# laertispappas/MPI-k-selection

Measured on AMD Instinct MI355X. Metric: Gkeys/s exact k-th select, 2^30 int32 (1 GPU) / 2^33 (8 GPU); % HBM roofline, higher is better.
Workload: dtype int32; 1 GPU; exact k-th select (median) of 2^30 int32 keys per GPU, uniform_half; n_total=1073741824, k=536870912, keys_per_gpu=1073741824, family=uniform_half, parallelism=single, ranks=1

## Files before the change

include/kth.h:

```cpp
#ifndef KTH_H
#define KTH_H

#include <stddef.h>
#include <stdint.h>

#ifdef __cplusplus
extern "C" {
#endif

#define KTH_OK 0
#define KTH_EINVAL (-1)
#define KTH_ENOMEM (-2)
#define KTH_EHIP (-3)
#define KTH_ENODEV (-4)
#define KTH_EINTERNAL (-5)
#define KTH_ECOMM (-6)

#define KTH_VERSION 1

#define KTH_PATH_LDS 1
#define KTH_PATH_RADIX 2
#define KTH_PATH_WINDOW 3
#define KTH_PATH_WINDOW_FALLBACK 4

typedef struct kth_ctx kth_ctx;

typedef struct kth_stats {
    int32_t path;
    int32_t mode;
    uint32_t lo_key, hi_key;
    uint64_t n, k;
    uint64_t cnt_lt;
    uint64_t cnt_eq_lo, cnt_eq_hi;
    uint64_t candidates;
    uint64_t capacity;
    int32_t answer;
    int32_t error;
} kth_stats;

const char *kth_strerror(int code);
int kth_version(void);
const char *kth_build_id(void);
int kth_device_count(void);

int kth_select_i32(const int32_t *keys, int64_t n, int64_t k, int32_t *out);

int kth_ctx_create(int device, kth_ctx **ctx);
int kth_ctx_destroy(kth_ctx *ctx);
int kth_ctx_set_stream(kth_ctx *ctx, void *hip_stream);
int kth_ctx_sync(kth_ctx *ctx);
int kth_ctx_reserve(kth_ctx *ctx, int64_t n);

int kth_select_i32_ctx(kth_ctx *ctx, const int32_t *keys, int64_t n, int64_t k, int32_t *out);

int kth_select_i32_async(kth_ctx *ctx, const int32_t *d_keys, int64_t n, int64_t k, int32_t *d_out);

int kth_ctx_last_stats(kth_ctx *ctx, kth_stats *st);

int kth_ctx_coop(const kth_ctx *ctx);

#define KTH_HOOK_FAULT_TOPK_RANK 1
#define KTH_HOOK_FAULT_BARRIER 2
#define KTH_HOOK_TOPK_SEG_CAP 3
int kth_ctx_test_hook(kth_ctx *ctx, int hook, int64_t value);

int kth_ctx_enable_timing(kth_ctx *ctx, int on);
int kth_ctx_take_timing(kth_ctx *ctx, int64_t *n_selects, double *main_ms, double *total_ms);

#define KTH_ROWS_MAX_COLS 16384
int kth_select_rows_i32(kth_ctx *ctx, const int32_t *d_keys, int64_t rows, int32_t cols, int32_t k,
                        int32_t *d_out);
int kth_select_rows_f32(kth_ctx *ctx, const float *d_keys, int64_t rows, int32_t cols, int32_t k,
                        float *d_out);

#define KTH_TOPK_MAX_COLS 4096
int kth_topk_rows_i32(kth_ctx *ctx, const int32_t *d_keys, int64_t rows, int32_t cols, int32_t k, int largest,
                      int32_t *d_vals, int32_t *d_idx);
int kth_topk_rows_f32(kth_ctx *ctx, const float *d_keys, int64_t rows, int32_t cols, int32_t k, int largest,
                      float *d_vals, int32_t *d_idx);

int kth_topk_i32(kth_ctx *ctx, const int32_t *d_keys, int64_t n, int64_t k, int largest, int32_t *d_vals,
                 int64_t *d_idx);

int kth_fill_synthetic(kth_ctx *ctx, int32_t *d_out, int64_t n, int64_t offset, int64_t n_total,
                       int dist, uint64_t seed, int32_t param);

#define KTH_STATS_WORDS (8 + 2 * 2048)
#define KTH_DIST_DONE 3
#define KTH_DIST_MAX_LEVELS 3
#define KTH_DIST_LEVELS KTH_DIST_MAX_LEVELS
int kth_dist_begin(kth_ctx *ctx, uint64_t *d_slots, int64_t n_total, int64_t k);
int kth_dist_sample(kth_ctx *ctx, const int32_t *d_keys, int64_t n_local, uint32_t *d_sample,
                    int64_t s_local);
int kth_dist_window(kth_ctx *ctx, const uint32_t *d_sample, int64_t s_total);
int kth_dist_scan(kth_ctx *ctx, const int32_t *d_keys, int64_t n_local);
int kth_dist_level(kth_ctx *ctx, const int32_t *d_keys, int64_t n_local, int level);
int kth_dist_result(kth_ctx *ctx, int32_t *d_out);
int kth_dist_result_early(kth_ctx *ctx, int32_t *d_out);
int kth_dist_select_rccl(kth_ctx *ctx, void *nccl_all_reduce, void *nccl_all_gather, void *nccl_comm, int world,
                         const int32_t *d_keys, int64_t n_local, int64_t n_total, int64_t k, uint64_t *d_slots,
                         uint32_t *d_sample, uint32_t *d_gathered, int64_t s_local, int32_t *d_out, int early);
int64_t kth_dist_sample_size(int64_t n);
int kth_sample_chunk(void);
double kth_window_z(void);
int64_t kth_dist_cand_capacity(int64_t n_local);
int kth_window_slack64(void);

typedef struct kth_sharded kth_sharded;
int kth_sharded_create(const int *devices, int ngpu, kth_sharded **out);
int kth_sharded_destroy(kth_sharded *h);
int kth_sharded_select_i32(kth_sharded *h, const int32_t *const *shards, const int64_t *shard_n, int64_t k,
                           int32_t *out);
int kth_select_i32_sharded(const int32_t *const *dev_shards, const int64_t *shard_n, int ngpu, int64_t k,
                           int32_t *out);
int64_t kth_sharded_sample_split(const int64_t *shard_n, int P, int64_t *s_dev);
double kth_sharded_enqueue_us(const kth_sharded *h);

#ifdef __cplusplus
}
#endif
#endif
```

mpi-k-selection_amd/csrc/kth_api.hip:

```cpp
#include <hip/hip_runtime.h>

#include <algorithm>
#include <cmath>
#include <cstdio>
#include <cstdlib>
#include <cstring>
#include <vector>

#include "kth.h"
#include "kth_internal.h"
#include "kth_kernels.hip"
#include "kth_topk.hpp"

using kth::SelState;
using kth::StepArgs;
using kth::u64;

namespace {

constexpr int64_t SMALL_N = 16384;
constexpr int64_t RADIX_MAX_N = 1ll << 22;
constexpr int64_t SAMPLE_MAX = 1ll << 20;
constexpr double WINDOW_Z = 5.0;
double window_z() {
    static const double z = [] {
        const char *e = getenv("KTH_WINDOW_Z");
        const double v = e ? atof(e) : 0.0;
        return v > 0.0 ? v : WINDOW_Z;
    }();
    return z;
}
constexpr int LEVEL_GRID_MAX = 1024;
constexpr int POST_DENSE_GRID = 256;
constexpr int HEAD_GRID_MAX = 64;
int gather_grid(u64 nchunks) {
    const u64 per_wg = (u64)(kth::DENSE_BLK / kth::WAVE) * kth::GATHER_BATCH;
    return (int)std::max<u64>(1, (nchunks + per_wg - 1) / per_wg);
}
constexpr size_t ISLOT_WORDS = 3 * (size_t)kth::STATS_WORDS + 2;
constexpr size_t HSLOT_OFF = ISLOT_WORDS;
constexpr size_t HSLOT_WORDS = (size_t)kth::HEAD_LEVELS * kth::STATS_WORDS;
constexpr size_t FSLOT_OFF = HSLOT_OFF + HSLOT_WORDS;
constexpr size_t FSLOT_WORDS = (size_t)kth::FIN_LEVELS * kth::STATS_WORDS;
constexpr size_t PRE_OFF = FSLOT_OFF + 2 * FSLOT_WORDS;
constexpr size_t PRE_SET_WORDS = (size_t)kth::PRE_WORDS / 2;
static_assert(kth::PRE_WORDS % 4 == 0, "PreHist sets stay 16-byte aligned");
constexpr size_t ZERO_WORDS = PRE_OFF + 2 * PRE_SET_WORDS;
constexpr size_t BAR_OFF = ZERO_WORDS;
constexpr size_t TAIL_OFF = BAR_OFF + kth::BAR_WORDS / 2;
constexpr size_t SLOT_ALLOC_WORDS = TAIL_OFF + kth::FIN_LDS_KEYS / 2;
static_assert(kth::BAR_TAIL % 2 == 0, "the tail word is a u64");
constexpr u64 FIN_SPARSE_PER_WG = (u64)kth::DENSE_BLK * kth::FIN_UNROLL * 4;
constexpr double HEAD_SLACK = 1.5;
static_assert(KTH_STATS_WORDS == kth::STATS_WORDS, "include/kth.h slot size");
constexpr int MAX_EVENTS = 4 * 2048;
constexpr u64 TK_STAGE_MAX_FRAC = 16;
constexpr int TK5_SPLIT = 4;
constexpr int COOP_BACKOFF = 64;
constexpr uint64_t DSCAN_PER_WG = 1ull << 16;

#define HIP_TRY(x)                                                                                    \
    do {                                                                                              \
        hipError_t e_ = (x);                                                                          \
        if (e_ != hipSuccess) {                                                                       \
            if (getenv("KTH_DEBUG")) fprintf(stderr, "kth: %s failed: %s\n", #x, hipGetErrorString(e_)); \
            return KTH_EHIP;                                                                          \
        }                                                                                             \
    } while (0)

#define KTH_TRY(x)              \
    do {                        \
        int r_ = (x);           \
        if (r_ != KTH_OK) return r_; \
    } while (0)

}

struct kth_ctx {
    int device = 0;
    int main_grid[7] = {0, 0, 0, 0, 0, 0, 0};
    bool fault_topk_rank = false;
    bool fault_barrier = false;
    bool fault_once = false;
    bool topk_stage = true;
    u64 topk_seg_cap = 0;
    u64 sparse_per_wg = 0;
    int post_dense_grid = POST_DENSE_GRID;
    int post_sparse_grid = LEVEL_GRID_MAX;
    bool coop = true;
    bool coop_wanted = true;
    int coop_backoff = 0;
    bool coop_resident = true;
    int fin_grid = 256;
    uint32_t head_slack64 = (uint32_t)(HEAD_SLACK * 64);
    uint32_t head_abs_div = 1024;
    int fin_set = 0;
    bool pre_hist = true;
    hipStream_t stream = nullptr;
    bool own_stream = false;
    int num_cu = 256;
    SelState *st = nullptr;
    u64 *islots = nullptr;
    uint32_t *sample = nullptr;
    u64 sample_cap = 0;
    uint32_t *cand = nullptr;
    u64 cand_cap = 0;
    uint32_t *cand_rows = nullptr;
    u64 cand_rows_cap = 0;
    int32_t *tk_segv = nullptr;
    u64 tk_segv_cap = 0;
    uint8_t *tk_segp = nullptr;
    u64 tk_segp_cap = 0;
    uint32_t *tk_wcnt = nullptr;
    u64 tk_wcnt_cap = 0;
    uint32_t *tk_wstart = nullptr;
    u64 tk_wstart_cap = 0;
    kth::TkSeg tk_seg{};
    int32_t *staging = nullptr;
    u64 staging_cap = 0;
    u64 *topk = nullptr;
    u64 topk_cap = 0;
    int32_t *d_status = nullptr;
    int32_t *h_status = nullptr;
    SelState *h_state = nullptr;
    int last_state = -1;
    bool timing = false;
    std::vector<hipEvent_t> ev_main, ev_total;
    int main_used = 0, total_used = 0;
    bool dirty = false;
    bool dist_zero = false;
    bool dist_open = false;
    bool dist_coop_window = false;
    bool counts_left = false;
    u64 *stamps = nullptr;
    int stamp_next = 0;
    u64 *uslots = nullptr;
    int64_t dist_n = 0, dist_k = 0, dist_cap = 0;
    int dist_level_next = 0;
    u64 dscan_per_wg = DSCAN_PER_WG;
    int dist_levels = -1;
    int dist_result_slot = -1;
    int32_t *dist_early_out = nullptr;
    uint32_t *h_dist = nullptr;
    uint32_t *d_dist = nullptr;
    hipEvent_t ev_dist = nullptr;
    uint32_t dist_tag = 0;
};

namespace {

u64 *islot(kth_ctx *c, int i) { return c->islots + (size_t)i * kth::STATS_WORDS; }
u64 *cand_count(kth_ctx *c) { return c->islots + 3 * (size_t)kth::STATS_WORDS; }

int set_device(kth_ctx *c) {
    HIP_TRY(hipSetDevice(c->device));
    return KTH_OK;
}

int grow(void **p, u64 *cap, u64 want_bytes) {
    if (*cap >= want_bytes) return KTH_OK;
    (void)hipDeviceSynchronize();
    if (*p) (void)hipFree(*p);
    *p = nullptr;
    *cap = 0;
    if (hipMalloc(p, want_bytes) != hipSuccess) {
        (void)hipGetLastError();
        *p = nullptr;
        return KTH_ENOMEM;
    }
    *cap = want_bytes;
    return KTH_OK;
}

u64 cand_capacity(int64_t n) { return std::max<u64>(1ull << 20, (u64)n / 32); }

int64_t sample_size(int64_t n) {
    int64_t s = (n / 64) & ~int64_t(63);
    return std::min<int64_t>(SAMPLE_MAX, std::max<int64_t>(s, 64));
}

int reserve_cand(kth_ctx *c, int64_t n) {
    u64 bytes = cand_capacity(n) * 4;
    return grow(reinterpret_cast<void **>(&c->cand), &c->cand_cap, bytes);
}

void window_ranks(int64_t n, int64_t k, int64_t s, u64 *r_lo, u64 *r_hi) {
    const double p = (double)k / (double)n;
    const double r = p * (double)s;
    const double sig = std::sqrt(std::max(1.0, (double)s * p * (1.0 - p)));
    const double z = window_z();
    const double lo = std::floor(r - z * sig - 2.0), hi = std::ceil(r + z * sig + 2.0);
    *r_lo = lo < 1.0 ? 0 : (u64)lo;
    *r_hi = hi > (double)s ? (u64)s + 1 : (u64)std::max(1.0, hi);
}

constexpr int STAMP_LAUNCHES = 16, STAMP_WGS = 4096;
u64 *next_stamps(kth_ctx *c) {
    if (!c->stamps || c->stamp_next >= STAMP_LAUNCHES) return nullptr;
    return c->stamps + (size_t)(c->stamp_next++) * STAMP_WGS * 8;
}

void dump_stamps(kth_ctx *c) {
    if (!c->stamps) return;
    std::vector<u64> h((size_t)STAMP_LAUNCHES * STAMP_WGS * 8);
    (void)hipStreamSynchronize(c->stream);
    (void)hipMemcpy(h.data(), c->stamps, h.size() * 8, hipMemcpyDeviceToHost);
    u64 prev_end = 0;
    for (int l = 0; l < c->stamp_next; ++l) {
        const u64 *b = h.data() + (size_t)l * STAMP_WGS * 8;
        u64 t0 = ~0ull, tend = 0;
        int nwg = 0;
        for (int w = 0; w < STAMP_WGS; ++w)
            if (b[w * 8]) {
                nwg++;
                t0 = std::min(t0, b[w * 8]);
                for (int i = 0; i < 8; ++i) tend = std::max(tend, b[w * 8 + i]);
            }
        if (!nwg) continue;
        fprintf(stderr, "kth-stamps launch %d wgs %4d gap %7.2f |", l, nwg, prev_end ? (t0 - prev_end) / 100.0 : 0.0);
        for (int i = 0; i < 8; ++i) {
            double sum = 0, mx = 0;
            int cnt = 0;
            for (int w = 0; w < STAMP_WGS; ++w)
                if (b[w * 8] && b[w * 8 + i]) {
                    const double d = (b[w * 8 + i] - t0) / 100.0;
                    sum += d;
                    mx = std::max(mx, d);
                    cnt++;
                }
            if (cnt) fprintf(stderr, " p%d %6.2f/%6.2f", i, sum / cnt, mx);
        }
        fprintf(stderr, "\n");
        if (nwg >= 512) {
            std::vector<double> e;
            std::vector<double> ex[8];
            for (int w = 0; w < STAMP_WGS; ++w)
                if (b[w * 8] && b[w * 8 + 5]) {
                    const double d = (b[w * 8 + 5] - t0) / 100.0;
                    e.push_back(d);
                    ex[w % 8].push_back(d);
                }
            std::sort(e.begin(), e.end());
            if (!e.empty()) {
                auto pc = [&](double q) { return e[std::min(e.size() - 1, (size_t)(q * (double)e.size()))]; };
                fprintf(stderr, "kth-stamps   p5 pct: 1%% %.1f 10%% %.1f 25%% %.1f 50%% %.1f 75%% %.1f 90%% %.1f 99%% %.1f max %.1f\n",
                        pc(0.01), pc(0.10), pc(0.25), pc(0.50), pc(0.75), pc(0.90), pc(0.99), e.back());
                fprintf(stderr, "kth-stamps   p5 mean by wg%%8:");
                for (int x = 0; x < 8; ++x) {
                    double sm = 0;
                    for (double d : ex[x]) sm += d;
                    fprintf(stderr, " %.1f", ex[x].empty() ? 0.0 : sm / ex[x].size());
                }
                fprintf(stderr, "\n");
            }
        }
        if (nwg >= 512) {
            for (int x = 0; x < 8; ++x) {
                double sum = 0, mn = 1e30, mx = 0;
                int cnt = 0;
                for (int w = x; w < STAMP_WGS; w += 8)
                    if (b[w * 8] && b[w * 8 + 3]) {
                        const double d = (b[w * 8 + 3] - t0) / 100.0;
                        sum += d;
                        mn = std::min(mn, d);
                        mx = std::max(mx, d);
                        cnt++;
                    }
                if (cnt) fprintf(stderr, "kth-stamps   wg%%8=%d p3 min %7.2f mean %7.2f max %7.2f\n", x, mn, sum / cnt, mx);
            }
        }
        prev_end = tend;
    }
    (void)hipMemsetAsync(c->stamps, 0, h.size() * 8, c->stream);
    c->stamp_next = 0;
}

StepArgs step(kth_ctx *c, int adv, int st_in, int st_out, const u64 *in, u64 *acc, u64 *zero) {
    StepArgs a;
    memset(&a, 0, sizeof a);
    a.stamps = next_stamps(c);
    a.st_in = st_in >= 0 ? c->st + st_in : nullptr;
    a.st_out = c->st + st_out;
    a.stats_in = in;
    a.stats_acc = acc;
    a.stats_zero = zero;
    a.adv = adv;
    a.cand = c->cand;
    a.cand_count = cand_count(c);
    a.cap = c->cand_cap / 4;
    return a;
}

void ev_mark(kth_ctx *c, std::vector<hipEvent_t> &pool, int &used) {
    if (!c->timing || used >= (int)pool.size()) return;
    (void)hipEventRecord(pool[used++], c->stream);
}
void ev_main(kth_ctx *c) { ev_mark(c, c->ev_main, c->main_used); }

int launch_check() {
    hipError_t e = hipGetLastError();
    if (e != hipSuccess) {
        if (getenv("KTH_DEBUG")) fprintf(stderr, "kth: launch failed: %s\n", hipGetErrorString(e));
        return KTH_EHIP;
    }
    return KTH_OK;
}

constexpr u64 DENSE_PER_WG = 1ull << 16;
constexpr u64 SPARSE_PER_WG = (u64)kth::BLK * kth::LEVEL_UNROLL * 4;

int level_grid(u64 count, u64 per_wg) {
    u64 g = (count + per_wg - 1) / per_wg;
    return (int)std::max<u64>(1, std::min<u64>(LEVEL_GRID_MAX, g));
}

u64 sparse_wg(const kth_ctx *c) { return c->sparse_per_wg ? c->sparse_per_wg : SPARSE_PER_WG; }

void launch_level(kth_ctx *c, StepArgs a, bool dense, int grid) {
    if (dense) {
        a.min_per_wg = DENSE_PER_WG;
        kth::k_level<kth::DENSE_BLK><<<grid, kth::DENSE_BLK, 0, c->stream>>>(a);
    } else {
        a.min_per_wg = sparse_wg(c);
        kth::k_level<kth::BLK><<<grid, kth::BLK, 0, c->stream>>>(a);
    }
}

int run_small(kth_ctx *c, const int32_t *keys, int64_t n, int64_t k, int32_t *d_out, int32_t *d_status) {
    c->last_state = 1;
    ev_main(c);
    kth::k_small<<<1, kth::SMALL_BLOCK, (size_t)n * 4, c->stream>>>(keys, (u64)n, (u64)k, d_out, d_status,
                                                                    c->st + 1);
    ev_main(c);
    return launch_check();
}

kth::CoopArgs coop_args(kth_ctx *c, u64 slot_off, int32_t *d_out, int32_t *d_status) {
    kth::CoopArgs x;
    memset(&x, 0, sizeof x);
    x.slots = c->islots + slot_off;
    x.bar = reinterpret_cast<uint32_t *>(c->islots + BAR_OFF);
    x.tail = reinterpret_cast<uint32_t *>(c->islots + TAIL_OFF);
    x.d_out = d_out;
    x.d_status = d_status;
    x.dense_per_wg = DENSE_PER_WG;
    x.sparse_per_wg = FIN_SPARSE_PER_WG;
    x.slack64 = c->head_slack64;
    x.fault = c->fault_barrier ? 1u : 0u;
    if (c->fault_once) c->fault_barrier = false;
    return x;
}

constexpr size_t FIN_DYN_LDS = (size_t)kth::FIN_LDS_KEYS * 4;
uint32_t *pre_set(kth_ctx *c, int set) {
    return reinterpret_cast<uint32_t *>(c->islots + PRE_OFF + (size_t)set * PRE_SET_WORDS);
}

void launch_finish(kth_ctx *c, StepArgs a, int32_t *d_out, int32_t *d_status, bool with_pre = false) {
    const size_t mine = FSLOT_OFF + (size_t)c->fin_set * FSLOT_WORDS;
    a.stats_zero = c->islots + FSLOT_OFF + (size_t)(1 - c->fin_set) * FSLOT_WORDS;
    a.zero_words = FSLOT_WORDS;
    kth::CoopArgs x = coop_args(c, mine, d_out, d_status);
    x.zero2 = c->islots + HSLOT_OFF;
    x.zero2_words = HSLOT_WORDS;
    x.pre = with_pre ? pre_set(c, c->fin_set) : nullptr;
    x.pre_zero = pre_set(c, 1 - c->fin_set);
    kth::k_finish<<<c->fin_grid, kth::DENSE_BLK, FIN_DYN_LDS, c->stream>>>(a, x);
    c->fin_set ^= 1;
}

int run_radix(kth_ctx *c, const int32_t *keys, int64_t n, int64_t k, int32_t *d_out, int32_t *d_status) {
    if (c->coop) {
        StepArgs a = step(c, kth::ADV_INIT_FULL, -1, 1, nullptr, nullptr, nullptr);
        a.keys = keys;
        a.n_local = (u64)n;
        a.init_n = (u64)n;
        a.init_k = (u64)k;
        ev_main(c);
        launch_finish(c, a, d_out, d_status);
        ev_main(c);
        c->last_state = 1;
        return launch_check();
    }
    StepArgs a = step(c, kth::ADV_INIT_FULL, -1, 0, nullptr, islot(c, 1), islot(c, 2));
    a.keys = keys;
    a.n_local = (u64)n;
    a.init_n = (u64)n;
    a.init_k = (u64)k;
    ev_main(c);
    launch_level(c, a, true, level_grid((u64)n, DENSE_PER_WG));
    ev_main(c);
    a = step(c, kth::ADV_PICK, 0, 1, islot(c, 1), islot(c, 2), islot(c, 0));
    a.keys = keys;
    a.n_local = (u64)n;
    launch_level(c, a, false, level_grid((u64)n, sparse_wg(c)));
    a = step(c, kth::ADV_PICK, 1, 0, islot(c, 2), islot(c, 0), islot(c, 1));
    a.keys = keys;
    a.n_local = (u64)n;
    launch_level(c, a, false, level_grid((u64)n, sparse_wg(c)));
    a = step(c, kth::ADV_PICK, 0, 1, islot(c, 0), nullptr, nullptr);
    kth::k_result<<<1, kth::BLK, 0, c->stream>>>(a, d_out, d_status, c->islots, ISLOT_WORDS);
    c->last_state = 1;
    return launch_check();
}

void launch_main(kth_ctx *c, const StepArgs &a, int tflag, uint32_t *tflags) {
    const int g = c->main_grid[tflag];
    const kth::TkSeg none{};
    switch (tflag) {
    case 1: kth::k_main<1><<<g, kth::BLK, 0, c->stream>>>(a, c->cand, tflags, nullptr, none); break;
    case 2: kth::k_main<2><<<g, kth::BLK, 0, c->stream>>>(a, c->cand, tflags, nullptr, none); break;
    case 3: kth::k_main<3><<<g, kth::BLK, 0, c->stream>>>(a, c->cand, tflags, c->cand_rows, none); break;
    case 4: kth::k_main<4><<<g, kth::BLK, 0, c->stream>>>(a, c->cand, tflags, c->cand_rows, none); break;
    case 5: kth::k_main<5><<<g, kth::BLK, 0, c->stream>>>(a, c->cand, tflags, nullptr, c->tk_seg); break;
    case 6: kth::k_main<6><<<g, kth::BLK, 0, c->stream>>>(a, c->cand, tflags, nullptr, c->tk_seg); break;
    default: kth::k_main<0><<<g, kth::BLK, 0, c->stream>>>(a, c->cand, nullptr, nullptr, none); break;
    }
}

int run_window(kth_ctx *c, const int32_t *keys, int64_t n, int64_t k, int32_t *d_out, int32_t *d_status,
               int tflag = 0, uint32_t *tflags = nullptr) {
    const int64_t s = sample_size(n);
    const u64 nchunks = ((u64)s + kth::SAMPLE_CHUNK - 1) / kth::SAMPLE_CHUNK;
    const u64 stride = (u64)n / nchunks;
    u64 r_lo, r_hi;
    window_ranks(n, k, s, &r_lo, &r_hi);
    KTH_TRY(grow(reinterpret_cast<void **>(&c->sample), &c->sample_cap, (u64)s * 4));
    KTH_TRY(reserve_cand(c, n));

    if (c->coop) {
        StepArgs a = step(c, kth::ADV_INIT_SAMPLE, -1, 0, nullptr, nullptr, islot(c, 1));
        a.zero_words = 2 * (u64)kth::STATS_WORDS + 1;
        a.init_n = (u64)n;
        a.init_k = (u64)k;
        a.init_s = (u64)s;
        a.r_lo = r_lo;
        a.r_hi = r_hi;
        kth::CoopArgs hx = coop_args(c, HSLOT_OFF, nullptr, nullptr);
        if (tflag == 0 && c->head_abs_div) hx.abs_min = (u64)s / c->head_abs_div;
        kth::k_head<<<gather_grid(nchunks), kth::DENSE_BLK, 0, c->stream>>>(a, hx, keys, (u64)n, stride, c->sample,
                                                                          (u64)s);
        a = step(c, kth::ADV_CARRY, 0, 1, nullptr, islot(c, 1), nullptr);
        a.keys = keys;
        a.n_local = (u64)n;
        const bool pre = tflag == 0 && c->pre_hist;
        if (pre) a.pre_hist = pre_set(c, c->fin_set);
        ev_main(c);
        launch_main(c, a, tflag, tflags);
        ev_main(c);
        a = step(c, kth::ADV_DECIDE, 1, 0, islot(c, 1), nullptr, nullptr);
        a.keys = keys;
        a.n_local = (u64)n;
        launch_finish(c, a, d_out, d_status, pre);
        c->last_state = 0;
        c->counts_left = true;
        return launch_check();
    }
    StepArgs a = step(c, kth::ADV_INIT_SAMPLE, -1, 0, nullptr, islot(c, 1), islot(c, 2));
    a.init_n = (u64)n;
    a.init_k = (u64)k;
    a.init_s = (u64)s;
    a.r_lo = r_lo;
    a.r_hi = r_hi;
    kth::k_gather<true><<<gather_grid(nchunks), kth::DENSE_BLK, 0, c->stream>>>(a, keys, (u64)n, stride, c->sample,
                                                                              (u64)s);
    const int gs = level_grid((u64)s, sparse_wg(c));
    a = step(c, kth::ADV_PICK, 0, 1, islot(c, 1), islot(c, 2), islot(c, 0));
    a.sample = c->sample;
    a.sample_count = (u64)s;
    launch_level(c, a, false, gs);
    a = step(c, kth::ADV_PICK, 1, 0, islot(c, 2), islot(c, 0), islot(c, 1));
    a.sample = c->sample;
    a.sample_count = (u64)s;
    launch_level(c, a, false, gs);
    a = step(c, kth::ADV_PICK, 0, 1, islot(c, 0), islot(c, 1), islot(c, 2));
    a.keys = keys;
    a.n_local = (u64)n;
    ev_main(c);
    launch_main(c, a, tflag, tflags);
    ev_main(c);
    a = step(c, kth::ADV_DECIDE, 1, 0, islot(c, 1), islot(c, 2), islot(c, 0));
    a.keys = keys;
    a.n_local = (u64)n;
    launch_level(c, a, true, c->post_dense_grid);
    a = step(c, kth::ADV_PICK, 0, 1, islot(c, 2), islot(c, 0), islot(c, 1));
    a.keys = keys;
    a.n_local = (u64)n;
    launch_level(c, a, false, c->post_sparse_grid);
    a = step(c, kth::ADV_PICK, 1, 0, islot(c, 0), islot(c, 1), islot(c, 2));
    a.keys = keys;
    a.n_local = (u64)n;
    launch_level(c, a, false, c->post_sparse_grid);
    a = step(c, kth::ADV_PICK, 0, 1, islot(c, 1), nullptr, nullptr);
    kth::k_result<<<1, kth::BLK, 0, c->stream>>>(a, d_out, d_status, c->islots, ISLOT_WORDS);
    c->last_state = 1;
    return launch_check();
}

void coop_tick(kth_ctx *c) {
    if (c->coop_backoff > 0 && --c->coop_backoff == 0) c->coop = c->coop_wanted;
}

int select_async(kth_ctx *c, const int32_t *d_keys, int64_t n, int64_t k, int32_t *d_out, int32_t *d_status,
                 int tflag = 0, uint32_t *tflags = nullptr) {
    if (!c || !d_keys || (!d_out && !d_status) || n < 1 || k < 1 || k > n) return KTH_EINVAL;
    KTH_TRY(set_device(c));
    coop_tick(c);
    if (c->dirty) {
        HIP_TRY(hipMemsetAsync(c->islots, 0, SLOT_ALLOC_WORDS * sizeof(u64), c->stream));
        c->dirty = false;
    }
    int rc;
    ev_mark(c, c->ev_total, c->total_used);
    if (n <= SMALL_N)
        rc = run_small(c, d_keys, n, k, d_out, d_status);
    else if (n <= RADIX_MAX_N)
        rc = run_radix(c, d_keys, n, k, d_out, d_status);
    else
        rc = run_window(c, d_keys, n, k, d_out, d_status, tflag, tflags);
    ev_mark(c, c->ev_total, c->total_used);
    if (rc != KTH_OK) c->dirty = true;
    if (c->stamps) dump_stamps(c);
    return rc;
}

bool is_device_ptr(const void *p) {
    hipPointerAttribute_t at;
    hipError_t e = hipPointerGetAttributes(&at, p);
    if (e != hipSuccess) {
        (void)hipGetLastError();
        return false;
    }
    return at.type == hipMemoryTypeDevice || at.type == hipMemoryTypeManaged;
}

thread_local kth_ctx *tl_ctx = nullptr;

#ifndef KTH_ROWS_R0
#define KTH_ROWS_R0 4
#endif
template <bool F32, int KPL, bool TOPK>
void launch_rows_reg(kth_ctx *c, bool vec, int g, const uint32_t *d_keys, u64 R, uint32_t C, uint32_t K,
                     uint32_t *d_out, uint32_t flip, uint32_t *vals, int32_t *idx) {
    if (vec && C == (uint32_t)(KPL * kth::WAVE))
        kth::k_rows_reg<F32, KPL, true, KTH_ROWS_R0, TOPK, true>
            <<<g, kth::RW_BLOCK, 0, c->stream>>>(d_keys, R, C, K, d_out, flip, vals, idx);
    else if (vec)
        kth::k_rows_reg<F32, KPL, true, KTH_ROWS_R0, TOPK, false>
            <<<g, kth::RW_BLOCK, 0, c->stream>>>(d_keys, R, C, K, d_out, flip, vals, idx);
    else
        kth::k_rows_reg<F32, KPL, false, KTH_ROWS_R0, TOPK, false>
            <<<g, kth::RW_BLOCK, 0, c->stream>>>(d_keys, R, C, K, d_out, flip, vals, idx);
}

template <bool F32, bool TOPK>
int launch_rows(kth_ctx *c, const uint32_t *d_keys, int64_t rows, int32_t cols, int32_t k, uint32_t *d_out,
                uint32_t flip = 0, uint32_t *vals = nullptr, int32_t *idx = nullptr) {
    const bool vec = (reinterpret_cast<uintptr_t>(d_keys) & 15u) == 0 && cols % 4 == 0;
    const int rows_per_wg = kth::RW_BLOCK / kth::WAVE;
    const int64_t g64 = (rows + rows_per_wg - 1) / rows_per_wg;
    if (g64 > 0x7FFFFFFF) return KTH_EINVAL;
    const int g = (int)g64;
    const u64 R = (u64)rows;
    const uint32_t C = (uint32_t)cols, K = (uint32_t)k;
    if (cols <= 1024)
        launch_rows_reg<F32, 16, TOPK>(c, vec, g, d_keys, R, C, K, d_out, flip, vals, idx);
    else if (cols <= 2048)
        launch_rows_reg<F32, 32, TOPK>(c, vec, g, d_keys, R, C, K, d_out, flip, vals, idx);
    else if (cols <= 4096)
        launch_rows_reg<F32, 64, TOPK>(c, vec, g, d_keys, R, C, K, d_out, flip, vals, idx);
    else if (!TOPK)
        kth::k_rows<F32><<<(int)std::min<int64_t>(rows, 1 << 20), kth::ROWS_BLOCK, (size_t)cols * 4, c->stream>>>(
            d_keys, R, C, (u64)k, d_out);
    return launch_check();
}

}

extern "C" {

const char *kth_strerror(int code) {
    switch (code) {
    case KTH_OK: return "ok";
    case KTH_EINVAL: return "invalid argument";
    case KTH_ENOMEM: return "out of memory";
    case KTH_EHIP: return "HIP runtime error";
    case KTH_ENODEV: return "no HIP device";
    case KTH_EINTERNAL: return "device-side consistency check failed";
    case KTH_ECOMM: return "RCCL unavailable or a collective failed";
    default: return "unknown error";
    }
}

int kth_version(void) { return KTH_VERSION; }

#ifndef KTH_BUILD_ID
#define KTH_BUILD_ID "unknown"
#endif
const char *kth_build_id(void) { return KTH_BUILD_ID; }

int kth_device_count(void) {
    int n = 0;
    if (hipGetDeviceCount(&n) != hipSuccess) {
        (void)hipGetLastError();
        return 0;
    }
    return n;
}

int kth_ctx_create(int device, kth_ctx **out) {
    if (!out) return KTH_EINVAL;
    *out = nullptr;
    int ndev = kth_device_count();
    if (ndev <= 0) return KTH_ENODEV;
    if (device < 0 || device >= ndev) return KTH_EINVAL;
    kth_ctx *c = new kth_ctx();
    c->device = device;
    if (getenv("KTH_STAMPS")) {
        const size_t bytes = (size_t)STAMP_LAUNCHES * STAMP_WGS * 8 * 8;
        if (hipMalloc(reinterpret_cast<void **>(&c->stamps), bytes) != hipSuccess || hipMemset(c->stamps, 0, bytes) != hipSuccess) {
            (void)hipGetLastError();
            c->stamps = nullptr;
        }
    }
    int rc = KTH_OK;
    do {
        if (hipSetDevice(device) != hipSuccess) { rc = KTH_EHIP; break; }
        hipDeviceProp_t prop;
        if (hipGetDeviceProperties(&prop, device) == hipSuccess && prop.multiProcessorCount > 0)
            c->num_cu = prop.multiProcessorCount;
        {
            const void *fns[7] = {reinterpret_cast<const void *>(kth::k_main<0>),
                                  reinterpret_cast<const void *>(kth::k_main<1>),
                                  reinterpret_cast<const void *>(kth::k_main<2>),
                                  reinterpret_cast<const void *>(kth::k_main<3>),
                                  reinterpret_cast<const void *>(kth::k_main<4>),
                                  reinterpret_cast<const void *>(kth::k_main<5>),
                                  reinterpret_cast<const void *>(kth::k_main<6>)};
            const char *e = getenv("KTH_MAIN_WG_PER_CU");
            for (int v = 0; v < 7; ++v) {
                int per = 4;
                hipFuncAttributes fa;
                if (hipFuncGetAttributes(&fa, fns[v]) == hipSuccess && fa.numRegs > 0) {
                    const int alloc = (fa.numRegs + 7) / 8 * 8;
                    const int by_vgpr = std::min(8, 512 / alloc);
                    const int lds = (int)fa.sharedSizeBytes;
                    const int by_lds = lds > 0 ? (160 * 1024) / lds : 8;
                    per = std::max(1, std::min(by_vgpr, by_lds));
                }
                (void)hipGetLastError();
                if (e && atoi(e) > 0) per = atoi(e);
                c->main_grid[v] = c->num_cu * per;
            }
            if (const char *g = getenv("KTH_SPARSE_PER_WG")) c->sparse_per_wg = (u64)std::max(0, atoi(g));
            if (const char *g = getenv("KTH_DSCAN_PER_WG")) c->dscan_per_wg = (u64)std::max(1024, atoi(g));
            if (const char *g = getenv("KTH_POST_DENSE_GRID")) c->post_dense_grid = std::max(1, atoi(g));
            if (const char *g = getenv("KTH_POST_SPARSE_GRID")) c->post_sparse_grid = std::max(1, atoi(g));
            if (const char *g = getenv("KTH_COOP")) c->coop = atoi(g) != 0;
            if (const char *g = getenv("KTH_PRE_HIST")) c->pre_hist = atoi(g) != 0;
            c->fin_grid = c->num_cu;
            if (const char *g = getenv("KTH_FIN_GRID")) c->fin_grid = std::max(1, std::min(atoi(g), c->num_cu));
            if (const char *g = getenv("KTH_HEAD_SLACK")) c->head_slack64 = (uint32_t)std::max(0.0, atof(g) * 64.0);
            if (const char *g = getenv("KTH_HEAD_ABS")) c->head_abs_div = (uint32_t)std::max(0, atoi(g));
            if (const char *g = getenv("KTH_TOPK_STAGE")) c->topk_stage = atoi(g) != 0;
        }
        if (hipStreamCreateWithFlags(&c->stream, hipStreamNonBlocking) != hipSuccess) { rc = KTH_EHIP; break; }
        c->own_stream = true;
        if (hipMalloc(reinterpret_cast<void **>(&c->st), 2 * sizeof(SelState)) != hipSuccess ||
            hipMalloc(reinterpret_cast<void **>(&c->islots), SLOT_ALLOC_WORDS * sizeof(u64)) != hipSuccess ||
            hipMalloc(reinterpret_cast<void **>(&c->d_status), 4 * sizeof(int32_t)) != hipSuccess ||
            hipHostMalloc(reinterpret_cast<void **>(&c->h_status), 4 * sizeof(int32_t), 0) != hipSuccess ||
            hipHostMalloc(reinterpret_cast<void **>(&c->h_state), sizeof(SelState), 0) != hipSuccess) {
            rc = KTH_ENOMEM;
            break;
        }
        if (hipMemset(c->st, 0, 2 * sizeof(SelState)) != hipSuccess ||
            hipMemset(c->islots, 0, SLOT_ALLOC_WORDS * sizeof(u64)) != hipSuccess) {
            rc = KTH_EHIP;
            break;
        }
        (void)hipFuncSetAttribute(reinterpret_cast<const void *>(kth::k_small),
                                  hipFuncAttributeMaxDynamicSharedMemorySize, SMALL_N * 4);
        (void)hipFuncSetAttribute(reinterpret_cast<const void *>(kth::k_rows<false>),
                                  hipFuncAttributeMaxDynamicSharedMemorySize, KTH_ROWS_MAX_COLS * 4);
        (void)hipFuncSetAttribute(reinterpret_cast<const void *>(kth::k_rows<true>),
                                  hipFuncAttributeMaxDynamicSharedMemorySize, KTH_ROWS_MAX_COLS * 4);
        if (hipFuncSetAttribute(reinterpret_cast<const void *>(kth::k_finish),
                                hipFuncAttributeMaxDynamicSharedMemorySize, (int)FIN_DYN_LDS) != hipSuccess)
            c->coop = false;
        (void)hipGetLastError();
        {
            int fin_per_cu = 0, head_per_cu = 0;
            if (hipOccupancyMaxActiveBlocksPerMultiprocessor(&fin_per_cu, reinterpret_cast<const void *>(kth::k_finish),
                                                             kth::DENSE_BLK, FIN_DYN_LDS) != hipSuccess ||
                hipOccupancyMaxActiveBlocksPerMultiprocessor(&head_per_cu, reinterpret_cast<const void *>(kth::k_head),
                                                             kth::DENSE_BLK, 0) != hipSuccess)
                fin_per_cu = head_per_cu = -1;
            (void)hipGetLastError();
            if (fin_per_cu >= 0 &&
                ((int64_t)fin_per_cu * c->num_cu < c->fin_grid || (int64_t)head_per_cu * c->num_cu < HEAD_GRID_MAX)) {
                c->coop = false;
                c->coop_resident = false;
            }
        }
    } while (0);
    c->coop_wanted = c->coop;
    if (rc != KTH_OK) {
        kth_ctx_destroy(c);
        return rc;
    }
    *out = c;
    return KTH_OK;
}

int kth_ctx_test_hook(kth_ctx *c, int hook, int64_t value) {
    if (!c || value < 0) return KTH_EINVAL;
    switch (hook) {
    case KTH_HOOK_FAULT_TOPK_RANK: c->fault_topk_rank = value != 0; return KTH_OK;
    case KTH_HOOK_FAULT_BARRIER:
        if (value > 2) return KTH_EINVAL;
        c->fault_barrier = value != 0;
        c->fault_once = value == 2;
        return KTH_OK;
    case KTH_HOOK_TOPK_SEG_CAP:
        if (value > (int64_t)1 << 40) return KTH_EINVAL;
        c->topk_seg_cap = (u64)value;
        return KTH_OK;
    default: return KTH_EINVAL;
    }
}

int kth_ctx_destroy(kth_ctx *c) {
    if (!c) return KTH_EINVAL;
    (void)hipSetDevice(c->device);
    if (c->stream) (void)hipStreamSynchronize(c->stream);
    for (hipEvent_t e : c->ev_main) (void)hipEventDestroy(e);
    for (hipEvent_t e : c->ev_total) (void)hipEventDestroy(e);
    if (c->st) (void)hipFree(c->st);
    if (c->islots) (void)hipFree(c->islots);
    if (c->sample) (void)hipFree(c->sample);
    if (c->cand) (void)hipFree(c->cand);
    if (c->cand_rows) (void)hipFree(c->cand_rows);
    if (c->tk_segv) (void)hipFree(c->tk_segv);
    if (c->tk_segp) (void)hipFree(c->tk_segp);
    if (c->tk_wcnt) (void)hipFree(c->tk_wcnt);
    if (c->tk_wstart) (void)hipFree(c->tk_wstart);
    if (c->staging) (void)hipFree(c->staging);
    if (c->topk) (void)hipFree(c->topk);
    if (c->d_status) (void)hipFree(c->d_status);
    if (c->stamps) (void)hipFree(c->stamps);
    if (c->h_status) (void)hipHostFree(c->h_status);
    if (c->h_state) (void)hipHostFree(c->h_state);
    if (c->h_dist) (void)hipHostFree(c->h_dist);
    if (c->ev_dist) (void)hipEventDestroy(c->ev_dist);
    if (c->own_stream && c->stream) (void)hipStreamDestroy(c->stream);
    if (tl_ctx == c) tl_ctx = nullptr;
    delete c;
    return KTH_OK;
}

int kth_ctx_set_stream(kth_ctx *c, void *s) {
    if (!c) return KTH_EINVAL;
    KTH_TRY(set_device(c));
    if (c->own_stream && c->stream) {
        (void)hipStreamSynchronize(c->stream);
        (void)hipStreamDestroy(c->stream);
        c->own_stream = false;
    }
    c->stream = reinterpret_cast<hipStream_t>(s);
    return KTH_OK;
}

int kth_ctx_sync(kth_ctx *c) {
    if (!c) return KTH_EINVAL;
    KTH_TRY(set_device(c));
    HIP_TRY(hipStreamSynchronize(c->stream));
    return KTH_OK;
}

int kth_ctx_reserve(kth_ctx *c, int64_t n) {
    if (!c || n < 0) return KTH_EINVAL;
    KTH_TRY(set_device(c));
    if (n > RADIX_MAX_N) {
        KTH_TRY(grow(reinterpret_cast<void **>(&c->sample), &c->sample_cap, (u64)sample_size(n) * 4));
        KTH_TRY(reserve_cand(c, n));
    }
    return KTH_OK;
}

int kth_select_i32_async(kth_ctx *c, const int32_t *d_keys, int64_t n, int64_t k, int32_t *d_out) {
    if (!d_out) return KTH_EINVAL;
    return select_async(c, d_keys, n, k, d_out, nullptr);
}

int kth_select_i32_ctx(kth_ctx *c, const int32_t *keys, int64_t n, int64_t k, int32_t *out) {
    if (!c || !keys || !out || n < 1 || k < 1 || k > n) return KTH_EINVAL;
    KTH_TRY(set_device(c));
    const int32_t *dk = keys;
    if (!is_device_ptr(keys)) {
        KTH_TRY(grow(reinterpret_cast<void **>(&c->staging), &c->staging_cap, (u64)n * 4));
        HIP_TRY(hipMemcpyAsync(c->staging, keys, (size_t)n * 4, hipMemcpyHostToDevice, c->stream));
        dk = c->staging;
    }
    KTH_TRY(select_async(c, dk, n, k, nullptr, c->d_status));
    HIP_TRY(hipMemcpyAsync(c->h_status, c->d_status, 2 * sizeof(int32_t), hipMemcpyDeviceToHost, c->stream));
    HIP_TRY(hipStreamSynchronize(c->stream));
    if (c->h_status[1] == (int32_t)kth::ERR_BARRIER && c->coop) {
        c->dirty = true;
        c->coop = false;
        c->coop_backoff = COOP_BACKOFF + 1;
        KTH_TRY(select_async(c, dk, n, k, nullptr, c->d_status));
        HIP_TRY(hipMemcpyAsync(c->h_status, c->d_status, 2 * sizeof(int32_t), hipMemcpyDeviceToHost, c->stream));
        HIP_TRY(hipStreamSynchronize(c->stream));
    }
    if (c->h_status[1] != 0) {
        c->dirty = true;
        return KTH_EINTERNAL;
    }
    *out = c->h_status[0];
    return KTH_OK;
}

int kth_select_i32(const int32_t *keys, int64_t n, int64_t k, int32_t *out) {
    if (!keys || !out || n < 1 || k < 1 || k > n) return KTH_EINVAL;
    if (!tl_ctx) {
        int dev = 0;
        if (kth_device_count() <= 0) return KTH_ENODEV;
        if (hipGetDevice(&dev) != hipSuccess) {
            (void)hipGetLastError();
            dev = 0;
        }
        KTH_TRY(kth_ctx_create(dev, &tl_ctx));
    }
    return kth_select_i32_ctx(tl_ctx, keys, n, k, out);
}

int kth_ctx_coop(const kth_ctx *c) {
    if (!c) return KTH_EINVAL;
    return c->coop ? 1 : 0;
}

int kth_ctx_last_stats(kth_ctx *c, kth_stats *out) {
    if (!c || !out) return KTH_EINVAL;
    if (c->last_state < 0) return KTH_EINVAL;
    KTH_TRY(set_device(c));
    HIP_TRY(hipMemcpyAsync(c->h_state, c->st + c->last_state, sizeof(SelState), hipMemcpyDeviceToHost,
                           c->stream));
    HIP_TRY(hipStreamSynchronize(c->stream));
    const SelState &s = *c->h_state;
    memset(out, 0, sizeof *out);
    out->path = (int32_t)s.path;
    out->mode = (int32_t)s.mode;
    out->lo_key = s.lo;
    out->hi_key = s.hi;
    out->n = s.n;
    out->k = s.k;
    out->cnt_lt = s.cnt[kth::C_LT];
    out->cnt_eq_lo = s.cnt[kth::C_EQLO];
    out->cnt_eq_hi = s.cnt[kth::C_EQHI];
    out->candidates = s.cnt[kth::C_IN];
    out->capacity = c->cand_cap / 4;
    out->answer = (int32_t)(s.answer ^ 0x80000000u);
    out->error = (int32_t)s.error;
    return KTH_OK;
}

int kth_ctx_enable_timing(kth_ctx *c, int on) {
    if (!c) return KTH_EINVAL;
    KTH_TRY(set_device(c));
    if (on && c->ev_main.empty()) {
        c->ev_main.resize(MAX_EVENTS);
        c->ev_total.resize(MAX_EVENTS);
        for (auto &e : c->ev_main) HIP_TRY(hipEventCreate(&e));
        for (auto &e : c->ev_total) HIP_TRY(hipEventCreate(&e));
    }
    c->timing = on != 0;
    c->main_used = c->total_used = 0;
    return KTH_OK;
}

int kth_ctx_take_timing(kth_ctx *c, int64_t *n_sel, double *main_ms, double *total_ms) {
    if (!c || !n_sel || !main_ms || !total_ms) return KTH_EINVAL;
    KTH_TRY(set_device(c));
    HIP_TRY(hipStreamSynchronize(c->stream));
    double m = 0, t = 0;
    int64_t nm = 0;
    for (int i = 0; i + 1 < c->main_used; i += 2) {
        float a = 0;
        HIP_TRY(hipEventElapsedTime(&a, c->ev_main[i], c->ev_main[i + 1]));
        m += a;
        nm++;
    }
    for (int i = 0; i + 1 < c->total_used; i += 2) {
        float b = 0;
        HIP_TRY(hipEventElapsedTime(&b, c->ev_total[i], c->ev_total[i + 1]));
        t += b;
    }
    c->main_used = c->total_used = 0;
    *n_sel = nm;
    *main_ms = m;
    *total_ms = t;
    return KTH_OK;
}

int kth_select_rows_i32(kth_ctx *c, const int32_t *d_keys, int64_t rows, int32_t cols, int32_t k, int32_t *d_out) {
    if (!c || !d_keys || !d_out || rows < 0 || cols < 1 || cols > KTH_ROWS_MAX_COLS || k < 1 || k > cols)
        return KTH_EINVAL;
    if (rows == 0) return KTH_OK;
    KTH_TRY(set_device(c));
    return launch_rows<false, false>(c, reinterpret_cast<const uint32_t *>(d_keys), rows, cols, k,
                              reinterpret_cast<uint32_t *>(d_out));
}

int kth_select_rows_f32(kth_ctx *c, const float *d_keys, int64_t rows, int32_t cols, int32_t k, float *d_out) {
    if (!c || !d_keys || !d_out || rows < 0 || cols < 1 || cols > KTH_ROWS_MAX_COLS || k < 1 || k > cols)
        return KTH_EINVAL;
    if (rows == 0) return KTH_OK;
    KTH_TRY(set_device(c));
    return launch_rows<true, false>(c, reinterpret_cast<const uint32_t *>(d_keys), rows, cols, k,
                             reinterpret_cast<uint32_t *>(d_out));
}

int kth_topk_rows_i32(kth_ctx *c, const int32_t *d_keys, int64_t rows, int32_t cols, int32_t k, int largest,
                      int32_t *d_vals, int32_t *d_idx) {
    if (!c || !d_keys || (!d_vals && !d_idx) || rows < 0 || cols < 1 || cols > KTH_TOPK_MAX_COLS || k < 1 ||
        k > cols)
        return KTH_EINVAL;
    if (rows == 0) return KTH_OK;
    KTH_TRY(set_device(c));
    return launch_rows<false, true>(c, reinterpret_cast<const uint32_t *>(d_keys), rows, cols, k, nullptr,
                                    largest ? 0xFFFFFFFFu : 0u, reinterpret_cast<uint32_t *>(d_vals), d_idx);
}

int kth_topk_rows_f32(kth_ctx *c, const float *d_keys, int64_t rows, int32_t cols, int32_t k, int largest,
                      float *d_vals, int32_t *d_idx) {
    if (!c || !d_keys || (!d_vals && !d_idx) || rows < 0 || cols < 1 || cols > KTH_TOPK_MAX_COLS || k < 1 ||
        k > cols)
        return KTH_EINVAL;
    if (rows == 0) return KTH_OK;
    KTH_TRY(set_device(c));
    return launch_rows<true, true>(c, reinterpret_cast<const uint32_t *>(d_keys), rows, cols, k, nullptr,
                                   largest ? 0xFFFFFFFFu : 0u, reinterpret_cast<uint32_t *>(d_vals), d_idx);
}

int kth_topk_i32(kth_ctx *c, const int32_t *d_keys, int64_t n, int64_t k, int largest, int32_t *d_vals,
                 int64_t *d_idx) {
    if (!c || !d_keys || (!d_vals && !d_idx) || n < 1 || k < 1 || k > n) return KTH_EINVAL;
    KTH_TRY(set_device(c));
    const u64 ntiles = ((u64)n + kth::TK_TILE - 1) / kth::TK_TILE;
    const u64 nblk = (ntiles + kth::TK_TILES_PER_BLOCK - 1) / kth::TK_TILES_PER_BLOCK;
    u64 head = ((16u - (uint32_t)(reinterpret_cast<uintptr_t>(d_keys) & 15u)) & 15u) >> 2;
    if (head > (u64)n) head = (u64)n;
    const u64 nfull = (((u64)n - head) >> 2) / ((u64)kth::BLK * kth::MAIN_UNROLL);
    const bool aligned = (reinterpret_cast<uintptr_t>(d_keys) & 15u) == 0;
    const bool window = n > RADIX_MAX_N;
    const bool few = (u64)k * kth::TK_TILE * 64 <= (u64)n;
    const bool staged = aligned && window && !few && (u64)k * TK_STAGE_MAX_FRAC <= (u64)n && c->topk_stage;
    const int tf = staged                                  ? (largest ? 6 : 5)
                   : (aligned && window && !few)           ? (largest ? 4 : 3)
                   : (u64)k * kth::TK_TILE <= (u64)n ? (largest ? 2 : 1)
                                                             : 0;
    const u64 ncov = tf >= 3 ? nfull * kth::MAIN_UNROLL : 0;
    const u64 Gm = (u64)c->main_grid[tf];
    const kth::RowWords rwl{Gm, tf >= 3 ? kth::rw_seg_words(nfull, Gm) : kth::fl_seg_bytes(nfull, Gm)};
    const u64 fwords = tf >= 3 ? kth::TF_W0 + rwl.G * (kth::BLK / kth::WAVE) * rwl.seg
                               : 4 + rwl.G * (kth::BLK / kth::WAVE) * rwl.seg / 4;
    const u64 fw64 = (fwords + 1) / 2, before = (ntiles + 1) / 2 + ntiles + 4 * nblk + 2;
    const u64 words = before + fw64 + 32;
    KTH_TRY(grow(reinterpret_cast<void **>(&c->topk), &c->topk_cap, words * sizeof(u64)));
    const u64 foff = (before + 31) & ~31ull;
    uint32_t *tflags = reinterpret_cast<uint32_t *>(c->topk + foff);
    HIP_TRY(hipMemsetAsync(tflags, 0, 16, c->stream));
    if (tf == 3 || tf == 4) {
        KTH_TRY(reserve_cand(c, n));
        KTH_TRY(grow(reinterpret_cast<void **>(&c->cand_rows), &c->cand_rows_cap, c->cand_cap));
    }
    u64 seg_cap = 0;
    uint32_t nwin = 0;
    if (tf >= 5) {
        const u64 nwaves = (u64)c->main_grid[tf] * (kth::BLK / kth::WAVE);
        const u64 seg_total = std::max<u64>({1ull << 20, (u64)n / 16, (u64)k + (u64)k / 8 + (u64)n / 64});
        seg_cap = c->topk_seg_cap ? c->topk_seg_cap : (seg_total + nwaves - 1) / nwaves;
        seg_cap = (seg_cap + 3) & ~3ull;
        KTH_TRY(reserve_cand(c, n));
        KTH_TRY(grow(reinterpret_cast<void **>(&c->tk_segv), &c->tk_segv_cap, seg_cap * nwaves * 4));
        KTH_TRY(grow(reinterpret_cast<void **>(&c->tk_segp), &c->tk_segp_cap, seg_cap * nwaves));
        KTH_TRY(grow(reinterpret_cast<void **>(&c->tk_wcnt), &c->tk_wcnt_cap, ncov * (kth::BLK / kth::WAVE) * 4 + 16));
        const u64 G = (u64)c->main_grid[tf];
        nwin = (uint32_t)(((nfull + G - 1) / G + kth::TK5_WIN_TILES - 1) / kth::TK5_WIN_TILES);
        KTH_TRY(grow(reinterpret_cast<void **>(&c->tk_wstart), &c->tk_wstart_cap, nwaves * std::max(nwin, 1u) * 4));
        const uint32_t nt = (u64)k * 32 >= (u64)n ? 1u : 0u;
        c->tk_seg = kth::TkSeg{c->tk_segv, c->tk_segp, (uint32_t)seg_cap, tflags + 3, c->tk_wstart, nwin, nt};
    }
    int64_t rank = largest ? n - k + 1 : k;
    if (c->fault_topk_rank && n > 1) rank = rank < n ? rank + 1 : rank - 1;
    KTH_TRY(select_async(c, d_keys, n, rank, nullptr, c->d_status, tf, tflags));
    const uint32_t *keys = reinterpret_cast<const uint32_t *>(d_keys);
    const uint32_t flip = largest ? 0xFFFFFFFFu : 0u;
    u64 *toff = c->topk, *bsum = toff + ntiles, *bbase = bsum + 2 * nblk, *meta = bbase + 2 * nblk;
    uint32_t *tcnt = reinterpret_cast<uint32_t *>(meta + 2);
    const SelState *sel_st = c->st + c->last_state;
    const int waves = kth::TK_BLOCK / kth::WAVE;
    const int g = (int)std::min<u64>((ntiles + waves * kth::WAVE - 1) / (waves * kth::WAVE), (u64)c->num_cu * 16);
    if (tf >= 5) {
        auto tk5c = (u64)k * 64 >= (u64)n ? kth::k_tk5_count<true> : kth::k_tk5_count<false>;
        tk5c<<<c->main_grid[tf] * TK5_SPLIT, kth::TK_BLOCK, 0, c->stream>>>(
            c->tk_segv, seg_cap, c->tk_wstart, nwin, (u64)c->main_grid[tf], tflags, nfull, c->d_status, flip,
            c->tk_wcnt, tcnt);
        kth::k_topk_count<true, 2><<<g, kth::TK_BLOCK, 0, c->stream>>>(keys, (u64)n, ntiles, c->d_status, flip, tcnt,
                                                                       tflags, head, nfull, sel_st, ncov);
    } else if (tf >= 3) {
        HIP_TRY(hipMemsetAsync(tcnt, 0, ntiles * 4, c->stream));
        kth::k_topk_cands<<<c->num_cu * 8, kth::TK_BLOCK, 0, c->stream>>>(
            c->cand, c->cand_rows, cand_count(c), c->cand_cap / 4, c->d_status, flip, tcnt, tflags, sel_st);
        kth::k_topk_count<true, 1><<<g, kth::TK_BLOCK, 0, c->stream>>>(keys, (u64)n, ntiles, c->d_status, flip,
                                                                          tcnt, tflags, head, nfull, sel_st, ncov, rwl);
    } else if (aligned) {
        kth::k_topk_count<true, 0><<<g, kth::TK_BLOCK, 0, c->stream>>>(keys, (u64)n, ntiles, c->d_status, flip,
                                                                           tcnt, tflags, head, nfull, sel_st, 0, rwl);
    } else {
        kth::k_topk_count<false, 0><<<g, kth::TK_BLOCK, 0, c->stream>>>(keys, (u64)n, ntiles, c->d_status, flip,
                                                                            tcnt, tflags, head, nfull, sel_st, 0, rwl);
    }
    kth::k_topk_bases<<<(int)nblk, kth::TK_BLOCK, 0, c->stream>>>(
        tcnt, ntiles, toff, bsum, (u64)k, bbase, meta, c->st + c->last_state,
        reinterpret_cast<uint32_t *>(c->islots + BAR_OFF) + kth::BAR_TOPK_ARRIVE);
    if (tf >= 5) {
        auto tk5w = (u64)k * 32 <= (u64)n ? kth::k_tk5_write<kth::TK5_STAGE_SMALL> : kth::k_tk5_write<kth::TK5_STAGE_LARGE>;
        tk5w<<<c->main_grid[tf] * TK5_SPLIT, kth::TK_BLOCK, 0, c->stream>>>(
            c->tk_segv, c->tk_segp, seg_cap, c->tk_wstart, nwin, (u64)c->main_grid[tf], tflags, nfull, c->d_status,
            flip, c->tk_wcnt, tcnt, toff, bbase, meta, d_vals, d_idx);
        kth::k_topk_write<true, true><<<g, kth::TK_BLOCK, 0, c->stream>>>(keys, (u64)n, ntiles, c->d_status, flip,
                                                                          tcnt, toff, bbase, meta, d_vals, d_idx,
                                                                          tflags, ncov);
    } else if (aligned)
        kth::k_topk_write<true><<<g, kth::TK_BLOCK, 0, c->stream>>>(keys, (u64)n, ntiles, c->d_status, flip, tcnt,
                                                                    toff, bbase, meta, d_vals, d_idx);
    else
        kth::k_topk_write<false><<<g, kth::TK_BLOCK, 0, c->stream>>>(keys, (u64)n, ntiles, c->d_status, flip, tcnt,
                                                                     toff, bbase, meta, d_vals, d_idx);
    return launch_check();
}

int kth_fill_synthetic(kth_ctx *c, int32_t *d_out, int64_t n, int64_t offset, int64_t n_total, int dist, uint64_t seed,
                       int32_t param) {
    if (!c || (!d_out && n > 0) || n < 0 || offset < 0 || dist < 0 || dist > 7) return KTH_EINVAL;
    if (n == 0) return KTH_OK;
    KTH_TRY(set_device(c));
    uint32_t step = 1;
    if (n_total > 0 && n_total <= (int64_t)0xFFFFFFFFll) {
        u64 s = (1ull << 32) / (u64)n_total;
        step = s > 0xFFFFFFFFull ? 0xFFFFFFFFu : (s ? (uint32_t)s : 1u);
    }
    const int g = (int)std::min<int64_t>((n + kth::BLK - 1) / kth::BLK, (int64_t)c->num_cu * 16);
    kth::k_fill<<<g, kth::BLK, 0, c->stream>>>(d_out, (u64)n, (u64)offset, step, dist, seed, param);
    return launch_check();
}

int64_t kth_dist_sample_size(int64_t n) { return sample_size(n); }

int kth_sample_chunk(void) { return kth::SAMPLE_CHUNK; }

double kth_window_z(void) { return window_z(); }

int64_t kth_dist_cand_capacity(int64_t n_local) { return (int64_t)cand_capacity(std::max<int64_t>(n_local, 1)); }

int kth_window_slack64(void) { return (int)(HEAD_SLACK * 64); }

int kth_dist_begin(kth_ctx *c, uint64_t *d_slots, int64_t n_total, int64_t k) {
    if (!c || !d_slots || n_total < 1 || k < 1 || k > n_total) return KTH_EINVAL;
    KTH_TRY(set_device(c));
    if (!c->h_dist) {
        if (hipHostMalloc(reinterpret_cast<void **>(&c->h_dist), kth::DIST_STATUS_WORDS * sizeof(uint32_t),
                          hipHostMallocMapped | hipHostMallocCoherent) != hipSuccess) {
            (void)hipGetLastError();
            c->h_dist = nullptr;
            return KTH_ENOMEM;
        }
        HIP_TRY(hipHostGetDevicePointer(reinterpret_cast<void **>(&c->d_dist), c->h_dist, 0));
        HIP_TRY(hipEventCreateWithFlags(&c->ev_dist, hipEventDisableTiming));
    }
    coop_tick(c);
    c->uslots = reinterpret_cast<u64 *>(d_slots);
    c->dist_n = n_total;
    c->dist_k = k;
    c->dist_level_next = -1;
    c->dist_levels = -1;
    c->dist_result_slot = -1;
    c->dist_early_out = nullptr;
    c->dist_zero = true;
    if (c->dirty || c->dist_open || c->counts_left)
        HIP_TRY(hipMemsetAsync(c->islots, 0, SLOT_ALLOC_WORDS * sizeof(u64), c->stream));
    c->dirty = false;
    c->counts_left = false;
    c->dist_open = true;
    return KTH_OK;
}

int kth_dist_sample(kth_ctx *c, const int32_t *d_keys, int64_t n_local, uint32_t *d_sample, int64_t s_local) {
    if (!c || !d_keys || !d_sample || s_local < 64 || s_local % 64 || n_local < s_local) return KTH_EINVAL;
    KTH_TRY(set_device(c));
    const u64 nchunks = ((u64)s_local + kth::SAMPLE_CHUNK - 1) / kth::SAMPLE_CHUNK;
    const u64 stride = (u64)n_local / nchunks;
    StepArgs a;
    memset(&a, 0, sizeof a);
    if (c->dist_zero && c->uslots) {
        a.stats_zero = c->uslots;
        a.zero_words = 3 * (u64)KTH_STATS_WORDS;
    }
    kth::k_gather<false><<<gather_grid(nchunks), kth::DENSE_BLK, 0, c->stream>>>(a, d_keys, (u64)n_local, stride, d_sample,
                                                                                (u64)s_local);
    KTH_TRY(launch_check());
    if (a.zero_words) c->dist_zero = false;
    return KTH_OK;
}

int kth_dist_window(kth_ctx *c, const uint32_t *d_sample, int64_t s_total) {
    if (!c || !d_sample || s_total < 1 || !c->uslots) return KTH_EINVAL;
    KTH_TRY(set_device(c));
    if (c->dist_zero) {
        HIP_TRY(hipMemsetAsync(c->uslots, 0, 3 * (size_t)KTH_STATS_WORDS * 8, c->stream));
        c->dist_zero = false;
    }
    u64 r_lo, r_hi;
    window_ranks(c->dist_n, c->dist_k, s_total, &r_lo, &r_hi);
    if (c->coop && s_total % 64 == 0 && s_total < (1ll << 29)) {
        StepArgs a = step(c, kth::ADV_INIT_SAMPLE, -1, 0, nullptr, nullptr, nullptr);
        a.init_n = (u64)c->dist_n;
        a.init_k = (u64)c->dist_k;
        a.init_s = (u64)s_total;
        a.r_lo = r_lo;
        a.r_hi = r_hi;
        kth::CoopArgs x = coop_args(c, HSLOT_OFF, nullptr, nullptr);
        x.sample_ready = 1;
        const int grid = (int)std::min<int64_t>(64, std::max<int64_t>(1, s_total / (16 * 1024)));
        kth::k_head<<<grid, kth::DENSE_BLK, 0, c->stream>>>(a, x, nullptr, 0, 0, const_cast<uint32_t *>(d_sample),
                                                           (u64)s_total);
        c->dist_coop_window = true;
        return launch_check();
    }
    c->dist_coop_window = false;
    StepArgs a = step(c, kth::ADV_INIT_SAMPLE, -1, 0, nullptr, islot(c, 1), islot(c, 2));
// ... 160 lines not shown
```

mpi-k-selection_amd/csrc/kth_coop.hpp:

```cpp
#pragma once

namespace kth {

struct CoopArgs {
    u64 *slots;
    uint32_t *bar;
    int32_t *d_out, *d_status;
    u64 dense_per_wg, sparse_per_wg;
    uint32_t slack64;
    u64 abs_min;
    u64 *zero2;
    u64 zero2_words;
    uint32_t *tail;
    uint32_t sample_ready;
    uint32_t fault;
    const uint32_t *pre;
    uint32_t *pre_zero;
};

template <int BLOCK>
__device__ __forceinline__ void pick_slot_copies(SelState &ss, const u64 *slot, uint32_t nb, uint32_t copies,
                                                 u64 *tmp , u64 *scratch, u64 *cnt0) {
    constexpr int PER = NBINS / BLOCK;
#pragma unroll
    for (int j = 0; j < PER; ++j)
        tmp[threadIdx.x * PER + j] =
            __hip_atomic_load(slot + NCOUNTS + threadIdx.x * PER + j, __ATOMIC_RELAXED, __HIP_MEMORY_SCOPE_AGENT);
    __syncthreads();
    u64 h0[PER];
#pragma unroll
    for (int j = 0; j < PER; ++j) {
        const uint32_t b = threadIdx.x * PER + j;
        u64 sum = 0;
        if (b < nb)
            for (uint32_t c = 0; c < copies; ++c) sum += tmp[c * nb + b];
        h0[j] = sum;
    }
    __syncthreads();
    pick_state<BLOCK, PER>(ss, h0, h0, true, scratch, nullptr, cnt0);
}

template <int BLOCK>
__device__ __forceinline__ void pick_pre(SelState &ss, const uint32_t *pre, uint32_t nb, u64 *scratch, u64 *cnt0) {
    constexpr int PER = NBINS / BLOCK;
    u64 h0[PER];
#pragma unroll
    for (int j = 0; j < PER; ++j) {
        const uint32_t b = threadIdx.x * PER + j;
        uint32_t sum = 0;
        if (b < nb)
#pragma unroll
            for (int c = 0; c < PRE_COPIES; ++c) sum += pre[c * PRE_BINS + b];
        h0[j] = sum;
    }
    pick_state<BLOCK, PER>(ss, h0, h0, true, scratch, nullptr, cnt0);
}

template <int BLOCK>
__device__ __forceinline__ void hist_flush_copies(uint32_t (*lh)[NBINS], uint32_t nb, uint32_t copies, u64 *acc) {
    __syncthreads();
    u64 *dst = acc + NCOUNTS + (blockIdx.x % copies) * nb;
    for (uint32_t b = threadIdx.x; b < nb; b += BLOCK) {
        const uint32_t c = lh[0][b];
        if (c) atomicAdd(&dst[b], (u64)c);
    }
}

__device__ __forceinline__ uint32_t active_wgs(u64 count, u64 per_wg) {
    const u64 want = (count + per_wg - 1) / per_wg;
    return (uint32_t)(want < (u64)gridDim.x ? want : (u64)gridDim.x);
}

__global__ __launch_bounds__(DENSE_BLK) void k_head(StepArgs a, CoopArgs x, const int32_t *__restrict__ keys,
                                                    u64 n_keys, u64 stride, uint32_t *__restrict__ sample, u64 s) {
    __shared__ SelState ss;
    __shared__ u64 scratch[2 * (DENSE_BLK / WAVE) + 8];
    __shared__ __attribute__((aligned(16))) uint32_t lh[2][NBINS];
    __shared__ uint32_t s_base[BAR_NG];
    KTH_STAMP(a, 0);
    GridBar gb = grid_bar_init(x.bar, s_base);
    for (int i = threadIdx.x; i < 2 * NBINS / 4; i += DENSE_BLK) reinterpret_cast<uint4 *>(&lh[0][0])[i] = make_uint4(0, 0, 0, 0);
    for (u64 i = (u64)blockIdx.x * DENSE_BLK + threadIdx.x; i < a.zero_words; i += (u64)gridDim.x * DENSE_BLK)
        a.stats_zero[i] = 0;
    advance<DENSE_BLK>(ss, a, scratch);
    bool share;
    HistPlan plan = make_plan(ss, &share);
    auto hist_sample = [&]() {
        const CoherentBuf sb(sample, (uint32_t)(s * 4));
        const uint32_t nv = (uint32_t)(s / 4), per = DENSE_BLK * HEAD_UNROLL;
        for (uint32_t v0 = blockIdx.x * per; v0 < nv; v0 += gridDim.x * per) {
            uint4 q[HEAD_UNROLL];
#pragma unroll
            for (int u = 0; u < HEAD_UNROLL; ++u) {
                const uint32_t v = v0 + u * DENSE_BLK + threadIdx.x;
                q[u] = sb.load16(v < nv ? v * 16u : 0u);
            }
#pragma unroll
            for (int u = 0; u < HEAD_UNROLL; ++u) {
                const bool in = v0 + u * DENSE_BLK + threadIdx.x < nv;
                hist_add<DENSE_BLK>(lh, plan, q[u].x, in);
                hist_add<DENSE_BLK>(lh, plan, q[u].y, in);
                hist_add<DENSE_BLK>(lh, plan, q[u].z, in);
                hist_add<DENSE_BLK>(lh, plan, q[u].w, in);
            }
        }
    };
    bool from_chunks = false;
#ifdef KTH_HEAD_STORE_SAMPLE
    constexpr bool kHeadStore = true;
#else
    constexpr bool kHeadStore = false;
#endif
    if (x.sample_ready)
        hist_sample();
    else if (gather_head_fast<DENSE_BLK, kHeadStore>(keys, stride, sample, s, lh, plan, blockIdx.x, gridDim.x))
        from_chunks = !kHeadStore;
    else
        gather_chunks<DENSE_BLK, true, true>(keys, n_keys, stride, sample, s, lh, plan);
#ifdef KTH_HEAD_DIAG
    KTH_STAMP(a, 4);
#endif
    hist_flush<DENSE_BLK>(lh, plan, x.slots);
    KTH_STAMP(a, 1);
#ifdef KTH_HEAD_DIAG
    wait_mem();
    KTH_STAMP(a, 6);
#endif
    const EarlyWindow ew{a.r_lo, a.r_hi, x.slack64, x.abs_min};
    bool ok = true;
    for (int L = 0;; ++L) {
        grid_sync(gb, s_base, ok);
        if (x.fault) ok = false;
        if (L == 0) KTH_STAMP(a, 2);
        if (L == 1) KTH_STAMP(a, 5);
        pick_slot<DENSE_BLK>(ss, x.slots + (size_t)L * STATS_WORDS, share, scratch, &ew);
        if (L == 0) KTH_STAMP(a, 3);
        if (L == 1) KTH_STAMP(a, 6);
        if (ss.mode != MODE_SAMPLE || L + 1 >= HEAD_LEVELS) break;
        plan = make_plan(ss, &share);
        for (int i = threadIdx.x; i < 2 * NBINS / 4; i += DENSE_BLK)
            reinterpret_cast<uint4 *>(&lh[0][0])[i] = make_uint4(0, 0, 0, 0);
        __syncthreads();
        if (from_chunks)
            head_hist_chunks<DENSE_BLK>(keys, stride, s, lh, plan, blockIdx.x, gridDim.x);
        else
            hist_sample();
        hist_flush<DENSE_BLK>(lh, plan, x.slots + (size_t)(L + 1) * STATS_WORDS);
        if (L == 0) KTH_STAMP(a, 4);
    }
    if (blockIdx.x == 0 && threadIdx.x == 0) {
        SelState o = ss;
        const uint32_t berr = __hip_atomic_exchange(x.bar + BAR_ERR, 0u, __ATOMIC_RELAXED, __HIP_MEMORY_SCOPE_AGENT);
        if ((!ok || berr) && !o.error) {
            o.error = ERR_BARRIER;
            o.mode = MODE_DONE;
        } else if (o.mode == MODE_SAMPLE && !o.error) {
            o.error = 16 + o.mode;
            o.mode = MODE_DONE;
        }
        o.share = 0;
        *a.st_out = o;
    }
    grid_bar_finish(gb, s_base);
    KTH_STAMP(a, 7);
}

constexpr int FIN_LDS_KEYS = 32768;
constexpr int FIN_UNROLL = 4;

__device__ __forceinline__ void finish_keys(uint32_t (*lh)[NBINS], const HistPlan &plan, const uint4 &x, bool xr,
                                            uint32_t valid4) {
    const uint32_t X = xr ? 0x80000000u : 0u;
    hist_add<DENSE_BLK>(lh, plan, x.x ^ X, valid4 & 1u);
    hist_add<DENSE_BLK>(lh, plan, x.y ^ X, valid4 & 2u);
    hist_add<DENSE_BLK>(lh, plan, x.z ^ X, valid4 & 4u);
    hist_add<DENSE_BLK>(lh, plan, x.w ^ X, valid4 & 8u);
}

constexpr uint32_t TAIL_STAGE = 2 * NBINS;

__device__ bool finish_tail(const StepArgs &a, SelState &ss, const CoopArgs &x, uint4 *res, u64 nk, bool xr,
                            uint32_t (*lh)[NBINS], u64 *scratch) {
    __shared__ uint32_t s_n, s_last, s_total, s_ln;
    __shared__ uint32_t s_list[WAVE];
    __shared__ u64 s_off, s_c;
    const uint32_t X = xr ? 0x80000000u : 0u;
    const uint32_t W = ss.W, base = ss.base, done = ss.t[0].done, prefix = ss.t[0].prefix;
    const uint32_t psh = W - done;
    const uint32_t nv = (uint32_t)((nk + 3) / 4);
    u64 *ctl = reinterpret_cast<u64 *>(x.bar + BAR_TAIL);
    uint32_t *stage = &lh[0][0];
    const int lane = threadIdx.x & (WAVE - 1);
    if (threadIdx.x == 0) s_n = 0;
    __syncthreads();
    auto keep = [&](uint32_t key, bool valid) {
        const bool m = valid && ((key - base) >> psh) == prefix;
        const u64 b = __ballot(m);
        if (b == 0) return;
        uint32_t at = 0;
        if (lane == 0) at = atomicAdd(&s_n, (uint32_t)__popcll(b));
        at = __shfl(at, 0, WAVE);
        const uint32_t i = at + (uint32_t)__builtin_amdgcn_mbcnt_hi((uint32_t)(b >> 32), __builtin_amdgcn_mbcnt_lo((uint32_t)b, 0u));
        if (m && i < TAIL_STAGE) stage[i] = key;
    };
    for (uint32_t v0 = 0; v0 < nv; v0 += DENSE_BLK) {
        const uint32_t v = v0 + threadIdx.x;
        uint4 q = make_uint4(0, 0, 0, 0);
        uint32_t valid4 = 0;
        if (v < nv) {
            q = res[v];
            const u64 e = 4ull * v;
            valid4 = nk - e >= 4 ? 0xFu : (1u << (uint32_t)(nk - e)) - 1u;
        }
        keep(q.x ^ X, valid4 & 1u);
        keep(q.y ^ X, valid4 & 2u);
        keep(q.z ^ X, valid4 & 4u);
        keep(q.w ^ X, valid4 & 8u);
    }
    __syncthreads();
    const uint32_t n_mine = s_n;
    if (threadIdx.x == 0) {
        const u64 old = __hip_atomic_fetch_add(ctl, (1ull << 32) | n_mine, __ATOMIC_RELAXED, __HIP_MEMORY_SCOPE_AGENT);
        s_off = (uint32_t)old;
        s_last = (uint32_t)(old >> 32) == gridDim.x - 1u;
        s_total = (uint32_t)old + n_mine;
    }
    __syncthreads();
    const uint32_t off = (uint32_t)s_off;
    if (n_mine <= TAIL_STAGE) {
        for (uint32_t i = threadIdx.x; i < n_mine; i += DENSE_BLK)
            if (off + i < (uint32_t)FIN_LDS_KEYS)
                __hip_atomic_store(x.tail + off + i, stage[i], __ATOMIC_RELAXED, __HIP_MEMORY_SCOPE_AGENT);
    } else {
        __shared__ uint32_t s_pos;
        if (threadIdx.x == 0) s_pos = 0;
        __syncthreads();
        for (uint32_t v = threadIdx.x; v < nv; v += DENSE_BLK) {
            const uint4 q = res[v];
            const u64 e = 4ull * v;
            const uint32_t valid4 = nk - e >= 4 ? 0xFu : (1u << (uint32_t)(nk - e)) - 1u;
            const uint32_t k4[4] = {q.x ^ X, q.y ^ X, q.z ^ X, q.w ^ X};
#pragma unroll
            for (int j = 0; j < 4; ++j)
                if (((valid4 >> j) & 1u) && ((k4[j] - base) >> psh) == prefix) {
                    const uint32_t i = atomicAdd(&s_pos, 1u);
                    if (off + i < (uint32_t)FIN_LDS_KEYS)
                        __hip_atomic_store(x.tail + off + i, k4[j], __ATOMIC_RELAXED, __HIP_MEMORY_SCOPE_AGENT);
                }
        }
    }
    wait_mem();
    __syncthreads();
    uint32_t *written = x.bar + BAR_TAIL_WRITTEN;
    if (!s_last) {
        if (threadIdx.x == 0) __hip_atomic_fetch_add(written, 1u, __ATOMIC_RELAXED, __HIP_MEMORY_SCOPE_AGENT);
        KTH_STAMP(a, 5);
        return false;
    }
    if (threadIdx.x == 0) {
        uint32_t spins = 0;
        while (__hip_atomic_load(written, __ATOMIC_RELAXED, __HIP_MEMORY_SCOPE_AGENT) != gridDim.x - 1u) {
            __builtin_amdgcn_s_sleep(1);
            if (++spins >= BAR_SPIN_LIMIT) {
                ss.error = ERR_BARRIER;
                ss.mode = MODE_DONE;
                break;
            }
        }
        __hip_atomic_store(written, 0u, __ATOMIC_RELAXED, __HIP_MEMORY_SCOPE_AGENT);
        __hip_atomic_store(ctl, 0ull, __ATOMIC_RELAXED, __HIP_MEMORY_SCOPE_AGENT);
        if (x.fault) {
            ss.error = ERR_BARRIER;
            ss.mode = MODE_DONE;
        }
    }
    __syncthreads();
    KTH_STAMP(a, 5);
    if (ss.error) return true;
    const uint32_t total = s_total;
    if (total > (uint32_t)FIN_LDS_KEYS) {
        if (threadIdx.x == 0) {
            ss.error = 32;
            ss.mode = MODE_DONE;
        }
        __syncthreads();
        return true;
    }
    const uint32_t nq = (total + 3) / 4;
    const uint32_t pad = base + ((prefix ^ 1u) << psh);
    {
        constexpr int TU = FIN_LDS_KEYS / 4 / DENSE_BLK;
        static_assert(TU % FIN_UNROLL == 0, "tail loads in FIN_UNROLL batches");
        const CoherentBuf tb(x.tail, FIN_LDS_KEYS * 4);
        for (int u0 = 0; u0 < TU; u0 += FIN_UNROLL) {
            if ((uint32_t)(u0 * DENSE_BLK) >= nq) break;
            uint4 q[FIN_UNROLL];
#pragma unroll
            for (int u = 0; u < FIN_UNROLL; ++u) {
                const uint32_t v = (u0 + u) * DENSE_BLK + threadIdx.x;
                q[u] = v < nq ? tb.load16(v * 16u) : make_uint4(0, 0, 0, 0);
            }
#pragma unroll
            for (int u = 0; u < FIN_UNROLL; ++u) {
                const uint32_t v = (u0 + u) * DENSE_BLK + threadIdx.x;
                if (v == total / 4 && (total & 3u)) {
                    if ((total & 3u) <= 1) q[u].y = pad;
                    if ((total & 3u) <= 2) q[u].z = pad;
                    q[u].w = pad;
                }
                res[(u0 + u) * DENSE_BLK + threadIdx.x] = q[u];
            }
        }
        __syncthreads();
    }
    KTH_STAMP(a, 6);
    constexpr int PER = NBINS / DENSE_BLK;
    for (int it = 0; ss.mode == MODE_CAND || ss.mode == MODE_FULL; ++it) {
        (void)it;
        const uint32_t dn = ss.t[0].done, pf = ss.t[0].prefix, d = digit_bits(ss, dn);
        const uint32_t msh = W - dn, sh = W - dn - d, mask = (1u << d) - 1u;
        for (int i = threadIdx.x; i < NBINS / 4; i += DENSE_BLK) reinterpret_cast<uint4 *>(&lh[0][0])[i] = make_uint4(0, 0, 0, 0);
        __syncthreads();
        auto add = [&](uint32_t key) {
            const uint32_t v = key - base;
            if ((v >> msh) == pf) atomicAdd(&lh[0][(v >> sh) & mask], 1u);
        };
        for (uint32_t v = threadIdx.x; v < nq; v += DENSE_BLK) {
            const uint4 q = res[v];
            add(q.x);
            add(q.y);
            add(q.z);
            add(q.w);
        }
        __syncthreads();
        u64 h0[PER];
#pragma unroll
        for (int j = 0; j < PER; ++j) h0[j] = lh[0][threadIdx.x * PER + j];
        pick_state<DENSE_BLK, PER>(ss, h0, h0, true, scratch, nullptr, &s_c);
#ifdef KTH_STAMPS_BUILD
        if (it < 2) KTH_STAMP(a, 1 + it);
#endif
        if ((ss.mode == MODE_CAND || ss.mode == MODE_FULL) && s_c <= (u64)WAVE) {
            const uint32_t dl = ss.t[0].done, pl = ss.t[0].prefix, msl = W - dl;
            if (threadIdx.x == 0) s_ln = 0;
            __syncthreads();
            auto put = [&](uint32_t key) {
                const bool m = ((key - base) >> msl) == pl;
                const u64 b = __ballot(m);
                if (b == 0) return;
                uint32_t at = 0;
                if (lane == 0) at = atomicAdd(&s_ln, (uint32_t)__popcll(b));
                at = __shfl(at, 0, WAVE);
                const uint32_t i = at + (uint32_t)__builtin_amdgcn_mbcnt_hi((uint32_t)(b >> 32),
                                                                             __builtin_amdgcn_mbcnt_lo((uint32_t)b, 0u));
                if (m && i < (uint32_t)WAVE) s_list[i] = key;
            };
            for (uint32_t v0 = 0; v0 < nq; v0 += DENSE_BLK) {
                const uint32_t v = v0 + threadIdx.x;
                const uint4 q = v < nq ? res[v] : make_uint4(pad, pad, pad, pad);
                put(q.x);
                put(q.y);
                put(q.z);
                put(q.w);
            }
            __syncthreads();
            if (threadIdx.x < WAVE) {
                const uint32_t ln = s_ln < (uint32_t)WAVE ? s_ln : (uint32_t)WAVE;
                const uint32_t mine = (uint32_t)lane < ln ? s_list[lane] : 0u;
                uint32_t lt = 0, le = 0;
                for (uint32_t j = 0; j < ln; ++j) {
                    const uint32_t o = s_list[j];
                    lt += o < mine ? 1u : 0u;
                    le += o <= mine ? 1u : 0u;
                }
                const u64 kk = ss.t[0].k;
                const bool hit = (uint32_t)lane < ln && (u64)lt < kk && kk <= (u64)le;
                if (hit) ss.answer = mine;
                if (__ballot(hit) == 0 && lane == 0) ss.error = 33;
            }
            __syncthreads();
            if (threadIdx.x == 0) ss.mode = MODE_DONE;
            __syncthreads();
            break;
        }
    }
    KTH_STAMP(a, 3);
    return true;
}

__global__ __launch_bounds__(DENSE_BLK) void k_finish(StepArgs a, CoopArgs x) {
    __shared__ SelState ss;
    __shared__ u64 scratch[2 * (DENSE_BLK / WAVE) + 8];
    __shared__ __attribute__((aligned(16))) uint32_t lh[2][NBINS];
    extern __shared__ uint4 res[];
    __shared__ uint32_t s_base[BAR_NG];
    __shared__ u64 s_cnt0;
    KTH_STAMP(a, 0);
    GridBar gb = grid_bar_init(x.bar, s_base);
    for (int i = threadIdx.x; i < 2 * NBINS / 4; i += DENSE_BLK) reinterpret_cast<uint4 *>(&lh[0][0])[i] = make_uint4(0, 0, 0, 0);
    const uint32_t pre_incomplete = x.pre ? x.pre[PRE_INCOMPLETE] : 1u;
    advance<DENSE_BLK>(ss, a, scratch);
    if (threadIdx.x == 0 && (ss.mode == MODE_CAND || ss.mode == MODE_FULL) && ss.t[0].done == 0)
        ss.d0 = fin_first_digit(ss.W);
    __syncthreads();
    const bool use_pre = pre_incomplete == 0u && ss.mode == MODE_CAND && ss.t[0].done == 0;
    KTH_STAMP(a, 1);
    const uint32_t mode0 = ss.mode;
    const bool live = mode0 == MODE_CAND || mode0 == MODE_FULL;
    const uint32_t *dom = mode0 == MODE_FULL ? reinterpret_cast<const uint32_t *>(a.keys) : a.cand;
    const u64 count = mode0 == MODE_CAND ? min(*a.cand_count, a.cap) : a.n_local;
    const bool xr = mode0 == MODE_FULL;
    const bool aligned = (reinterpret_cast<uintptr_t>(dom) & 15u) == 0;
    const bool resident = live && count <= (u64)gridDim.x * FIN_LDS_KEYS;
    u64 b0 = 0, nk = 0;
    if (resident) {
        const u64 per = ((count + gridDim.x - 1) / gridDim.x + 3) & ~(u64)3;
        b0 = min((u64)blockIdx.x * per, count);
        nk = min(per, count - b0);
    }
    bool ok = true, tail = false;
    for (int L = 0; L < FIN_LEVELS; ++L) {
        const uint32_t mode = ss.mode;
        if (mode != MODE_CAND && mode != MODE_FULL) break;
        bool share;
        const HistPlan plan = make_plan(ss, &share);
        if (L > 0) {
            for (int i = threadIdx.x; i < 2 * NBINS / 4; i += DENSE_BLK)
                reinterpret_cast<uint4 *>(&lh[0][0])[i] = make_uint4(0, 0, 0, 0);
            __syncthreads();
        }
        const bool pre0 = L == 0 && use_pre;
        if (resident) {
            const uint32_t nv = (uint32_t)((nk + 3) / 4);
            if (L == 0) {
                const bool one = plan.h[0] && !plan.h[1] && plan.done[0] == 0;
                const uint32_t X = xr ? 0x80000000u : 0u, bs = plan.base, sh = plan.shift[0], mk = plan.mask[0];
                auto add4 = [&](const uint4 &q) {
                    atomicAdd(&lh[0][(((q.x ^ X) - bs) >> sh) & mk], 1u);
                    atomicAdd(&lh[0][(((q.y ^ X) - bs) >> sh) & mk], 1u);
                    atomicAdd(&lh[0][(((q.z ^ X) - bs) >> sh) & mk], 1u);
                    atomicAdd(&lh[0][(((q.w ^ X) - bs) >> sh) & mk], 1u);
                };
                if (aligned) {
                    const uint4 *src = reinterpret_cast<const uint4 *>(dom + b0);
                    for (uint32_t v0 = 0; v0 < nv; v0 += FIN_UNROLL * DENSE_BLK) {
                        uint4 q[FIN_UNROLL];
#pragma unroll
                        for (int u = 0; u < FIN_UNROLL; ++u) {
                            const uint32_t v = v0 + u * DENSE_BLK + threadIdx.x;
                            q[u] = v < nv ? load_nt(src + v) : make_uint4(0, 0, 0, 0);
                        }
#pragma unroll
                        for (int u = 0; u < FIN_UNROLL; ++u) {
                            const uint32_t v = v0 + u * DENSE_BLK + threadIdx.x;
                            if (v < nv) {
                                const u64 e = 4ull * v;
                                res[v] = q[u];
                                if (pre0)
                                    ;
                                else if (one && nk - e >= 4)
                                    add4(q[u]);
                                else
                                    finish_keys(lh, plan, q[u], xr, nk - e >= 4 ? 0xFu : (1u << (uint32_t)(nk - e)) - 1u);
                            }
                        }
                    }
                } else {
                    for (uint32_t v = threadIdx.x; v < nv; v += DENSE_BLK) {
                        uint4 q = make_uint4(0, 0, 0, 0);
                        const u64 e = b0 + 4ull * v, left = b0 + nk - e;
                        q.x = dom[e];
                        if (left > 1) q.y = dom[e + 1];
                        if (left > 2) q.z = dom[e + 2];
                        if (left > 3) q.w = dom[e + 3];
                        res[v] = q;
                        if (!pre0) finish_keys(lh, plan, q, xr, left >= 4 ? 0xFu : (1u << (uint32_t)left) - 1u);
                    }
                }
            } else {
                for (uint32_t v = threadIdx.x; v < nv; v += DENSE_BLK) {
                    const u64 e = 4ull * v;
                    finish_keys(lh, plan, res[v], xr, nk - e >= 4 ? 0xFu : (1u << (uint32_t)(nk - e)) - 1u);
                }
            }
        } else if (!pre0) {
            const uint32_t active = active_wgs(count, L == 0 ? x.dense_per_wg : x.sparse_per_wg);
            auto f = [&](const uint32_t *k, uint32_t valid, auto full) {
#pragma unroll
                for (int j = 0; j < 4 * FIN_UNROLL; ++j)
                    hist_add<DENSE_BLK>(lh, plan, k[j], decltype(full)::value || ((valid >> j) & 1u));
            };
            if (blockIdx.x < active) {
                if (xr)
                    stream_tiles<DENSE_BLK, FIN_UNROLL, true>(dom, count, blockIdx.x, active, f);
                else
                    stream_tiles<DENSE_BLK, FIN_UNROLL, false>(dom, count, blockIdx.x, active, f);
            }
        }
#ifdef KTH_STAMPS_BUILD
        if (pre0) {
            wait_mem();
            KTH_STAMP(a, 2);
        }
#endif
        u64 *slot = x.slots + (size_t)L * STATS_WORDS;
        const uint32_t nb = plan.mask[0] + 1u, copies = L == 0 ? NBINS / nb : 1u;
        if (pre0) {
            pick_pre<DENSE_BLK>(ss, x.pre, nb, scratch, &s_cnt0);
        } else {
            if (copies > 1)
                hist_flush_copies<DENSE_BLK>(lh, nb, copies, slot);
            else
                hist_flush<DENSE_BLK>(lh, plan, slot);
            if (L == 0) KTH_STAMP(a, 2);
            grid_sync(gb, s_base, ok);
            if (x.fault) ok = false;
            if (L == 0) KTH_STAMP(a, 3);
            if (copies > 1)
                pick_slot_copies<DENSE_BLK>(ss, slot, nb, copies, reinterpret_cast<u64 *>(&lh[0][0]), scratch, &s_cnt0);
            else
                pick_slot<DENSE_BLK>(ss, slot, share, scratch, nullptr, &s_cnt0);
        }
        KTH_STAMP(a, 4 + L);
        if (resident && (ss.mode == MODE_CAND || ss.mode == MODE_FULL) && s_cnt0 <= (u64)FIN_LDS_KEYS) {
            tail = true;
            break;
        }
    }
    grid_bar_finish(gb, s_base);
    bool writer = blockIdx.x == 0;
    if (tail) {
        writer = finish_tail(a, ss, x, res, nk, xr, lh, scratch);
    }
    if (writer && threadIdx.x == 0) {
        SelState o = ss;
        const uint32_t berr = __hip_atomic_exchange(x.bar + BAR_ERR, 0u, __ATOMIC_RELAXED, __HIP_MEMORY_SCOPE_AGENT);
        if ((!ok || berr) && !o.error) o.error = ERR_BARRIER;
        if (o.mode != MODE_DONE && !o.error) o.error = 16 + o.mode;
        *a.st_out = o;
        if (x.d_out && !o.error) *x.d_out = i32_of_key(o.answer);
        if (x.d_status) {
            x.d_status[0] = i32_of_key(o.answer);
            x.d_status[1] = (int32_t)o.error;
        }
    }
    for (u64 i = (u64)blockIdx.x * DENSE_BLK + threadIdx.x; i < a.zero_words; i += (u64)gridDim.x * DENSE_BLK)
        a.stats_zero[i] = 0;
    for (u64 i = (u64)blockIdx.x * DENSE_BLK + threadIdx.x; i < x.zero2_words; i += (u64)gridDim.x * DENSE_BLK)
        x.zero2[i] = 0;
    if (x.pre_zero)
        for (u64 i = (u64)blockIdx.x * DENSE_BLK + threadIdx.x; i < (u64)PRE_WORDS; i += (u64)gridDim.x * DENSE_BLK)
            x.pre_zero[i] = 0u;
    KTH_STAMP(a, 7);
}

}
```

mpi-k-selection_amd/csrc/kth_kernels.hip:

```cpp
#include <type_traits>

#include "kth_device.hpp"
#include "kth_gridbar.hpp"

namespace kth {

#define KTH_STR2(x) #x
#define KTH_STR(x) KTH_STR2(x)
constexpr int BLK = 256;
#ifndef KTH_MAIN_UNROLL
#define KTH_MAIN_UNROLL 8
#endif
constexpr int MAIN_UNROLL = KTH_MAIN_UNROLL;
constexpr int MAIN_SUB = MAIN_UNROLL < 8 ? MAIN_UNROLL : 8;
#ifndef KTH_WREG
#define KTH_WREG 2048
#endif
constexpr int WREG = KTH_WREG;
#ifndef KTH_WREG5
#define KTH_WREG5 2496
#endif
constexpr int WREG5 = KTH_WREG5;
constexpr int LEVEL_UNROLL = 8;
constexpr int DENSE_BLK = 1024;
// ... 584 lines not shown
            const uint32_t k4[4] = {q[r].x ^ 0x80000000u, q[r].y ^ 0x80000000u, q[r].z ^ 0x80000000u,
                                    q[r].w ^ 0x80000000u};
#pragma unroll
            for (int j = 0; j < 4; ++j) same = same && code(k4[j], 0) == f0 && code(k4[j], 1) == f1;
        }
        if (HEAD_UNI && __ballot(!same) == 0) {
            if (lane == 0) {
                if (f0 != NONE) atomicAdd(&lh[0][f0], (uint32_t)SAMPLE_CHUNK);
                if (f1 != NONE) atomicAdd(&lh[1][f1], (uint32_t)SAMPLE_CHUNK);
            }
            continue;
        }
#pragma unroll
        for (int r = 0; r < 4; ++r) {
            hist_add<BLOCK>(lh, plan, q[r].x ^ 0x80000000u, true);
            hist_add<BLOCK>(lh, plan, q[r].y ^ 0x80000000u, true);
            hist_add<BLOCK>(lh, plan, q[r].z ^ 0x80000000u, true);
            hist_add<BLOCK>(lh, plan, q[r].w ^ 0x80000000u, true);
        }
    }
}


__device__ __forceinline__ u64 reserve_cands(u64 *cand_count, u64 *acc, u64 cap, uint32_t cnt) {
    const int lane = threadIdx.x & (WAVE - 1);
    u64 g = 0;
    if (lane == WAVE - 1) {
        g = atomicAdd(cand_count, (u64)cnt);
        if (g <= cap && g + cnt > cap) atomicAdd(&acc[C_OVF], 1ull);
    }
    return __shfl(g, WAVE - 1, WAVE);
}

__device__ __forceinline__ void put_cand(uint32_t *p, uint32_t x) {
    __hip_atomic_store(p, x, __ATOMIC_RELAXED, __HIP_MEMORY_SCOPE_AGENT);
}

template <bool ROWS = false>
struct Stager {
    static constexpr uint32_t CAP = ROWS ? WREG / 2 : WREG;
    uint32_t *reg;
    uint32_t wfill;
    u64 winside;
    u64 *cand_count, *acc, cap;
    uint32_t *cand_out;
    uint32_t *rows_out;
    uint32_t flushed;

    __device__ __forceinline__ void put(u64 g, uint32_t cnt) const {
        const int lane = threadIdx.x & (WAVE - 1);
        for (uint32_t i = lane; i < cnt; i += WAVE)
            if (g + i < cap) {
                put_cand(&cand_out[g + i], reg[i]);
                if (ROWS) put_cand(&rows_out[g + i], reg[CAP + i]);
            }
    }

    __device__ __forceinline__ void flush() {
        __builtin_amdgcn_wave_barrier();
        const u64 g = reserve_cands(cand_count, acc, cap, wfill);
        put(g, wfill);
        __builtin_amdgcn_wave_barrier();
        wfill = 0;
        flushed = 1u;
    }

    __device__ __forceinline__ void slot_near(int32_t x, bool near, int32_t slo, int32_t shi, uint32_t &ceqlo,
                                              uint32_t &ceqhi, uint32_t row = ~0u) {
        if (__builtin_amdgcn_ballot_w64(near) == 0) return;
        ceqlo += (near & (x == slo)) ? 1u : 0u;
        ceqhi += (near & (x == shi)) ? 1u : 0u;
        slot((uint32_t)x ^ 0x80000000u, near & (x != slo) & (x != shi), row);
    }

    __device__ __forceinline__ void slot(uint32_t key, bool in, uint32_t row = ~0u) {
        const unsigned long long B = __builtin_amdgcn_ballot_w64(in);
#ifdef KTH_DIAG_NOSTAGE
        if (B == 0x123456789ull) {
#else
        if (B) {
#endif
            const uint32_t nb = (uint32_t)__popcll(B);
            if (wfill + nb > CAP) flush();
            const uint32_t below =
                __builtin_amdgcn_mbcnt_hi((uint32_t)(B >> 32), __builtin_amdgcn_mbcnt_lo((uint32_t)B, 0u));
            if (in) {
                reg[wfill + below] = key;
                if (ROWS) reg[CAP + wfill + below] = row;
            }
            wfill += nb;
            winside += nb;
        }
    }
};

struct TkSeg {
    int32_t *vals;
    uint8_t *pos;
    uint32_t cap;
    uint32_t *ovf;
    uint32_t *wstart;
    uint32_t nwin;
    uint32_t nt;
};
constexpr int TK5_WIN_TILES = 8;

struct OrdStager {
    static constexpr uint32_t CAP = ((uint32_t)WREG5 * 4 / 5) & ~63u;
    uint32_t *reg;
    uint32_t wfill;
    uint32_t seg_fill;
    u64 winside;
    u64 seg_base;
    int32_t slo, shi;
    u64 *cand_count, *acc, cap;
    uint32_t *cand_out;
    TkSeg seg;

    static constexpr int FQ = (int)((CAP + 4 * WAVE - 1) / (4 * WAVE));
    static constexpr int FH = (FQ + 1) / 2;
    __device__ __forceinline__ void flush(bool last = false) {
        const int lane = threadIdx.x & (WAVE - 1);
        __builtin_amdgcn_wave_barrier();
        uint8_t *pb = reinterpret_cast<uint8_t *>(reg + CAP);
        const uint32_t n4 = wfill & ~3u, nw = last ? wfill : n4;
        const u64 base = seg_base + seg_fill;
        const uint32_t room = seg_fill < seg.cap ? seg.cap - seg_fill : 0u;
        const uint4 *r4 = reinterpret_cast<const uint4 *>(reg);
        const uint32_t *p4 = reinterpret_cast<const uint32_t *>(pb);
        auto is_cand = [&](uint32_t x, uint32_t e) { return e < nw && (int32_t)x > slo && (int32_t)x < shi; };
        uint32_t nc = 0;
#pragma unroll 1
        for (int h = 0; h < 2; ++h) {
            uint4 kv[FH];
            uint32_t pv[FH];
#pragma unroll
            for (int j = 0; j < FH; ++j) {
                const uint32_t g = (uint32_t)((h * FH + j) * WAVE + lane);
                kv[j] = 4 * g < nw ? r4[g] : make_uint4(0u, 0u, 0u, 0u);
                pv[j] = 4 * g < nw ? p4[g] : 0u;
            }
#pragma unroll
            for (int j = 0; j < FH; ++j) {
                const uint32_t g = (uint32_t)((h * FH + j) * WAVE + lane), e = 4 * g;
#ifndef KTH_DIAG_TK5_NOSEGSTORE
                if (e + 4 <= n4 && e + 4 <= room) {
                    if (seg.nt) {
                        typedef uint32_t v4u __attribute__((ext_vector_type(4)));
                        const v4u kvv = {kv[j].x, kv[j].y, kv[j].z, kv[j].w};
                        __builtin_nontemporal_store(kvv, reinterpret_cast<v4u *>(seg.vals + base + e));
                        __builtin_nontemporal_store(pv[j], reinterpret_cast<uint32_t *>(seg.pos + base + e));
                    } else {
                        *reinterpret_cast<uint4 *>(seg.vals + base + e) = kv[j];
                        *reinterpret_cast<uint32_t *>(seg.pos + base + e) = pv[j];
                    }
                } else if (last && e < nw) {
                    const uint32_t kq[4] = {kv[j].x, kv[j].y, kv[j].z, kv[j].w};
#pragma unroll
                    for (int q = 0; q < 4; ++q)
                        if (e + q < nw && e + q < room) {
                            seg.vals[base + e + q] = (int32_t)kq[q];
                            seg.pos[base + e + q] = (uint8_t)(pv[j] >> (8 * q));
                        }
                }
#endif
                nc += (is_cand(kv[j].x, e) ? 1u : 0u) + (is_cand(kv[j].y, e + 1) ? 1u : 0u) +
                      (is_cand(kv[j].z, e + 2) ? 1u : 0u) + (is_cand(kv[j].w, e + 3) ? 1u : 0u);
            }
        }
        if (seg_fill + nw > seg.cap && lane == 0) *seg.ovf = 1u;
#ifndef KTH_DIAG_TK5_NOCANDS
        const uint32_t incl = wave_incl_scan32(nc);
        const uint32_t nin = (uint32_t)__builtin_amdgcn_readlane((int)incl, WAVE - 1);
        if (nin) {
            const u64 g0 = reserve_cands(cand_count, acc, cap, nin);
            u64 o = g0 + incl - nc;
#pragma unroll 1
            for (int h = 0; h < 2; ++h) {
                uint4 kv[FH];
#pragma unroll
                for (int j = 0; j < FH; ++j) {
                    const uint32_t g = (uint32_t)((h * FH + j) * WAVE + lane);
                    kv[j] = 4 * g < nw ? r4[g] : make_uint4(0u, 0u, 0u, 0u);
                }
#pragma unroll
                for (int j = 0; j < FH; ++j) {
                    const uint32_t e = 4u * (uint32_t)((h * FH + j) * WAVE + lane);
                    const uint32_t kq[4] = {kv[j].x, kv[j].y, kv[j].z, kv[j].w};
#pragma unroll
                    for (int q = 0; q < 4; ++q)
                        if (is_cand(kq[q], e + q)) {
                            if (o < cap) put_cand(&cand_out[o], kq[q] ^ 0x80000000u);
                            ++o;
                        }
                }
            }
            winside += nin;
        }
#endif
        const uint32_t left = wfill - nw;
        uint32_t kx = 0;
        uint8_t px = 0;
        if ((uint32_t)lane < left) {
            kx = reg[nw + lane];
            px = pb[nw + lane];
        }
        __builtin_amdgcn_wave_barrier();
        if ((uint32_t)lane < left) {
            reg[lane] = kx;
            pb[lane] = px;
        }
        seg_fill += nw;
        wfill = left;
        __builtin_amdgcn_wave_barrier();
    }

    template <int TF>
    __device__ __forceinline__ uint32_t row(const uint4 &q, uint32_t lane, uint32_t &ceqlo, uint32_t &ceqhi) {
        auto f1 = [&](uint32_t x) { return TF == 5 ? (int32_t)x <= shi : (int32_t)x >= slo; };
        const bool c0 = f1(q.x), c1 = f1(q.y), c2 = f1(q.z), c3 = f1(q.w);
        const unsigned long long b0 = __builtin_amdgcn_ballot_w64(c0), b1 = __builtin_amdgcn_ballot_w64(c1),
                                 b2 = __builtin_amdgcn_ballot_w64(c2), b3 = __builtin_amdgcn_ballot_w64(c3);
        if ((b0 | b1 | b2 | b3) == 0) return 0u;
        {
            const int32_t x0 = (int32_t)q.x, x1 = (int32_t)q.y, x2 = (int32_t)q.z, x3 = (int32_t)q.w;
            ceqlo += ((c0 & (x0 == slo)) ? 1u : 0u) + ((c1 & (x1 == slo)) ? 1u : 0u) +
                     ((c2 & (x2 == slo)) ? 1u : 0u) + ((c3 & (x3 == slo)) ? 1u : 0u);
            ceqhi += ((c0 & (x0 == shi)) ? 1u : 0u) + ((c1 & (x1 == shi)) ? 1u : 0u) +
                     ((c2 & (x2 == shi)) ? 1u : 0u) + ((c3 & (x3 == shi)) ? 1u : 0u);
        }
        const uint32_t n0 = (uint32_t)__popcll(b0), n1 = (uint32_t)__popcll(b1), n2 = (uint32_t)__popcll(b2);
        const uint32_t total = n0 + n1 + n2 + (uint32_t)__popcll(b3);
#ifdef KTH_DIAG_TK5_NOSTAGE
        return total;
#endif
        if (wfill + total > CAP) flush();
        uint8_t *pb = reinterpret_cast<uint8_t *>(reg + CAP);
        auto at = [](unsigned long long b, uint32_t base) {
            return __builtin_amdgcn_mbcnt_hi((uint32_t)(b >> 32), __builtin_amdgcn_mbcnt_lo((uint32_t)b, base));
        };
        const uint32_t a0 = at(b0, wfill), a1 = at(b1, wfill + n0), a2 = at(b2, wfill + n0 + n1),
                       a3 = at(b3, wfill + n0 + n1 + n2);
        if (c0) { reg[a0] = q.x; pb[a0] = (uint8_t)lane; }
        if (c1) { reg[a1] = q.y; pb[a1] = (uint8_t)(WAVE + lane); }
        if (c2) { reg[a2] = q.z; pb[a2] = (uint8_t)(2 * WAVE + lane); }
        if (c3) { reg[a3] = q.w; pb[a3] = (uint8_t)(3 * WAVE + lane); }
        wfill += total;
        return total;
    }
};
static_assert(OrdStager::CAP + OrdStager::CAP / 4 <= (uint32_t)WREG5 && OrdStager::CAP >= 4 * WAVE && WREG <= WREG5,
              "OrdStager region: keys + position bytes in one wave's region, >= one wave-row");

template <int CTRL, int ROWS = 0xF>
__device__ __forceinline__ uint32_t dpp_add(uint32_t x) {
    return (uint32_t)__builtin_amdgcn_update_dpp(0, (int)x, CTRL, ROWS, 0xF, false);
}

struct RowAcc {
    uint32_t r[8];
};

template <int K, bool FULL, bool ROWS, int RW = 0>
__device__ __forceinline__ void scan_keys(const uint32_t (&xw)[K], uint32_t valid, int32_t slo, int32_t shi,
                                          uint32_t &clt, uint32_t &ceqlo, uint32_t &ceqhi, Stager<ROWS> &st,
                                          uint32_t row0 = ~0u, RowAcc *ra = nullptr) {
    static_assert(RW == 0 || (FULL && K == 32), "row tallies cover a full tile's 8 rows");
    const uint32_t span = (uint32_t)shi - (uint32_t)slo;
#pragma unroll
    for (int j = 0; j < K; ++j) {
        const int32_t x = (int32_t)xw[j];
        const bool ok = FULL || ((valid >> j) & 1u);
        clt += (ok & (x < slo)) ? 1u : 0u;
        if constexpr (RW == 3) {
            if ((j & 3) == 3) ra->r[j / 4] = clt;
        } else if constexpr (RW == 4) {
            ra->r[j / 4] += x > shi ? 1u : 0u;
        }
        st.slot_near(x, ok & (xw[j] - (uint32_t)slo <= span), slo, shi, ceqlo, ceqhi,
                     row0 == ~0u ? ~0u : row0 + (uint32_t)(j / 4));
    }
}

constexpr uint32_t TK_RECOUNT = 1u << 31;
constexpr u64 TF_W0 = 64;
constexpr int RW_REGS = 16;
struct RowWords {
    u64 G;
    u64 seg;
};
__host__ __device__ __forceinline__ u64 rw_seg_words(u64 nfull, u64 G) {
    return ((nfull + G - 1) / G * MAIN_UNROLL + 63) / 64 * 64;
}
__host__ __device__ __forceinline__ u64 fl_seg_bytes(u64 nfull, u64 G) { return ((nfull + G - 1) / G + 255) / 256 * 256; }
__host__ __device__ __forceinline__ u64 fl_index(const RowWords &L, u64 t, uint32_t w) {
    return ((t % L.G) * (BLK / WAVE) + w) * L.seg + t / L.G;
}
__host__ __device__ __forceinline__ u64 rw_index(const RowWords &L, u64 r, uint32_t w) {
    const u64 t = r / MAIN_UNROLL;
    return TF_W0 + ((t % L.G) * (BLK / WAVE) + w) * L.seg + (t / L.G) * MAIN_UNROLL + r % MAIN_UNROLL;
}
static_assert(MAIN_UNROLL <= 8, "k_main<TF> keeps one row bit per 16-B load slot in a byte");
static_assert(BLK / WAVE == 4, "k_main<TF> stores one flag byte per wave, four per tile (tk_row_flagged's mask)");
template <int TF>
__global__ __launch_bounds__(BLK) void k_main(StepArgs a, uint32_t *__restrict__ cand_out,
                                              uint32_t *__restrict__ tflags, uint32_t *__restrict__ cand_rows,
                                              TkSeg seg) {
    constexpr int U = MAIN_UNROLL, S = MAIN_SUB, K = 4 * S;
#ifdef KTH_DIAG_NOROWS
    constexpr bool ROWS = false;
#else
    constexpr bool ROWS = TF == 3 || TF == 4;
#endif
    constexpr bool ORD = TF >= 5;
    static_assert(U % S == 0, "MAIN_UNROLL is a multiple of MAIN_SUB");
    __shared__ SelState ss;
    __shared__ u64 scratch[2 * (BLK / WAVE) + 8];
    __shared__ __attribute__((aligned(16))) uint32_t region[BLK / WAVE][TF >= 5 ? WREG5 : WREG];
    __shared__ u64 red[6][BLK / WAVE];
    __shared__ uint32_t rowx[BLK / WAVE][4];
    KTH_STAMP(a, 0);
    const uint32_t *p = reinterpret_cast<const uint32_t *>(a.keys);
    const u64 n = a.n_local;
    u64 head = ((16u - (uint32_t)(reinterpret_cast<uintptr_t>(p) & 15u)) & 15u) >> 2;
    if (head > n) head = n;
    const uint4 *__restrict__ v = reinterpret_cast<const uint4 *>(p + head);
    const u64 nv = (n - head) >> 2, tail0 = head + (nv << 2);
    const u64 tile = (u64)BLK * U, nfull = nv / tile;
    auto load_tile = [&](uint4 (&x)[U], u64 t) {
        const uint4 *src = v + t * tile + threadIdx.x;
#ifndef KTH_MAIN_FIRST
#define KTH_MAIN_FIRST 1
#define KTH_MAIN_WAITN 0
#endif
#pragma unroll
        for (int u = 0; u < KTH_MAIN_FIRST; ++u) x[u] = load_nt(src + u * BLK);
        asm volatile("s_waitcnt vmcnt(" KTH_STR(KTH_MAIN_WAITN) ")" ::: "memory");
#pragma unroll
        for (int u = KTH_MAIN_FIRST; u < U; ++u) x[u] = load_nt(src + u * BLK);
    };
    advance<BLK>(ss, a, scratch);
    publish<BLK>(ss, 0, a);
    KTH_STAMP(a, 1);
    if (ss.mode != MODE_MAIN) return;
    const int32_t slo = i32_of_key(ss.lo), shi = i32_of_key(ss.hi);
    const int lane = threadIdx.x & (WAVE - 1), wid = threadIdx.x / WAVE;
    if constexpr (TF != 0) {
        if (blockIdx.x == 0 && threadIdx.x == 0) {
            tflags[0] = (uint32_t)slo;
            tflags[1] = (uint32_t)shi;
            tflags[2] = 1u;
        }
    }
    Stager<ROWS> st{region[wid], 0u, 0ull, a.cand_count, a.stats_acc, a.cap, cand_out, cand_rows, 0u};
    OrdStager os{region[wid], 0u, 0u, 0ull, ((u64)blockIdx.x * (BLK / WAVE) + wid) * seg.cap, slo, shi,
                 a.cand_count, a.stats_acc, a.cap, cand_out, seg};
    uint32_t clt = 0, ceqlo = 0, ceqhi = 0;
    auto ord_keys = [&](const uint4 &q) -> uint32_t {
#ifdef KTH_DIAG_TK5_NOROW
        clt += q.x < (uint32_t)slo;
        return 0u;
#endif
        clt += ((int32_t)q.x < slo ? 1u : 0u) + ((int32_t)q.y < slo ? 1u : 0u) + ((int32_t)q.z < slo ? 1u : 0u) +
               ((int32_t)q.w < slo ? 1u : 0u);
        return os.template row<TF>(q, (uint32_t)lane, ceqlo, ceqhi);
    };
    auto load_tile_ord = [&](uint4 (&x)[U], u64 t) {
        const uint32_t *src = reinterpret_cast<const uint32_t *>(v + t * tile) + wid * (4 * WAVE) + lane;
        x[0].x = load_nt(src);
        asm volatile("s_waitcnt vmcnt(0)" ::: "memory");
        x[0].y = load_nt(src + WAVE);
        x[0].z = load_nt(src + 2 * WAVE);
        x[0].w = load_nt(src + 3 * WAVE);
#pragma unroll
        for (int u = 1; u < U; ++u) {
            const uint32_t *r = src + u * (4 * BLK);
            x[u] = make_uint4(load_nt(r), load_nt(r + WAVE), load_nt(r + 2 * WAVE), load_nt(r + 3 * WAVE));
        }
    };

    constexpr int RW = (TF == 3 || TF == 4) ? TF : 0;
    auto scan_tile = [&](const uint4 (&x)[U], u64 t, RowAcc &ra) {
        static_assert(RW == 0 || U == S, "row tallies: one key group per tile");
#pragma unroll
        for (int h = 0; h < U / S; ++h) {
            uint32_t kk[K];
#pragma unroll
            for (int u = 0; u < S; ++u) {
                kk[4 * u + 0] = x[h * S + u].x;
                kk[4 * u + 1] = x[h * S + u].y;
                kk[4 * u + 2] = x[h * S + u].z;
                kk[4 * u + 3] = x[h * S + u].w;
            }
            scan_keys<K, true, ROWS, RW>(kk, 0xFFFFFFFFu, slo, shi, clt, ceqlo, ceqhi, st,
                                         ROWS ? (uint32_t)(t * U + h * S) : ~0u, &ra);
        }
    };
    uint32_t tiles_done = 0;
    uint32_t tile_word = 0, grp[RW_REGS], wsr = 0, facc = 0;
    uint32_t *const fseg = TF == 1 || TF == 2
                               ? tflags + 4 + ((u64)blockIdx.x * (BLK / WAVE) + wid) * (fl_seg_bytes(nfull, gridDim.x) / 4)
                               : nullptr;
#pragma unroll
    for (int q = 0; q < RW_REGS; ++q) grp[q] = 0u;
    const u64 seg_words = rw_seg_words(nfull, gridDim.x);
    uint32_t *const wseg = tflags + TF_W0 + ((u64)blockIdx.x * (BLK / WAVE) + wid) * seg_words;
    auto flag_tile = [&](const uint4 (&x)[U], u64 t, RowAcc &ra, uint32_t e0, uint32_t c0) {
        if constexpr (TF == 1 || TF == 2) {
            uint32_t rows = 0;
#pragma unroll
            for (int u = 0; u < U; ++u) {
                const int32_t a0 = (int32_t)x[u].x, a1 = (int32_t)x[u].y, a2 = (int32_t)x[u].z, a3 = (int32_t)x[u].w;
                const bool nr = TF == 1 ? min(min(a0, a1), min(a2, a3)) <= shi : max(max(a0, a1), max(a2, a3)) >= slo;
                rows |= (__builtin_amdgcn_ballot_w64(nr) != 0 ? 1u : 0u) << u;
            }
            facc = (uint32_t)lane == (tiles_done / 4) % WAVE ? facc | rows << (8 * (tiles_done % 4)) : facc;
        }
#ifdef KTH_DIAG_NOROWW
        if constexpr (TF >= 5) {
#else
        if constexpr (TF >= 3) {
#endif
            static_assert(U == 8, "k_main<3/4> packs four rows' counts into each of two words");
            if constexpr (TF == 3) {
#pragma unroll
                for (int u = U - 1; u > 0; --u) ra.r[u] -= ra.r[u - 1];
                ra.r[0] -= c0;
            }
            uint32_t b0 = ra.r[0] | ra.r[1] << 8 | ra.r[2] << 16 | ra.r[3] << 24;
            uint32_t b1 = ra.r[4] | ra.r[5] << 8 | ra.r[6] << 16 | ra.r[7] << 24;
            auto half_scan = [](uint32_t c) {
                c += dpp_add<0x111>(c);
                c += dpp_add<0x112>(c);
                c += dpp_add<0x114>(c);
                c += dpp_add<0x118>(c);
                c += dpp_add<0x142, 0xA>(c);
                return c;
            };
#ifndef KTH_DIAG_NOSCAN
            b0 = half_scan(b0);
            b1 = half_scan(b1);
#endif
            uint32_t *rx = rowx[wid];
            if ((lane & 31) == 31) {
                rx[lane >> 5] = b0;
                rx[2 + (lane >> 5)] = b1;
            }
            const uint32_t mark = __builtin_amdgcn_ballot_w64(ceqlo + ceqhi != e0) != 0 ? TK_RECOUNT : 0u;
            __builtin_amdgcn_wave_barrier();
            if (lane < U) {
                const uint32_t q = lane < 4 ? 0u : 2u, sh = 8 * (lane & 3);
                const uint32_t word = ((rx[q] >> sh) & 0xFFu) + ((rx[q + 1] >> sh) & 0xFFu);
                tile_word = word | mark;
            }
            __builtin_amdgcn_wave_barrier();
        }
    };
    static_assert(TK5_WIN_TILES * U == WAVE, "a group of row words is one window of the staged kernels");
    for (u64 t = blockIdx.x; t < nfull; t += gridDim.x) {
        uint4 x[U];
        RowAcc ra{{0u, 0u, 0u, 0u, 0u, 0u, 0u, 0u}};
        const uint32_t e0 = ceqlo + ceqhi, c0 = clt;
        if constexpr (ORD)
            load_tile_ord(x, t);
        else
            load_tile(x, t);
        if constexpr (ORD) {
            uint32_t rw = 0;
#pragma unroll
            for (int u = 0; u < U; ++u) {
                const uint32_t tot = ord_keys(x[u]);
                rw = lane == u ? tot : rw;
            }
            tile_word = rw;
        } else {
            scan_tile(x, t, ra);
            flag_tile(x, t, ra, e0, c0);
        }
        if constexpr (TF == 1 || TF == 2) {
            ++tiles_done;
            if (tiles_done % (4 * WAVE) == 0) {
                fseg[(tiles_done - 4 * WAVE) / 4 + lane] = facc;
                facc = 0;
            }
        }
        if constexpr (TF >= 3) {
            const uint32_t v = (uint32_t)__shfl((int)tile_word, lane & (U - 1), WAVE);
            const bool mine = (uint32_t)(lane / U) == tiles_done % TK5_WIN_TILES;
            const uint32_t gi = (tiles_done / TK5_WIN_TILES) % RW_REGS;
#pragma unroll
            for (int q = 0; q < RW_REGS; ++q) grp[q] = mine && gi == (uint32_t)q ? v : grp[q];
            ++tiles_done;
#ifndef KTH_DIAG_NOPEND
            if (tiles_done % (RW_REGS * TK5_WIN_TILES) == 0) {
#pragma unroll
                for (int q = 0; q < RW_REGS; ++q)
                    wseg[(tiles_done - RW_REGS * TK5_WIN_TILES) * U + q * WAVE + lane] = grp[q];
            }
#endif
            if constexpr (ORD)
                if (tiles_done % TK5_WIN_TILES == 0) {
                    const uint32_t wi = tiles_done / TK5_WIN_TILES;
                    wsr = (uint32_t)lane == wi % WAVE ? os.seg_fill + os.wfill : wsr;
                    if (wi % WAVE == WAVE - 1 && wi - (WAVE - 1) + lane < seg.nwin)
                        seg.wstart[((u64)blockIdx.x * (BLK / WAVE) + wid) * seg.nwin + wi - (WAVE - 1) + lane] = wsr;
                }
        }
    }
    if constexpr (TF == 1 || TF == 2) {
        const uint32_t left = tiles_done % (4 * WAVE);
        if (left != 0 && (uint32_t)lane < (left + 3) / 4) fseg[(tiles_done - left) / 4 + lane] = facc;
    }
    if constexpr (TF >= 3) {
        const uint32_t g0 = tiles_done - tiles_done % (RW_REGS * TK5_WIN_TILES);
#pragma unroll
        for (int q = 0; q < RW_REGS; ++q) {
            const uint32_t t0 = g0 + (uint32_t)q * TK5_WIN_TILES;
            if (t0 < tiles_done && (uint32_t)lane < (tiles_done - t0 < TK5_WIN_TILES ? tiles_done - t0 : TK5_WIN_TILES) * U)
                wseg[t0 * U + lane] = grp[q];
        }
        if constexpr (ORD) {
            const uint32_t wl = tiles_done / TK5_WIN_TILES, w0 = wl - wl % WAVE;
            if (wl % WAVE != WAVE - 1 && (uint32_t)lane <= wl % WAVE && w0 + lane < seg.nwin)
                seg.wstart[((u64)blockIdx.x * (BLK / WAVE) + wid) * seg.nwin + w0 + lane] = wsr;
        }
    }
    if constexpr (ORD) os.flush(true);
    const u64 rem0 = nfull * tile;
    if (blockIdx.x == (uint32_t)(nfull % gridDim.x))
        for (int h = 0; h < U / S; ++h) {
            uint32_t kk[K];
            uint32_t ok = 0;
#pragma unroll
            for (int u = 0; u < S; ++u) {
                const u64 i = rem0 + (h * S + u) * BLK + threadIdx.x;
                const bool in = i < nv;
                const uint4 x = in ? v[i] : make_uint4(0, 0, 0, 0);
                kk[4 * u + 0] = x.x;
                kk[4 * u + 1] = x.y;
                kk[4 * u + 2] = x.z;
                kk[4 * u + 3] = x.w;
                ok |= in ? (0xFu << (4 * u)) : 0u;
            }
            scan_keys<K, false>(kk, ok, slo, shi, clt, ceqlo, ceqhi, st);
        }
    if (blockIdx.x == 0) {
        const bool okh = threadIdx.x < head, okt = threadIdx.x < n - tail0;
        const uint32_t kk[2] = {okh ? p[threadIdx.x] : 0u, okt ? p[tail0 + threadIdx.x] : 0u};
        scan_keys<2, false>(kk, (okh ? 1u : 0u) | (okt ? 2u : 0u), slo, shi, clt, ceqlo, ceqhi, st);
    }
    u64 r0 = clt, r1 = ceqlo, r2 = ceqhi;
#pragma unroll
    for (int o = WAVE / 2; o > 0; o >>= 1) {
        r0 += __shfl_xor(r0, o, WAVE);
        r1 += __shfl_xor(r1, o, WAVE);
        r2 += __shfl_xor(r2, o, WAVE);
    }
    if (lane == 0) {
        red[0][wid] = r0;
        red[1][wid] = r1;
        red[2][wid] = r2;
        red[3][wid] = (ORD ? os.winside : 0ull) + st.winside;
        red[4][wid] = st.wfill;
    }
    __syncthreads();
    if (threadIdx.x < 5) {
        u64 sum = 0;
        for (int w = 0; w < BLK / WAVE; ++w) sum += red[threadIdx.x][w];
        if (threadIdx.x == 4) {
            u64 g = 0;
            if (sum) {
                g = atomicAdd(a.cand_count, sum);
                if (g <= a.cap && g + sum > a.cap) atomicAdd(&a.stats_acc[C_OVF], 1ull);
            }
            red[5][0] = g;
        } else {
            const int slot[4] = {C_LT, C_EQLO, C_EQHI, C_IN};
            if (sum) atomicAdd(&a.stats_acc[slot[threadIdx.x]], sum);
        }
    }
    __syncthreads();
    if (st.wfill) {
        u64 g = red[5][0];
        for (int w = 0; w < wid; ++w) g += red[4][w];
        st.put(g, st.wfill);
    }
    if constexpr (TF == 0) {
        if (a.pre_hist) {
            __shared__ uint32_t phist[PRE_BINS];
            __shared__ uint32_t pflushed;
            const uint32_t W = cand_width(ss.lo, ss.hi);
            const uint32_t d = min(W, fin_first_digit(W)), sh = W - d, base = ss.lo + 1u;
            if (threadIdx.x == 0) pflushed = 0u;
            for (int b = threadIdx.x; b < PRE_BINS; b += BLK) phist[b] = 0u;
            __syncthreads();
            if (lane == 0 && st.flushed) atomicOr(&pflushed, 1u);
            __syncthreads();
            if (pflushed) {
                if (threadIdx.x == 0) atomicAdd(&a.pre_hist[PRE_INCOMPLETE], 1u);
            } else if (W > 0u) {
#pragma unroll
                for (int q = 0; q < BLK / WAVE; ++q) {
                    const uint32_t nq = (uint32_t)red[4][q];
                    for (uint32_t i = threadIdx.x; i < nq; i += BLK) {
                        const uint32_t b = (region[q][i] - base) >> sh, f = __builtin_amdgcn_readfirstlane(b);
                        const u64 act = __ballot(true);
                        if (HEAD_UNI && __ballot(b != f) == 0) {
                            if ((uint32_t)lane == (uint32_t)__builtin_ctzll(act)) atomicAdd(&phist[f], (uint32_t)__popcll(act));
                        } else {
                            atomicAdd(&phist[b], 1u);
                        }
                    }
                }
                __syncthreads();
                uint32_t *dst = a.pre_hist + (blockIdx.x % PRE_COPIES) * PRE_BINS;
                for (uint32_t b = threadIdx.x; b < (1u << d); b += BLK) {
                    const uint32_t c = phist[b];
                    if (c) atomicAdd(&dst[b], c);
                }
            }
        }
    }
    KTH_STAMP(a, 5);
}

__global__ __launch_bounds__(BLK) void k_result(StepArgs a, int32_t *d_out, int32_t *d_status, u64 *izero,
                                                u64 izero_words) {
    __shared__ SelState ss;
    __shared__ u64 scratch[2 * (BLK / WAVE) + 8];
    KTH_STAMP(a, 0);
    advance<BLK>(ss, a, scratch);
    if (threadIdx.x == 0) {
        SelState o = ss;
        if (o.mode != MODE_DONE && !o.error) o.error = 16 + o.mode;
        *a.st_out = o;
        if (d_out && !o.error) *d_out = i32_of_key(o.answer);
        if (d_status) {
            d_status[0] = i32_of_key(o.answer);
            d_status[1] = (int32_t)o.error;
        }
    }
    __syncthreads();
    for (u64 i = threadIdx.x; i < izero_words; i += BLK) izero[i] = 0;
    KTH_STAMP(a, 5);
}

constexpr int DDIG = 12;
constexpr int DNB = 1 << DDIG;
static_assert(DNB == 2 * NBINS, "a stats slot's histogram words hold one DDIG-bit digit");
constexpr uint32_t DIST_FULL_D0 = 32 - 2 * DDIG;

struct CandDom {
    uint32_t base, W, d0;
};
__device__ __forceinline__ CandDom cand_domain(uint32_t lo, uint32_t hi) {
    CandDom d{lo + 1u, 0u, 0u};
    if (hi - lo < 2u) return d;
    const uint32_t range = hi - lo - 2u;
    d.W = range ? 32u - (uint32_t)__clz(range) : 0u;
    const uint32_t nd = (d.W + DDIG - 1) / DDIG;
    d.d0 = d.W - (uint32_t)DDIG * (nd ? nd - 1u : 0u);
    return d;
}

__device__ __forceinline__ void decide_dist(SelState &s, const u64 *c) {
    const u64 L = c[C_LT], E1 = c[C_EQLO], M = c[C_IN], ovf = c[C_OVF];
    const u64 E2 = (s.lo == s.hi) ? 0 : c[C_EQHI];
    for (int i = 0; i < 5; ++i) s.cnt[i] = c[i];
    const u64 k = s.k;
    s.t[1].active = 0;
    s.t[0] = Target{k, 0, 0, 1, 0};
    s.path = 3;
    s.dw = DDIG;
    if (k > L && k <= L + E1) {
        s.answer = s.lo;
        s.mode = MODE_DONE;
    } else if (k > L + E1 && k <= L + E1 + M && ovf == 0) {
        const CandDom d = cand_domain(s.lo, s.hi);
        s.base = d.base;
        s.W = d.W;
        s.d0 = d.d0;
        s.t[0].k = k - L - E1;
        s.mode = MODE_CAND;
        if (s.W == 0) {
            s.answer = s.base;
            s.mode = MODE_DONE;
        }
    } else if (k > L + E1 + M && k <= L + E1 + M + E2) {
        s.answer = s.hi;
        s.mode = MODE_DONE;
    } else {
        s.mode = MODE_FULL;
        s.W = 32;
        s.base = 0;
        s.d0 = DIST_FULL_D0;
        s.path = 4;
    }
}

__device__ __forceinline__ bool dist_live(const SelState &s) {
    return (s.mode == MODE_CAND || s.mode == MODE_FULL) && s.t[0].done < s.W;
}

template <int BLOCK>
__device__ __forceinline__ void pick_wide(SelState &ss, const u64 (&h)[DNB / BLOCK], u64 *scratch) {
    if (!dist_live(ss)) return;
    uint32_t bin;
    u64 below;
    const bool ok = block_pick_vals<BLOCK, DNB / BLOCK>(h, ss.t[0].k, &bin, &below, scratch);
    if (threadIdx.x == 0) {
        const uint32_t d = digit_bits(ss, ss.t[0].done);
        if (!ok || bin >= (1u << d)) {
            ss.error = 1;
            ss.mode = MODE_DONE;
        } else {
            ss.t[0].k -= below;
            ss.t[0].prefix = (ss.t[0].prefix << d) | bin;
            ss.t[0].done += d;
            resolve(ss);
        }
    }
    __syncthreads();
}

template <int BLOCK>
__device__ __forceinline__ void dist_state(SelState &ss, const StepArgs &a, u64 *cnts) {
    constexpr int SV = sizeof(SelState) / 16;
    static_assert(SV <= BLOCK && NCOUNTS <= BLOCK, "state and counts load in one step");
    uint4 sv = make_uint4(0u, 0u, 0u, 0u);
    if (threadIdx.x < SV) sv = reinterpret_cast<const uint4 *>(a.st_in)[threadIdx.x];
    if (a.adv == ADV_DECIDE && threadIdx.x < NCOUNTS) cnts[threadIdx.x] = a.stats_in[threadIdx.x];
    if (threadIdx.x < SV) reinterpret_cast<uint4 *>(&ss)[threadIdx.x] = sv;
    __syncthreads();
    if (a.adv == ADV_DECIDE) {
        if (threadIdx.x == 0 && ss.mode == MODE_MAIN) decide_dist(ss, cnts);
        __syncthreads();
    }
}

template <int BLOCK>
__device__ __forceinline__ void dist_pick(SelState &ss, const StepArgs &a, u64 *scratch) {
    if (a.adv == ADV_DECIDE ? ss.mode != MODE_CAND : !dist_live(ss)) return;
    constexpr int PER = DNB / BLOCK;
    const u64 *b = a.stats_in + NCOUNTS + threadIdx.x * PER;
    u64 h[PER];
#pragma unroll
    for (int j = 0; j < PER; ++j) h[j] = b[j];
    pick_wide<BLOCK>(ss, h, scratch);
}

template <int BLOCK, bool XOR>
__device__ __forceinline__ void dist_hist(uint32_t *lh, const uint32_t *dom, u64 count, uint32_t active,
                                          uint32_t base, uint32_t W, uint32_t done, uint32_t prefix, uint32_t d,
                                          u64 *acc) {
    const uint32_t sh = W - done - d, mask = (1u << d) - 1u, msh = W - done;
    auto f = [&](const uint32_t *k, uint32_t valid, auto full) {
#pragma unroll
        for (int j = 0; j < 4 * LEVEL_UNROLL; ++j) {
            const uint32_t v = k[j] - base;
            if ((decltype(full)::value || ((valid >> j) & 1u)) && ((u64)v >> msh) == (u64)prefix)
                atomicAdd(&lh[(v >> sh) & mask], 1u);
        }
    };
    if (blockIdx.x < active) stream_tiles<BLOCK, LEVEL_UNROLL, XOR>(dom, count, blockIdx.x, active, f);
    __syncthreads();
    for (uint32_t b = threadIdx.x; b <= mask; b += BLOCK) {
        const uint32_t c = lh[b];
        if (c) atomicAdd(&acc[NCOUNTS + b], (u64)c);
    }
}

struct DistStatus {
    uint32_t levels, mode, W, tag;
};
constexpr int DIST_STATUS_WORDS = sizeof(DistStatus) / 4;

template <int BLOCK>
__global__ __launch_bounds__(BLOCK) void k_dscan_hist(StepArgs a) {
    __shared__ __attribute__((aligned(16))) uint32_t lh[DNB];
    const SelState *st = a.st_in;
    const uint32_t mode = st->mode, lo = st->lo, hi = st->hi;
    const u64 count = min(*a.cand_count, a.cap);
    if (mode != MODE_MAIN) return;
    const CandDom dm = cand_domain(lo, hi);
    if (dm.W == 0 || count == 0) return;
    const uint32_t active = (uint32_t)min((u64)gridDim.x, (count + a.min_per_wg - 1) / a.min_per_wg);
    if (blockIdx.x >= active) return;
    for (int i = threadIdx.x; i < DNB / 4; i += BLOCK) reinterpret_cast<uint4 *>(lh)[i] = make_uint4(0, 0, 0, 0);
    __syncthreads();
    dist_hist<BLOCK, false>(lh, a.cand, count, active, dm.base, dm.W, 0u, 0u, dm.d0, a.stats_acc);
}

template <int BLOCK>
__global__ __launch_bounds__(BLOCK) void k_dlevel(StepArgs a) {
    __shared__ SelState ss;
    __shared__ u64 scratch[2 * (BLOCK / WAVE) + 8];
    __shared__ u64 cnts[NCOUNTS];
    __shared__ __attribute__((aligned(16))) uint32_t lh[DNB];
    const u64 cand_n = min(*a.cand_count, a.cap);
    dist_state<BLOCK>(ss, a, cnts);
    {
        const uint32_t m = ss.mode;
        const bool first = a.adv == ADV_DECIDE && m == MODE_FULL;
        const u64 count = m == MODE_CAND ? cand_n : m == MODE_FULL ? a.n_local : 0;
        const u64 per = first ? a.dense_per_wg : a.min_per_wg;
        if (blockIdx.x != 0 && (u64)blockIdx.x * per >= count) return;
    }
    for (int i = threadIdx.x; i < DNB / 4; i += BLOCK) reinterpret_cast<uint4 *>(lh)[i] = make_uint4(0, 0, 0, 0);
    dist_pick<BLOCK>(ss, a, scratch);
    __syncthreads();
    const bool live = dist_live(ss);
    const uint32_t mode = ss.mode, W = ss.W, done = ss.t[0].done, prefix = ss.t[0].prefix, base = ss.base;
    const uint32_t d = live ? digit_bits(ss, done) : 0u;
    if (blockIdx.x == 0) {
        if (threadIdx.x == 0) {
            *a.st_out = ss;
            if (a.host_status) {
                const uint32_t left = live ? W - done - d : 0u;
                const uint32_t v[DIST_STATUS_WORDS] = {1u + (left + DDIG - 1) / DDIG, mode, W, a.tag};
#pragma unroll
                for (int i = 0; i < DIST_STATUS_WORDS; ++i)
                    __hip_atomic_store(&a.host_status[i], v[i], __ATOMIC_RELAXED, __HIP_MEMORY_SCOPE_SYSTEM);
            }
        }
        if (a.stats_zero)
            for (int i = threadIdx.x; i < STATS_WORDS; i += BLOCK) a.stats_zero[i] = 0;
    }
    if (!live) return;
    const u64 count = mode == MODE_CAND ? cand_n : a.n_local;
    const u64 per = done == 0 ? a.dense_per_wg : a.min_per_wg;
    const uint32_t active = (uint32_t)min((u64)gridDim.x, (count + per - 1) / per);
    if (blockIdx.x >= active) return;
    if (mode == MODE_FULL)
        dist_hist<BLOCK, true>(lh, reinterpret_cast<const uint32_t *>(a.keys), count, active, base, W, done, prefix,
                               d, a.stats_acc);
    else
        dist_hist<BLOCK, false>(lh, a.cand, count, active, base, W, done, prefix, d, a.stats_acc);
}

template <int BLOCK>
__global__ __launch_bounds__(BLOCK) void k_dresult(StepArgs a, int32_t *d_out, int32_t *d_status, u64 *izero,
                                                   u64 izero_words, uint32_t early) {
    __shared__ SelState ss;
    __shared__ u64 scratch[2 * (BLOCK / WAVE) + 8];
    __shared__ u64 cnts[NCOUNTS];
    if (blockIdx.x == 0 || early) {
        dist_state<BLOCK>(ss, a, cnts);
        dist_pick<BLOCK>(ss, a, scratch);
        if (early && dist_live(ss) && !ss.error) return;
    }
    if (blockIdx.x == 0) {
        if (threadIdx.x == 0) {
            SelState o = ss;
            if (o.mode != MODE_DONE && !o.error) o.error = 16 + o.mode;
            *a.st_out = o;
            if (d_out && !o.error) *d_out = i32_of_key(o.answer);
            if (d_status) {
                d_status[0] = i32_of_key(o.answer);
                d_status[1] = (int32_t)o.error;
            }
        }
    }
    uint4 *z = reinterpret_cast<uint4 *>(izero);
    const u64 nz = izero_words / 2;
    for (u64 i = (u64)blockIdx.x * BLOCK + threadIdx.x; i < nz; i += (u64)gridDim.x * BLOCK) z[i] = make_uint4(0, 0, 0, 0);
    if ((izero_words & 1) && blockIdx.x == 0 && threadIdx.x == 0) izero[izero_words - 1] = 0;
}

__global__ __launch_bounds__(SMALL_BLOCK) void k_small(const int32_t *__restrict__ keys, u64 n, u64 k,
                                                       int32_t *d_out, int32_t *d_status, SelState *st_out) {
    extern __shared__ __attribute__((aligned(16))) uint32_t skeys[];
    __shared__ uint32_t hist[NBINS];
    __shared__ u64 scratch[SMALL_BLOCK / WAVE + 4];
    for (u64 i = threadIdx.x; i < n; i += SMALL_BLOCK) skeys[i] = key_of_i32((uint32_t)keys[i]);
    uint32_t prefix = 0, done = 0;
    u64 kk = k;
    bool ok = true;
    while (done < 32) {
        const uint32_t d = digit_bits(32, done), shift = 32 - done - d, mask = (1u << d) - 1u;
        for (int i = threadIdx.x; i < NBINS; i += SMALL_BLOCK) hist[i] = 0;
        __syncthreads();
        for (u64 i = threadIdx.x; i < n; i += SMALL_BLOCK) {
            const uint32_t v = skeys[i];
            if (prefix_match(v, 32, done, prefix)) atomicAdd(&hist[(v >> shift) & mask], 1u);
        }
        __syncthreads();
        uint32_t bin;
        u64 below;
        ok = block_pick<SMALL_BLOCK>([&](int i) { return (u64)hist[i]; }, 1 << d, kk, &bin, &below, scratch);
        if (!ok) break;
        kk -= below;
        prefix = (prefix << d) | bin;
        done += d;
    }
    if (threadIdx.x == 0) {
        if (d_out && ok) d_out[0] = i32_of_key(prefix);
        if (d_status) {
            d_status[0] = i32_of_key(prefix);
            d_status[1] = ok ? 0 : 1;
        }
        if (st_out) {
            SelState o;
            memset(&o, 0, sizeof o);
            o.n = n;
            o.k = k;
            o.mode = MODE_DONE;
            o.W = 32;
            o.answer = prefix;
            o.error = ok ? 0 : 1;
            o.path = 1;
            o.hi = 0xFFFFFFFFu;
            *st_out = o;
        }
    }
}

template <bool F32>
__global__ __launch_bounds__(ROWS_BLOCK) void k_rows(const uint32_t *__restrict__ m, u64 rows, uint32_t cols, u64 k,
                                                     uint32_t *__restrict__ out) {
    extern __shared__ __attribute__((aligned(16))) uint32_t rk[];
    __shared__ uint32_t hist[NBINS];
    __shared__ u64 scratch[ROWS_BLOCK / WAVE + 4];
    for (u64 r = blockIdx.x; r < rows; r += gridDim.x) {
        const uint32_t *row = m + r * (u64)cols;
        const bool vec = ((reinterpret_cast<uintptr_t>(row) & 15u) == 0) && (cols % 4 == 0);
        if (vec) {
            const uint4 *rv = reinterpret_cast<const uint4 *>(row);
// ... 101 lines not shown
```

mpi-k-selection_amd/kselect/__init__.py:

```python
import ctypes

import numpy as np

from ._lib import (
    KTH_DIST_DONE,
    KTH_DIST_MAX_LEVELS,
    KTH_ECOMM,
    KTH_EINTERNAL,
    KTH_EINVAL,
    KTH_ENODEV,
    KTH_HOOK_FAULT_BARRIER,
    KTH_HOOK_FAULT_TOPK_RANK,
    KTH_HOOK_TOPK_SEG_CAP,
    KTH_OK,
    KTH_PATH_LDS,
    KTH_PATH_RADIX,
    KTH_PATH_WINDOW,
    KTH_PATH_WINDOW_FALLBACK,
    KTH_ROWS_MAX_COLS,
    KTH_STATS_WORDS,
    KTH_TOPK_MAX_COLS,
    IntVector,
    KthError,
    KthLibraryMissing,
    KthStats,
    check,
    check_single_runtime,
    hip_runtimes,
    load,
    strerror,
)

LIB = load()

UNIFORM_FULL, UNIFORM_HALF, UNIFORM_REF, ALL_EQUAL, FEW_DISTINCT, SORTED_ASC, SORTED_DESC, MOD_1000 = range(8)
FAMILIES = {
    "uniform_full": UNIFORM_FULL,
    "uniform_half": UNIFORM_HALF,
    "uniform_ref": UNIFORM_REF,
    "all_equal": ALL_EQUAL,
    "few_distinct": FEW_DISTINCT,
    "sorted_asc": SORTED_ASC,
    "sorted_desc": SORTED_DESC,
    "mod_1000": MOD_1000,
}
DEFAULT_SEED = 0x5EED0001


def device_count():
    return LIB.kth_device_count()


def _ptr(x):
    if isinstance(x, int):
        return x
    if hasattr(x, "data_ptr"):
        return x.data_ptr()
    if isinstance(x, np.ndarray):
        return x.ctypes.data
    raise TypeError(f"cannot take the address of {type(x)}")


def _numel(x):
    return x.numel() if hasattr(x, "numel") else len(x)


def _stream_handle(stream):
    if stream is None:
        return None
    if isinstance(stream, int):
        return stream or None
    return stream.cuda_stream or None


class Selector:

    def __init__(self, device=0, stream=None):
        self._ctx = ctypes.c_void_p()
        check(LIB.kth_ctx_create(device, ctypes.byref(self._ctx)), "kth_ctx_create")
        self.device = device
        if stream is not None:
            self.set_stream(stream)

    def close(self):
        if self._ctx:
            LIB.kth_ctx_destroy(self._ctx)
            self._ctx = ctypes.c_void_p()

    def __del__(self):
        try:
            self.close()
        except Exception:
            pass

    def __enter__(self):
        return self

    def __exit__(self, *exc):
        self.close()

    @property
    def handle(self):
        return self._ctx

    def set_stream(self, stream):
        if stream is not None and not isinstance(stream, int):
            check_single_runtime()
        check(LIB.kth_ctx_set_stream(self._ctx, _stream_handle(stream)), "kth_ctx_set_stream")

    def sync(self):
        check(LIB.kth_ctx_sync(self._ctx), "kth_ctx_sync")

    def reserve(self, n):
        check(LIB.kth_ctx_reserve(self._ctx, int(n)), "kth_ctx_reserve")

    def select(self, keys, k, n=None):
        if n is None:
            n = keys.numel() if hasattr(keys, "numel") else len(keys)
        if isinstance(keys, np.ndarray):
            keys = np.ascontiguousarray(keys, dtype=np.int32)
        out = ctypes.c_int32()
        check(LIB.kth_select_i32_ctx(self._ctx, _ptr(keys), int(n), int(k), ctypes.byref(out)),
              "kth_select_i32_ctx")
        return out.value

    def select_async(self, d_keys, n, k, d_out):
        check(LIB.kth_select_i32_async(self._ctx, _ptr(d_keys), int(n), int(k), _ptr(d_out)),
              "kth_select_i32_async")

    def coop(self):
        r = LIB.kth_ctx_coop(self._ctx)
        if r < 0:
            check(r, "kth_ctx_coop")
        return bool(r)

    def test_hook(self, hook, value):
        check(LIB.kth_ctx_test_hook(self._ctx, int(hook), int(value)), "kth_ctx_test_hook")

    def stats(self):
        st = KthStats()
        check(LIB.kth_ctx_last_stats(self._ctx, ctypes.byref(st)), "kth_ctx_last_stats")
        return st.as_dict()

    def rows(self, d_keys, rows, cols, k, d_out, f32=False):
        fn = LIB.kth_select_rows_f32 if f32 else LIB.kth_select_rows_i32
        check(fn(self._ctx, _ptr(d_keys), int(rows), int(cols), int(k), _ptr(d_out)), "kth_select_rows")

    def topk_rows(self, d_keys, rows, cols, k, d_vals=None, d_idx=None, largest=False, f32=False):
        fn = LIB.kth_topk_rows_f32 if f32 else LIB.kth_topk_rows_i32
        check(fn(self._ctx, _ptr(d_keys), int(rows), int(cols), int(k), 1 if largest else 0,
                 _ptr(d_vals) if d_vals is not None else None, _ptr(d_idx) if d_idx is not None else None),
              "kth_topk_rows")

    def topk(self, d_keys, n, k, d_vals=None, d_idx=None, largest=False):
        check(LIB.kth_topk_i32(self._ctx, _ptr(d_keys), int(n), int(k), 1 if largest else 0,
                               _ptr(d_vals) if d_vals is not None else None,
                               _ptr(d_idx) if d_idx is not None else None), "kth_topk_i32")

    def fill(self, d_out, n, family=UNIFORM_FULL, seed=DEFAULT_SEED, param=0, offset=0, n_total=None):
        if isinstance(family, str):
            family = FAMILIES[family]
        if n_total is None:
            n_total = offset + n
        check(LIB.kth_fill_synthetic(self._ctx, _ptr(d_out), int(n), int(offset), int(n_total), int(family),
                                      ctypes.c_uint64(seed), int(param)), "kth_fill_synthetic")

    def enable_timing(self, on=True):
        check(LIB.kth_ctx_enable_timing(self._ctx, 1 if on else 0), "kth_ctx_enable_timing")

    def take_timing(self):
        n = ctypes.c_int64()
        m = ctypes.c_double()
        t = ctypes.c_double()
        check(LIB.kth_ctx_take_timing(self._ctx, ctypes.byref(n), ctypes.byref(m), ctypes.byref(t)),
              "kth_ctx_take_timing")
        return n.value, m.value, t.value


def kth_select(keys, k):
    if isinstance(keys, np.ndarray):
        keys = np.ascontiguousarray(keys, dtype=np.int32)
        n = keys.size
    else:
        n = keys.numel()
    out = ctypes.c_int32()
    check(LIB.kth_select_i32(_ptr(keys), int(n), int(k), ctypes.byref(out)), "kth_select_i32")
    return out.value


class ShardedSelector:

    def __init__(self, devices):
        self.devices = [int(d) for d in devices]
        arr = (ctypes.c_int * len(self.devices))(*self.devices)
        self._h = ctypes.c_void_p()
        check(LIB.kth_sharded_create(arr, len(self.devices), ctypes.byref(self._h)), "kth_sharded_create")

    def select(self, shards, k, sizes=None):
        if len(shards) != len(self.devices):
            raise ValueError(f"{len(shards)} shards for {len(self.devices)} devices")
        sizes = [_numel(s) for s in shards] if sizes is None else [int(x) for x in sizes]
        ptrs = (ctypes.c_void_p * len(shards))(*[_ptr(s) for s in shards])
        ns = (ctypes.c_int64 * len(shards))(*sizes)
        out = ctypes.c_int32()
        check(LIB.kth_sharded_select_i32(self._h, ptrs, ns, int(k), ctypes.byref(out)), "kth_sharded_select_i32")
        return out.value

    def enqueue_us(self):
        return LIB.kth_sharded_enqueue_us(self._h)

    def close(self):
        if self._h:
            LIB.kth_sharded_destroy(self._h)
            self._h = ctypes.c_void_p()

    def __del__(self):
        try:
            self.close()
        except Exception:
            pass


def select_sharded(shards, k, sizes=None):
    sizes = [_numel(s) for s in shards] if sizes is None else [int(x) for x in sizes]
    ptrs = (ctypes.c_void_p * len(shards))(*[_ptr(s) for s in shards])
    ns = (ctypes.c_int64 * len(shards))(*sizes)
    out = ctypes.c_int32()
    check(LIB.kth_select_i32_sharded(ptrs, ns, len(shards), int(k), ctypes.byref(out)), "kth_select_i32_sharded")
    return out.value


class IntVec:

    def __init__(self, capacity):
        self.p = LIB.VecNew(int(capacity))
        if not self.p:
            raise MemoryError("VecNew")

    @classmethod
    def from_array(cls, a):
        a = np.ascontiguousarray(a, dtype=np.int32)
        v = cls(max(1, a.size))
        ctypes.memmove(v.p.contents.data, a.ctypes.data, a.size * 4)
        v.p.contents.size = a.size
        return v

    def add(self, x):
        return LIB.VecAdd(self.p, int(x))

    def get(self, i):
        return LIB.VecGet(self.p, int(i))

    def size(self):
        return LIB.VecGetSize(self.p)

    def array(self):
        n = self.p.contents.size
        return np.ctypeslib.as_array(self.p.contents.data, shape=(n,)).copy() if n else np.empty(0, np.int32)

    def quicksort(self):
        LIB.VecQuickSort(self.p)

    def kth_select(self, k):
        return LIB.VecKthSelect(self.p, int(k))

    def kth_select_ex(self, k):
        out = ctypes.c_int()
        check(LIB.VecKthSelectEx(self.p, int(k), ctypes.byref(out)), "VecKthSelectEx")
        return out.value

    def close(self):
        if self.p:
            LIB.VecDelete(self.p)
            self.p = None

    def __del__(self):
        try:
            self.close()
        except Exception:
            pass
```

mpi-k-selection_amd/kselect/_lib.py:

```python
import ctypes
import os

HERE = os.path.dirname(os.path.abspath(__file__))
PKG_ROOT = os.path.dirname(HERE)
LIB_PATH = os.environ.get("KTH_LIB") or os.path.join(PKG_ROOT, "lib", "libkth.so")

KTH_OK = 0
KTH_EINVAL = -1
KTH_ENOMEM = -2
KTH_EHIP = -3
KTH_ENODEV = -4
KTH_EINTERNAL = -5
KTH_ECOMM = -6

KTH_PATH_LDS, KTH_PATH_RADIX, KTH_PATH_WINDOW, KTH_PATH_WINDOW_FALLBACK = 1, 2, 3, 4
KTH_STATS_WORDS = 8 + 2 * 2048
KTH_DIST_DONE = 3
KTH_DIST_MAX_LEVELS = 3
KTH_ROWS_MAX_COLS = 16384
KTH_TOPK_MAX_COLS = 4096
KTH_HOOK_FAULT_TOPK_RANK, KTH_HOOK_FAULT_BARRIER, KTH_HOOK_TOPK_SEG_CAP = 1, 2, 3

c_i32p = ctypes.POINTER(ctypes.c_int32)
c_u32p = ctypes.POINTER(ctypes.c_uint32)
c_u64p = ctypes.POINTER(ctypes.c_uint64)
c_vp = ctypes.c_void_p


class KthStats(ctypes.Structure):
    _fields_ = [
        ("path", ctypes.c_int32),
        ("mode", ctypes.c_int32),
        ("lo_key", ctypes.c_uint32),
        ("hi_key", ctypes.c_uint32),
        ("n", ctypes.c_uint64),
        ("k", ctypes.c_uint64),
        ("cnt_lt", ctypes.c_uint64),
        ("cnt_eq_lo", ctypes.c_uint64),
        ("cnt_eq_hi", ctypes.c_uint64),
        ("candidates", ctypes.c_uint64),
        ("capacity", ctypes.c_uint64),
        ("answer", ctypes.c_int32),
        ("error", ctypes.c_int32),
    ]

    def as_dict(self):
        return {f: getattr(self, f) for f, _ in self._fields_}


class IntVector(ctypes.Structure):
    _fields_ = [("size", ctypes.c_int), ("capacity", ctypes.c_int), ("data", ctypes.POINTER(ctypes.c_int))]


IntVectorPtr = ctypes.POINTER(IntVector)


class KthError(RuntimeError):
    def __init__(self, code, what=""):
        self.code = code
        super().__init__(f"{what}: {code} ({strerror(code)})" if what else f"{code} ({strerror(code)})")


class KthLibraryMissing(ImportError):
    pass


PROTOS = {
    "kth_strerror": (ctypes.c_char_p, [ctypes.c_int]),
    "kth_version": (ctypes.c_int, []),
    "kth_build_id": (ctypes.c_char_p, []),
    "kth_device_count": (ctypes.c_int, []),
    "kth_select_i32": (ctypes.c_int, [c_vp, ctypes.c_int64, ctypes.c_int64, c_i32p]),
    "kth_ctx_create": (ctypes.c_int, [ctypes.c_int, ctypes.POINTER(c_vp)]),
    "kth_ctx_destroy": (ctypes.c_int, [c_vp]),
    "kth_ctx_set_stream": (ctypes.c_int, [c_vp, c_vp]),
    "kth_ctx_sync": (ctypes.c_int, [c_vp]),
    "kth_ctx_reserve": (ctypes.c_int, [c_vp, ctypes.c_int64]),
    "kth_select_i32_ctx": (ctypes.c_int, [c_vp, c_vp, ctypes.c_int64, ctypes.c_int64, c_i32p]),
    "kth_select_i32_async": (ctypes.c_int, [c_vp, c_vp, ctypes.c_int64, ctypes.c_int64, c_vp]),
    "kth_ctx_last_stats": (ctypes.c_int, [c_vp, ctypes.POINTER(KthStats)]),
    "kth_ctx_coop": (ctypes.c_int, [c_vp]),
    "kth_ctx_test_hook": (ctypes.c_int, [c_vp, ctypes.c_int, ctypes.c_int64]),
    "kth_ctx_enable_timing": (ctypes.c_int, [c_vp, ctypes.c_int]),
    "kth_ctx_take_timing": (ctypes.c_int, [c_vp, ctypes.POINTER(ctypes.c_int64), ctypes.POINTER(ctypes.c_double),
                                           ctypes.POINTER(ctypes.c_double)]),
    "kth_select_rows_i32": (ctypes.c_int, [c_vp, c_vp, ctypes.c_int64, ctypes.c_int32, ctypes.c_int32, c_vp]),
    "kth_select_rows_f32": (ctypes.c_int, [c_vp, c_vp, ctypes.c_int64, ctypes.c_int32, ctypes.c_int32, c_vp]),
    "kth_topk_rows_i32": (ctypes.c_int, [c_vp, c_vp, ctypes.c_int64, ctypes.c_int32, ctypes.c_int32, ctypes.c_int,
                                         c_vp, c_vp]),
    "kth_topk_rows_f32": (ctypes.c_int, [c_vp, c_vp, ctypes.c_int64, ctypes.c_int32, ctypes.c_int32, ctypes.c_int,
                                         c_vp, c_vp]),
    "kth_topk_i32": (ctypes.c_int, [c_vp, c_vp, ctypes.c_int64, ctypes.c_int64, ctypes.c_int, c_vp, c_vp]),
    "kth_fill_synthetic": (ctypes.c_int, [c_vp, c_vp, ctypes.c_int64, ctypes.c_int64, ctypes.c_int64, ctypes.c_int,
                                          ctypes.c_uint64, ctypes.c_int32]),
    "kth_dist_begin": (ctypes.c_int, [c_vp, c_vp, ctypes.c_int64, ctypes.c_int64]),
    "kth_dist_sample": (ctypes.c_int, [c_vp, c_vp, ctypes.c_int64, c_vp, ctypes.c_int64]),
    "kth_dist_window": (ctypes.c_int, [c_vp, c_vp, ctypes.c_int64]),
    "kth_dist_scan": (ctypes.c_int, [c_vp, c_vp, ctypes.c_int64]),
    "kth_dist_level": (ctypes.c_int, [c_vp, c_vp, ctypes.c_int64, ctypes.c_int]),
    "kth_dist_result": (ctypes.c_int, [c_vp, c_vp]),
    "kth_dist_result_early": (ctypes.c_int, [c_vp, c_vp]),
    "kth_dist_select_rccl": (ctypes.c_int, [c_vp, c_vp, c_vp, c_vp, ctypes.c_int, c_vp, ctypes.c_int64, ctypes.c_int64,
                                            ctypes.c_int64, c_vp, c_vp, c_vp, ctypes.c_int64, c_vp, ctypes.c_int]),
    "kth_dist_sample_size": (ctypes.c_int64, [ctypes.c_int64]),
    "kth_sample_chunk": (ctypes.c_int, []),
    "kth_window_z": (ctypes.c_double, []),
    "kth_dist_cand_capacity": (ctypes.c_int64, [ctypes.c_int64]),
    "kth_window_slack64": (ctypes.c_int, []),
    "kth_sharded_create": (ctypes.c_int, [c_vp, ctypes.c_int, ctypes.POINTER(c_vp)]),
    "kth_sharded_destroy": (ctypes.c_int, [c_vp]),
    "kth_sharded_select_i32": (ctypes.c_int, [c_vp, c_vp, c_vp, ctypes.c_int64, c_i32p]),
    "kth_select_i32_sharded": (ctypes.c_int, [c_vp, c_vp, ctypes.c_int, ctypes.c_int64, c_i32p]),
    "kth_sharded_enqueue_us": (ctypes.c_double, [c_vp]),
    "kth_sharded_sample_split": (ctypes.c_int64, [c_vp, ctypes.c_int, c_vp]),
    "VecNew": (IntVectorPtr, [ctypes.c_int]),
    "VecAdd": (ctypes.c_int, [IntVectorPtr, ctypes.c_int]),
    "VecDelete": (None, [IntVectorPtr]),
    "VecErase": (ctypes.c_int, [IntVectorPtr, ctypes.c_int]),
    "MinFind": (ctypes.c_int, [IntVectorPtr]),
    "MaxFind": (ctypes.c_int, [IntVectorPtr]),
    "AverageFind": (ctypes.c_double, [IntVectorPtr]),
    "VecGetCapacity": (ctypes.c_int, [IntVectorPtr]),
    "VecGetSize": (ctypes.c_int, [IntVectorPtr]),
    "VecIsFull": (ctypes.c_int, [IntVectorPtr]),
    "VecSet": (ctypes.c_int, [IntVectorPtr, ctypes.c_int, ctypes.c_int]),
    "VecGet": (ctypes.c_int, [IntVectorPtr, ctypes.c_int]),
    "VecSearch": (ctypes.c_int, [IntVectorPtr, ctypes.c_int, ctypes.c_int]),
    "VecQuickSort": (None, [IntVectorPtr]),
    "VecQuickSort2": (None, [IntVectorPtr]),
    "VecBinarySearch": (ctypes.c_int, [IntVectorPtr, ctypes.c_int]),
    "VecBinarySearch2": (ctypes.c_int, [IntVectorPtr, ctypes.c_int]),
    "VecKthSelect": (ctypes.c_int, [IntVectorPtr, ctypes.c_int]),
    "VecKthSelectEx": (ctypes.c_int, [IntVectorPtr, ctypes.c_int, ctypes.POINTER(ctypes.c_int)]),
}

_lib = None


def hip_runtimes():
    found = set()
    try:
        with open("/proc/self/maps") as f:
            for line in f:
                path = line.rsplit(None, 1)[-1] if "/" in line else ""
                if "libamdhip64" in os.path.basename(path):
                    found.add(os.path.realpath(path))
    except OSError:
        pass
    return sorted(found)


def check_single_runtime():
    rts = hip_runtimes()
    if len(rts) > 1:
        raise RuntimeError(
            "two HIP runtimes are loaded in this process (" + ", ".join(rts) + "); "
            "import torch before libkth.so is loaded (kselect does this itself when torch is importable)")


def load():
    global _lib
    if _lib is not None:
        return _lib
    if not os.path.exists(LIB_PATH):
        raise KthLibraryMissing(
            f"libkth.so not found at {LIB_PATH}; build it with `make -C {PKG_ROOT}` "
            "(there is no CPU fallback)")
    try:
        import torch
    except ImportError:
        pass
    lib = ctypes.CDLL(LIB_PATH)
    check_single_runtime()
    for name, (res, args) in PROTOS.items():
        fn = getattr(lib, name)
        fn.restype = res
        fn.argtypes = args
    _lib = lib
    return lib


def strerror(code):
    try:
        return load().kth_strerror(code).decode()
    except Exception:
        return "?"


def check(code, what=""):
    if code != KTH_OK:
        raise KthError(code, what)
    return code
```

Baseline: 1599 Gkeys/s.

## Finish the selection inside the main pass when the candidate bucket fits on chip

Adds an in-pass finish to the main scan kernel. The last workgroup to arrive reduces the counts and the pre-histogram, decides whether the candidate bin is small enough, and either finishes the radix refinement over keys gathered per group or declines. When it finishes, the separate k_finish kernel exits early, saving its launch and its grid-barrier passes. The cost is extra housekeeping work and spin-waiting in the main kernel, plus a more complex decision protocol with fallbacks when the grid sizes differ or the bucket is too large.

```diff
diff --git a/include/kth.h b/include/kth.h
--- a/include/kth.h
+++ b/include/kth.h
@@ -57,11 +57,16 @@
 
 int kth_ctx_last_stats(kth_ctx *ctx, kth_stats *st);
 
+int kth_ctx_last_finish(kth_ctx *ctx);
+
+int kth_ctx_main_grid(const kth_ctx *ctx);
+
 int kth_ctx_coop(const kth_ctx *ctx);
 
 #define KTH_HOOK_FAULT_TOPK_RANK 1
 #define KTH_HOOK_FAULT_BARRIER 2
 #define KTH_HOOK_TOPK_SEG_CAP 3
+#define KTH_HOOK_INPASS 4
 int kth_ctx_test_hook(kth_ctx *ctx, int hook, int64_t value);
 
 int kth_ctx_enable_timing(kth_ctx *ctx, int on);
diff --git a/mpi-k-selection_amd/csrc/kth_api.hip b/mpi-k-selection_amd/csrc/kth_api.hip
--- a/mpi-k-selection_amd/csrc/kth_api.hip
+++ b/mpi-k-selection_amd/csrc/kth_api.hip
@@ -48,7 +48,11 @@
 constexpr size_t ZERO_WORDS = PRE_OFF + 2 * PRE_SET_WORDS;
 constexpr size_t BAR_OFF = ZERO_WORDS;
 constexpr size_t TAIL_OFF = BAR_OFF + kth::BAR_WORDS / 2;
-constexpr size_t SLOT_ALLOC_WORDS = TAIL_OFF + kth::FIN_LDS_KEYS / 2;
+constexpr size_t IP_OFF = TAIL_OFF + kth::FIN_LDS_KEYS / 2;
+constexpr size_t IP_TAIL_OFF = IP_OFF + kth::IP_WORDS / 2;
+constexpr size_t SLOT_ALLOC_WORDS = IP_TAIL_OFF + (size_t)kth::IP_NG * kth::IP_MAX_KEYS / 2;
+constexpr size_t IP_DEC_OFF = 3 * (size_t)kth::STATS_WORDS + 1;
+static_assert(IP_DEC_OFF == ISLOT_WORDS - 1 && kth::IP_WORDS % 2 == 0, "the decision word is the islots' last word");
 static_assert(kth::BAR_TAIL % 2 == 0, "the tail word is a u64");
 constexpr u64 FIN_SPARSE_PER_WG = (u64)kth::DENSE_BLK * kth::FIN_UNROLL * 4;
 constexpr double HEAD_SLACK = 1.5;
@@ -96,6 +100,10 @@
     uint32_t head_abs_div = 1024;
     int fin_set = 0;
     bool pre_hist = true;
+    bool inpass = true;
+    int inpass_grid = 0;
+    int inpass_hook = 0;
+    int last_window = 0;
     hipStream_t stream = nullptr;
     bool own_stream = false;
     int num_cu = 256;
@@ -356,7 +364,8 @@
     return reinterpret_cast<uint32_t *>(c->islots + PRE_OFF + (size_t)set * PRE_SET_WORDS);
 }
 
-void launch_finish(kth_ctx *c, StepArgs a, int32_t *d_out, int32_t *d_status, bool with_pre = false) {
+void launch_finish(kth_ctx *c, StepArgs a, int32_t *d_out, int32_t *d_status, bool with_pre = false,
+                   bool window = false, bool after_inpass = false) {
     const size_t mine = FSLOT_OFF + (size_t)c->fin_set * FSLOT_WORDS;
     a.stats_zero = c->islots + FSLOT_OFF + (size_t)(1 - c->fin_set) * FSLOT_WORDS;
     a.zero_words = FSLOT_WORDS;
@@ -365,6 +374,8 @@
     x.zero2_words = HSLOT_WORDS;
     x.pre = with_pre ? pre_set(c, c->fin_set) : nullptr;
     x.pre_zero = pre_set(c, 1 - c->fin_set);
+    if (after_inpass) x.ip_dec = reinterpret_cast<const uint32_t *>(c->islots + IP_DEC_OFF);
+    if (window) x.ip_kind = reinterpret_cast<uint32_t *>(c->islots + IP_OFF) + kth::IP_KIND;
     kth::k_finish<<<c->fin_grid, kth::DENSE_BLK, FIN_DYN_LDS, c->stream>>>(a, x);
     c->fin_set ^= 1;
 }
@@ -430,7 +441,7 @@
 
     if (c->coop) {
         StepArgs a = step(c, kth::ADV_INIT_SAMPLE, -1, 0, nullptr, nullptr, islot(c, 1));
-        a.zero_words = 2 * (u64)kth::STATS_WORDS + 1;
+        a.zero_words = 2 * (u64)kth::STATS_WORDS + 2;
         a.init_n = (u64)n;
         a.init_k = (u64)k;
         a.init_s = (u64)s;
@@ -445,13 +456,33 @@
         a.n_local = (u64)n;
         const bool pre = tflag == 0 && c->pre_hist;
         if (pre) a.pre_hist = pre_set(c, c->fin_set);
+        const bool ip = pre && !tflags && c->inpass;
         ev_main(c);
-        launch_main(c, a, tflag, tflags);
+        if (ip) {
+            kth::InPass p;
+            memset(&p, 0, sizeof p);
+            p.dec = reinterpret_cast<uint32_t *>(c->islots + IP_DEC_OFF);
+            p.w = reinterpret_cast<uint32_t *>(c->islots + IP_OFF);
+            p.tail = reinterpret_cast<uint32_t *>(c->islots + IP_TAIL_OFF);
+            p.st_fin = c->st + 0;
+            p.d_out = d_out;
+            p.d_status = d_status;
+            p.zero1 = c->islots + FSLOT_OFF + (size_t)(1 - c->fin_set) * FSLOT_WORDS;
+            p.zero1_words = FSLOT_WORDS;
+            p.zero2 = c->islots + HSLOT_OFF;
+            p.zero2_words = HSLOT_WORDS;
+            p.pre_zero = pre_set(c, 1 - c->fin_set);
+            p.hook = (uint32_t)c->inpass_hook;
+            kth::k_main<0, kth::InPass><<<c->inpass_grid, kth::BLK, 0, c->stream>>>(a, c->cand, nullptr, nullptr, kth::TkSeg{}, p);
+        } else {
+            launch_main(c, a, tflag, tflags);
+        }
         ev_main(c);
         a = step(c, kth::ADV_DECIDE, 1, 0, islot(c, 1), nullptr, nullptr);
         a.keys = keys;
         a.n_local = (u64)n;
-        launch_finish(c, a, d_out, d_status, pre);
+        launch_finish(c, a, d_out, d_status, pre, true, ip);
+        c->last_window = 1;
         c->last_state = 0;
         c->counts_left = true;
         return launch_check();
@@ -494,6 +525,7 @@
     a = step(c, kth::ADV_PICK, 0, 1, islot(c, 1), nullptr, nullptr);
     kth::k_result<<<1, kth::BLK, 0, c->stream>>>(a, d_out, d_status, c->islots, ISLOT_WORDS);
     c->last_state = 1;
+    c->last_window = 2;
     return launch_check();
 }
 
@@ -511,6 +543,7 @@
         c->dirty = false;
     }
     int rc;
+    c->last_window = 0;
     ev_mark(c, c->ev_total, c->total_used);
     if (n <= SMALL_N)
         rc = run_small(c, d_keys, n, k, d_out, d_status);
@@ -630,16 +663,18 @@
         if (hipGetDeviceProperties(&prop, device) == hipSuccess && prop.multiProcessorCount > 0)
             c->num_cu = prop.multiProcessorCount;
         {
-            const void *fns[7] = {reinterpret_cast<const void *>(kth::k_main<0>),
+            const void *fns[8] = {reinterpret_cast<const void *>(kth::k_main<0>),
                                   reinterpret_cast<const void *>(kth::k_main<1>),
                                   reinterpret_cast<const void *>(kth::k_main<2>),
                                   reinterpret_cast<const void *>(kth::k_main<3>),
                                   reinterpret_cast<const void *>(kth::k_main<4>),
                                   reinterpret_cast<const void *>(kth::k_main<5>),
-                                  reinterpret_cast<const void *>(kth::k_main<6>)};
+                                  reinterpret_cast<const void *>(kth::k_main<6>),
+                                  reinterpret_cast<const void *>(kth::k_main<0, kth::InPass>)};
             const char *e = getenv("KTH_MAIN_WG_PER_CU");
-            for (int v = 0; v < 7; ++v) {
+            for (int v = 0; v < 8; ++v) {
                 int per = 4;
+                bool known = false;
                 hipFuncAttributes fa;
                 if (hipFuncGetAttributes(&fa, fns[v]) == hipSuccess && fa.numRegs > 0) {
                     const int alloc = (fa.numRegs + 7) / 8 * 8;
@@ -647,10 +682,17 @@
                     const int lds = (int)fa.sharedSizeBytes;
                     const int by_lds = lds > 0 ? (160 * 1024) / lds : 8;
                     per = std::max(1, std::min(by_vgpr, by_lds));
+                    known = true;
                 }
                 (void)hipGetLastError();
+                const int fit = per;
                 if (e && atoi(e) > 0) per = atoi(e);
-                c->main_grid[v] = c->num_cu * per;
+                if (v < 7) {
+                    c->main_grid[v] = c->num_cu * per;
+                } else {
+                    c->inpass_grid = c->num_cu * per;
+                    if (!known || per > fit || c->inpass_grid != c->main_grid[0]) c->inpass = false;
+                }
             }
             if (const char *g = getenv("KTH_SPARSE_PER_WG")) c->sparse_per_wg = (u64)std::max(0, atoi(g));
             if (const char *g = getenv("KTH_DSCAN_PER_WG")) c->dscan_per_wg = (u64)std::max(1024, atoi(g));
@@ -658,6 +700,7 @@
             if (const char *g = getenv("KTH_POST_SPARSE_GRID")) c->post_sparse_grid = std::max(1, atoi(g));
             if (const char *g = getenv("KTH_COOP")) c->coop = atoi(g) != 0;
             if (const char *g = getenv("KTH_PRE_HIST")) c->pre_hist = atoi(g) != 0;
+            if (const char *g = getenv("KTH_INPASS")) c->inpass = c->inpass && atoi(g) != 0;
             c->fin_grid = c->num_cu;
             if (const char *g = getenv("KTH_FIN_GRID")) c->fin_grid = std::max(1, std::min(atoi(g), c->num_cu));
             if (const char *g = getenv("KTH_HEAD_SLACK")) c->head_slack64 = (uint32_t)std::max(0.0, atof(g) * 64.0);
@@ -722,6 +765,10 @@
         c->fault_barrier = value != 0;
         c->fault_once = value == 2;
         return KTH_OK;
+    case KTH_HOOK_INPASS:
+        if (value > 2) return KTH_EINVAL;
+        c->inpass_hook = (int)value;
+        return KTH_OK;
     case KTH_HOOK_TOPK_SEG_CAP:
         if (value > (int64_t)1 << 40) return KTH_EINVAL;
         c->topk_seg_cap = (u64)value;
@@ -838,6 +885,21 @@
 int kth_ctx_coop(const kth_ctx *c) {
     if (!c) return KTH_EINVAL;
     return c->coop ? 1 : 0;
+}
+
+int kth_ctx_last_finish(kth_ctx *c) {
+    if (!c) return KTH_EINVAL;
+    if (c->last_window != 1) return c->last_window;
+    KTH_TRY(set_device(c));
+    HIP_TRY(hipMemcpyAsync(c->h_status + 2, reinterpret_cast<uint32_t *>(c->islots + IP_OFF) + kth::IP_KIND,
+                           sizeof(int32_t), hipMemcpyDeviceToHost, c->stream));
+    HIP_TRY(hipStreamSynchronize(c->stream));
+    return c->h_status[2] == 1 ? 1 : 2;
+}
+
+int kth_ctx_main_grid(const kth_ctx *c) {
+    if (!c) return KTH_EINVAL;
+    return c->inpass ? c->inpass_grid : c->main_grid[0];
 }
 
 int kth_ctx_last_stats(kth_ctx *c, kth_stats *out) {
diff --git a/mpi-k-selection_amd/csrc/kth_coop.hpp b/mpi-k-selection_amd/csrc/kth_coop.hpp
--- a/mpi-k-selection_amd/csrc/kth_coop.hpp
+++ b/mpi-k-selection_amd/csrc/kth_coop.hpp
@@ -16,6 +16,8 @@
     uint32_t fault;
     const uint32_t *pre;
     uint32_t *pre_zero;
+    const uint32_t *ip_dec;
+    uint32_t *ip_kind;
 };
 
 template <int BLOCK>
@@ -396,6 +398,17 @@
     __shared__ uint32_t s_base[BAR_NG];
     __shared__ u64 s_cnt0;
     KTH_STAMP(a, 0);
+    {
+        const uint32_t dec = x.ip_dec ? *x.ip_dec : (uint32_t)IP_UNDECIDED;
+        const bool in_pass = dec == IP_DONE || dec == IP_INPASS;
+        if (x.ip_kind && blockIdx.x == 0 && threadIdx.x == 0) *x.ip_kind = in_pass ? 1u : 2u;
+        if (x.ip_dec && blockIdx.x == 0 && threadIdx.x < IP_NG)
+            (x.ip_kind - IP_KIND + IP_REP)[threadIdx.x * BAR_GROUP_STRIDE] = 0u;
+        if (in_pass) {
+            KTH_STAMP(a, 7);
+            return;
+        }
+    }
     GridBar gb = grid_bar_init(x.bar, s_base);
     for (int i = threadIdx.x; i < 2 * NBINS / 4; i += DENSE_BLK) reinterpret_cast<uint4 *>(&lh[0][0])[i] = make_uint4(0, 0, 0, 0);
     const uint32_t pre_incomplete = x.pre ? x.pre[PRE_INCOMPLETE] : 1u;
diff --git a/mpi-k-selection_amd/csrc/kth_inpass.hpp b/mpi-k-selection_amd/csrc/kth_inpass.hpp
--- /dev/null
+++ b/mpi-k-selection_amd/csrc/kth_inpass.hpp
@@ -0,0 +1,388 @@
+#pragma once
+
+namespace kth {
+
+enum : uint32_t { IP_UNDECIDED = 0, IP_DONE = 1, IP_INPASS = 2, IP_DECLINE = 3 };
+constexpr int IP_NG = 32;
+constexpr int IP_TOP = IP_NG * BAR_GROUP_STRIDE;
+constexpr int IP_TOP2 = IP_TOP + BAR_GROUP_STRIDE;
+constexpr int IP_KIND = IP_TOP2 + BAR_GROUP_STRIDE;
+constexpr int IP_REP = IP_KIND + BAR_GROUP_STRIDE;
+constexpr int IP_TG = IP_REP + IP_NG * BAR_GROUP_STRIDE;
+constexpr int IP_WORDS = IP_TG + IP_NG * BAR_GROUP_STRIDE;
+constexpr uint32_t IP_MAX_KEYS = (BLK / WAVE) * WREG;
+constexpr uint32_t IP_DIGIT = 10;
+constexpr int IP_POLL_SLEEP = 16;
+static_assert((1u << IP_DIGIT) <= (uint32_t)PRE_BINS, "the finisher's histogram is phist");
+static_assert(WREG % 4 == 0, "the regions are read as 16-byte words");
+
+struct NoInPass {};
+struct InPass {
+    uint32_t *dec;
+    uint32_t *w;
+    uint32_t *tail;
+    SelState *st_fin;
+    int32_t *d_out, *d_status;
+    u64 *zero1, *zero2;
+    u64 zero1_words, zero2_words;
+    uint32_t *pre_zero;
+    uint32_t hook;
+};
+
+__device__ __forceinline__ void inpass_housekeeping(const InPass &ip) {
+    const u64 i0 = (u64)blockIdx.x * BLK + threadIdx.x, step = (u64)gridDim.x * BLK;
+    for (u64 i = i0; i < ip.zero1_words; i += step) ip.zero1[i] = 0;
+    for (u64 i = i0; i < ip.zero2_words; i += step) ip.zero2[i] = 0;
+    for (u64 i = i0; i < (u64)PRE_WORDS; i += step) ip.pre_zero[i] = 0u;
+}
+
+__device__ __forceinline__ uint32_t ip_load(const uint32_t *p) {
+    return __hip_atomic_load(p, __ATOMIC_RELAXED, __HIP_MEMORY_SCOPE_AGENT);
+}
+__device__ __forceinline__ void ip_store(uint32_t *p, uint32_t v) {
+    __hip_atomic_store(p, v, __ATOMIC_RELAXED, __HIP_MEMORY_SCOPE_AGENT);
+}
+__device__ __forceinline__ uint32_t ip_publish(uint32_t *dec, uint32_t v) {
+    uint32_t old = IP_UNDECIDED;
+    const bool won = __hip_atomic_compare_exchange_strong(dec, &old, v, __ATOMIC_RELAXED, __ATOMIC_RELAXED,
+                                                          __HIP_MEMORY_SCOPE_AGENT);
+    return won ? v : old;
+}
+
+__device__ __forceinline__ void inpass_result(const InPass &ip, SelState &ss) {
+    SelState o = ss;
+    if (o.mode != MODE_DONE && !o.error) o.error = 16 + o.mode;
+    *ip.st_fin = o;
+    if (ip.d_out && !o.error) *ip.d_out = i32_of_key(o.answer);
+    if (ip.d_status) {
+        ip.d_status[0] = i32_of_key(o.answer);
+        ip.d_status[1] = (int32_t)o.error;
+    }
+}
+
+__device__ __forceinline__ void inpass_finish(const StepArgs &a, const InPass &ip, SelState &ss, u64 *scratch,
+                                              uint32_t *keys, const u64 *fill, uint32_t *phist,
+                                              const Stager<false> &st, u64 g) {
+    __shared__ uint32_t s_dec, s_last, s_pay[3], s_n, s_pos, s_off, s_total, s_ln, s_ans, s_err, s_bcast;
+    __shared__ uint32_t s_gcnt[IP_NG], s_gpre[IP_NG + 1];
+    __shared__ uint32_t s_list[WAVE];
+    const int lane = threadIdx.x & (WAVE - 1);
+    u64 *cnts = scratch + 8;
+    wait_mem();
+    __syncthreads();
+    if (threadIdx.x == 0) {
+        const uint32_t G = gridDim.x, ng = G < (uint32_t)IP_NG ? G : (uint32_t)IP_NG, grp = blockIdx.x % IP_NG;
+        const uint32_t gsz = (G - grp + IP_NG - 1u) / IP_NG;
+        uint32_t *gc = ip.w + grp * BAR_GROUP_STRIDE;
+        uint32_t last = 0;
+        if (__hip_atomic_fetch_add(gc, 1u, __ATOMIC_RELAXED, __HIP_MEMORY_SCOPE_AGENT) == gsz - 1u) {
+            ip_store(gc, 0u);
+            if (__hip_atomic_fetch_add(ip.w + IP_TOP, 1u, __ATOMIC_RELAXED, __HIP_MEMORY_SCOPE_AGENT) == ng - 1u) {
+                ip_store(ip.w + IP_TOP, 0u);
+                last = 1u;
+            }
+        }
+        s_last = last;
+        s_err = 0u;
+        s_bcast = 0u;
+    }
+    __syncthreads();
+    KTH_STAMP(a, 3);
+    const uint32_t W = cand_width(ss.lo, ss.hi), base = ss.lo + 1u;
+    const uint32_t d0 = min(W, fin_first_digit(W)), sh0 = W - d0;
+    if (s_last) {
+        if (threadIdx.x < NCOUNTS) cnts[threadIdx.x] = __hip_atomic_load(&a.stats_acc[threadIdx.x], __ATOMIC_RELAXED, __HIP_MEMORY_SCOPE_AGENT);
+        uint32_t incomplete = 1u;
+        if (a.pre_hist) {
+            static_assert(PRE_BINS == 4 * BLK, "a thread sums four bins of each copy");
+            const CoherentBuf pb(a.pre_hist, PRE_COPIES * PRE_BINS * 4);
+            uint4 q[PRE_COPIES];
+#pragma unroll
+            for (int c = 0; c < PRE_COPIES; ++c) q[c] = pb.load16((uint32_t)(c * PRE_BINS + 4 * threadIdx.x) * 4u);
+            incomplete = ip_load(a.pre_hist + PRE_INCOMPLETE);
+            uint4 s = make_uint4(0, 0, 0, 0);
+#pragma unroll
+            for (int c = 0; c < PRE_COPIES; ++c) {
+                s.x += q[c].x;
+                s.y += q[c].y;
+                s.z += q[c].z;
+                s.w += q[c].w;
+            }
+            reinterpret_cast<uint4 *>(phist)[threadIdx.x] = s;
+        }
+        __syncthreads();
+        if (threadIdx.x == 0) {
+            decide(ss, cnts);
+            if (ss.mode == MODE_CAND) ss.d0 = fin_first_digit(ss.W);
+        }
+        __syncthreads();
+        uint32_t out = IP_DECLINE, bin = 0, cnt = 0;
+        u64 below = 0;
+        if (ss.mode == MODE_DONE) {
+            out = IP_DONE;
+        } else if (ss.mode == MODE_CAND && incomplete == 0u && W > 0u) {
+            const bool ok = block_pick<BLK>([&](int i) { return (u64)phist[i]; }, 1 << d0, ss.t[0].k, &bin, &below, scratch);
+            cnt = ok ? phist[bin] : 0u;
+            if (ok && cnt + 3u * IP_NG <= IP_MAX_KEYS) out = IP_INPASS;
+        }
+        if (ip.hook == 1u) out = IP_DECLINE;
+        if (threadIdx.x == 0) {
+            const uint32_t pay[3] = {bin, (uint32_t)(ss.t[0].k - below), cnt};
+#pragma unroll
+            for (int i = 0; i < 3; ++i) s_pay[i] = pay[i];
+            const uint32_t now = ip_publish(ip.dec, out);
+            if (now == IP_DONE) inpass_result(ip, ss);
+            if (now == out) s_bcast = 1u;
+            s_dec = now;
+        }
+    } else if (threadIdx.x == 0) {
+        const uint32_t limit = ip.hook == 2u ? 0u : BAR_SPIN_LIMIT;
+        const uint32_t *mine = ip.w + IP_REP + (blockIdx.x % IP_NG) * BAR_GROUP_STRIDE;
+        uint32_t v = IP_UNDECIDED;
+        for (uint32_t spins = 0;; ++spins) {
+            if (spins >= limit) {
+                v = ip_publish(ip.dec, IP_DECLINE);
+                if (v == IP_DECLINE) s_bcast = 1u;
+                break;
+            }
+            v = ip_load(mine);
+            if (v != IP_UNDECIDED) break;
+            __builtin_amdgcn_s_sleep(IP_POLL_SLEEP);
+        }
+        if (v == IP_INPASS) {
+#pragma unroll
+            for (int i = 0; i < 3; ++i) s_pay[i] = ip_load(mine + 1 + i);
+        }
+        s_dec = v;
+    }
+    if (threadIdx.x == 0) s_n = 0u;
+    __syncthreads();
+    if (s_bcast && threadIdx.x < IP_NG) {
+        uint32_t *line = ip.w + IP_REP + threadIdx.x * BAR_GROUP_STRIDE;
+        if (s_dec == IP_INPASS) {
+#pragma unroll
+            for (int i = 0; i < 3; ++i) ip_store(line + 1 + i, s_pay[i]);
+            wait_mem();
+        }
+        ip_store(line, s_dec);
+    }
+    KTH_STAMP(a, 4);
+    const uint32_t dec = s_dec;
+    if (dec == IP_DECLINE) {
+        if (st.wfill) st.put(g, st.wfill);
+        return;
+    }
+    if (a.pre_hist)
+        for (u64 i = (u64)blockIdx.x * BLK + threadIdx.x; i < (u64)PRE_WORDS; i += (u64)gridDim.x * BLK) a.pre_hist[i] = 0u;
+    if (dec != IP_INPASS) return;
+    const uint32_t bin = s_pay[0], cnt = s_pay[2];
+    const uint32_t G = gridDim.x, ng = G < (uint32_t)IP_NG ? G : (uint32_t)IP_NG, grp = blockIdx.x % IP_NG;
+    const uint32_t gsz = (G - grp + IP_NG - 1u) / IP_NG;
+    uint32_t *gline = ip.w + IP_TG + grp * BAR_GROUP_STRIDE;
+    uint32_t *seg = ip.tail + (size_t)grp * IP_MAX_KEYS;
+    uint32_t *stage = phist;
+    auto keep = [&](uint32_t key, bool valid) {
+        const bool m = valid && ((key - base) >> sh0) == bin;
+        const u64 b = __ballot(m);
+        if (b == 0) return;
+        uint32_t at = 0;
+        if (lane == 0) at = atomicAdd(&s_n, (uint32_t)__popcll(b));
+        at = __shfl(at, 0, WAVE);
+        const uint32_t i = at + (uint32_t)__builtin_amdgcn_mbcnt_hi((uint32_t)(b >> 32), __builtin_amdgcn_mbcnt_lo((uint32_t)b, 0u));
+        if (m && i < (uint32_t)PRE_BINS) stage[i] = key;
+    };
+#pragma unroll
+    for (int q = 0; q < BLK / WAVE; ++q) {
+        const uint32_t nq = (uint32_t)fill[q];
+        for (uint32_t i0 = 0; i0 < nq; i0 += BLK) {
+            const uint32_t i = i0 + threadIdx.x;
+            keep(i < nq ? keys[q * WREG + i] : 0u, i < nq);
+        }
+    }
+    __syncthreads();
+    const uint32_t n_mine = s_n;
+    if (threadIdx.x == 0) {
+        const u64 old = __hip_atomic_fetch_add(reinterpret_cast<u64 *>(gline), (1ull << 32) | n_mine, __ATOMIC_RELAXED,
+                                               __HIP_MEMORY_SCOPE_AGENT);
+        uint32_t last = 0u;
+        if ((uint32_t)(old >> 32) == gsz - 1u)
+            last = __hip_atomic_fetch_add(ip.w + IP_TOP2, 1u, __ATOMIC_RELAXED, __HIP_MEMORY_SCOPE_AGENT) == ng - 1u;
+        s_off = (uint32_t)old;
+        s_last = last;
+        s_pos = 0u;
+    }
+    __syncthreads();
+    const uint32_t off = s_off;
+    if (n_mine <= (uint32_t)PRE_BINS) {
+        for (uint32_t i = threadIdx.x; i < n_mine; i += BLK)
+            if (off + i < IP_MAX_KEYS) ip_store(seg + off + i, stage[i]);
+    } else {
+#pragma unroll
+        for (int q = 0; q < BLK / WAVE; ++q) {
+            const uint32_t nq = (uint32_t)fill[q];
+            for (uint32_t i = threadIdx.x; i < nq; i += BLK) {
+                const uint32_t key = keys[q * WREG + i];
+                if (((key - base) >> sh0) == bin) {
+                    const uint32_t j = atomicAdd(&s_pos, 1u);
+                    if (off + j < IP_MAX_KEYS) ip_store(seg + off + j, key);
+                }
+            }
+        }
+    }
+    wait_mem();
+    __syncthreads();
+    if (threadIdx.x == 0) __hip_atomic_fetch_add(gline + 2, 1u, __ATOMIC_RELAXED, __HIP_MEMORY_SCOPE_AGENT);
+    if (!s_last) return;
+    if (threadIdx.x < NCOUNTS) cnts[threadIdx.x] = __hip_atomic_load(&a.stats_acc[threadIdx.x], __ATOMIC_RELAXED, __HIP_MEMORY_SCOPE_AGENT);
+    if (threadIdx.x < WAVE) {
+        const bool act = (uint32_t)lane < ng;
+        uint32_t *l = ip.w + IP_TG + (act ? lane : 0) * BAR_GROUP_STRIDE;
+        const uint32_t want = (G - (uint32_t)lane + IP_NG - 1u) / IP_NG;
+        bool done = !act;
+        for (uint32_t spins = 0;; ++spins) {
+            if (!done) done = ip_load(l + 2) == want;
+            if (__ballot(!done) == 0) break;
+            __builtin_amdgcn_s_sleep(1);
+            if (spins >= BAR_SPIN_LIMIT) {
+                if (lane == 0) s_err = ERR_BARRIER;
+                break;
+            }
+        }
+        uint32_t c4 = 0;
+        if (act) {
+            const uint32_t kc = ip_load(l);
+            s_gcnt[lane] = kc;
+            c4 = (kc + 3u) / 4u;
+            ip_store(l, 0u);
+            ip_store(l + 1, 0u);
+            ip_store(l + 2, 0u);
+        }
+        if (lane == 0) ip_store(ip.w + IP_TOP2, 0u);
+        const uint32_t inc = wave_incl_scan32(c4);
+        if ((uint32_t)lane < (uint32_t)IP_NG) s_gpre[lane + 1] = inc;
+        if (lane == 0) s_gpre[0] = 0u;
+        uint32_t tot = act ? s_gcnt[lane] : 0u;
+#pragma unroll
+        for (int o = WAVE / 2; o > 0; o >>= 1) tot += __shfl_xor(tot, o, WAVE);
+        if (lane == 0) s_total = tot;
+    }
+    __syncthreads();
+    const uint32_t total = s_total;
+    if (!s_err && total != cnt && threadIdx.x == 0) s_err = 32u;
+    __syncthreads();
+    const uint32_t nq4 = s_err ? 0u : s_gpre[IP_NG];
+    const uint32_t pad = base + ((bin ^ 1u) << sh0);
+    uint4 *k4 = reinterpret_cast<uint4 *>(keys);
+    {
+        const CoherentBuf tb(ip.tail, IP_NG * IP_MAX_KEYS * 4);
+        for (uint32_t v0 = 0; v0 < nq4; v0 += 4 * BLK) {
+            uint4 q[4];
+            uint32_t left[4];
+#pragma unroll
+            for (int u = 0; u < 4; ++u) {
+                const uint32_t v = v0 + u * BLK + threadIdx.x;
+                uint32_t gi = 0;
+#pragma unroll
+                for (uint32_t step = IP_NG / 2; step > 0; step >>= 1)
+                    if (s_gpre[gi + step] <= v) gi += step;
+                const uint32_t j = v - s_gpre[gi];
+                left[u] = v < nq4 ? s_gcnt[gi] - 4u * j : 0u;
+                q[u] = v < nq4 ? tb.load16((gi * IP_MAX_KEYS + 4u * j) * 4u) : make_uint4(0, 0, 0, 0);
+            }
+#pragma unroll
+            for (int u = 0; u < 4; ++u) {
+                const uint32_t v = v0 + u * BLK + threadIdx.x;
+                if (left[u] <= 1) q[u].y = pad;
+                if (left[u] <= 2) q[u].z = pad;
+                if (left[u] <= 3) q[u].w = pad;
+                if (v < nq4) k4[v] = q[u];
+            }
+        }
+    }
+    __syncthreads();
+    KTH_STAMP(a, 6);
+    uint32_t done = d0, prefix = bin, left = cnt;
+    u64 kk = s_pay[1];
+    while (!s_err) {
+        if (done == W) {
+            if (threadIdx.x == 0) s_ans = base + prefix;
+            break;
+        }
+        const uint32_t msh = W - done;
+        if (left <= (uint32_t)WAVE) {
+            if (threadIdx.x == 0) s_ln = 0u;
+            __syncthreads();
+            for (uint32_t v0 = 0; v0 < nq4; v0 += BLK) {
+                const uint32_t v = v0 + threadIdx.x;
+                const uint4 q = v < nq4 ? k4[v] : make_uint4(pad, pad, pad, pad);
+                const uint32_t kq[4] = {q.x, q.y, q.z, q.w};
+#pragma unroll
+                for (int j = 0; j < 4; ++j) {
+                    const bool m = ((kq[j] - base) >> msh) == prefix;
+                    const u64 b = __ballot(m);
+                    if (b == 0) continue;
+                    uint32_t at = 0;
+                    if (lane == 0) at = atomicAdd(&s_ln, (uint32_t)__popcll(b));
+                    at = __shfl(at, 0, WAVE);
+                    const uint32_t i = at + (uint32_t)__builtin_amdgcn_mbcnt_hi((uint32_t)(b >> 32), __builtin_amdgcn_mbcnt_lo((uint32_t)b, 0u));
+                    if (m && i < (uint32_t)WAVE) s_list[i] = kq[j];
+                }
+            }
+            __syncthreads();
+            if (threadIdx.x < WAVE) {
+                const uint32_t ln = s_ln < (uint32_t)WAVE ? s_ln : (uint32_t)WAVE;
+                const uint32_t mine = (uint32_t)lane < ln ? s_list[lane] : 0u;
+                uint32_t lt = 0, le = 0;
+                for (uint32_t j = 0; j < ln; ++j) {
+                    const uint32_t o = s_list[j];
+                    lt += o < mine ? 1u : 0u;
+                    le += o <= mine ? 1u : 0u;
+                }
+                const bool hit = (uint32_t)lane < ln && (u64)lt < kk && kk <= (u64)le;
+                if (hit) s_ans = mine;
+                if (__ballot(hit) == 0 && lane == 0) s_err = 33u;
+            }
+            break;
+        }
+        const uint32_t dd = msh < IP_DIGIT ? msh : IP_DIGIT, sh = msh - dd, mask = (1u << dd) - 1u;
+        for (int i = threadIdx.x; i < PRE_BINS; i += BLK) phist[i] = 0u;
+        __syncthreads();
+        for (uint32_t v = threadIdx.x; v < nq4; v += BLK) {
+            const uint4 q = k4[v];
+            const uint32_t kq[4] = {q.x - base, q.y - base, q.z - base, q.w - base};
+#pragma unroll
+            for (int j = 0; j < 4; ++j)
+                if ((kq[j] >> msh) == prefix) atomicAdd(&phist[(kq[j] >> sh) & mask], 1u);
+        }
+        __syncthreads();
+        uint32_t b = 0;
+        u64 below = 0;
+        const bool ok = block_pick<BLK>([&](int i) { return (u64)phist[i]; }, 1 << dd, kk, &b, &below, scratch);
+        if (!ok) {
+            if (threadIdx.x == 0) s_err = 1u;
+            break;
+        }
+        left = phist[b];
+        kk -= below;
+        prefix = (prefix << dd) | b;
+        done += dd;
+        __syncthreads();
+    }
+    __syncthreads();
+    if (threadIdx.x == 0) {
+        decide(ss, cnts);
+        ss.d0 = fin_first_digit(ss.W);
+        ss.t[0].done = ss.W;
+        if (s_err) {
+            ss.error = s_err;
+        } else {
+            ss.answer = s_ans;
+            ss.t[0].prefix = s_ans - base;
+        }
+        ss.mode = MODE_DONE;
+        inpass_result(ip, ss);
+    }
+    KTH_STAMP(a, 7);
+}
+
+}
diff --git a/mpi-k-selection_amd/csrc/kth_kernels.hip b/mpi-k-selection_amd/csrc/kth_kernels.hip
--- a/mpi-k-selection_amd/csrc/kth_kernels.hip
+++ b/mpi-k-selection_amd/csrc/kth_kernels.hip
@@ -910,10 +910,17 @@
 }
 static_assert(MAIN_UNROLL <= 8, "k_main<TF> keeps one row bit per 16-B load slot in a byte");
 static_assert(BLK / WAVE == 4, "k_main<TF> stores one flag byte per wave, four per tile (tk_row_flagged's mask)");
-template <int TF>
+}
+
+#include "kth_inpass.hpp"
+
+namespace kth {
+template <int TF, typename IPA = NoInPass>
 __global__ __launch_bounds__(BLK) void k_main(StepArgs a, uint32_t *__restrict__ cand_out,
                                               uint32_t *__restrict__ tflags, uint32_t *__restrict__ cand_rows,
-                                              TkSeg seg) {
+                                              TkSeg seg, IPA ip = IPA{}) {
+    constexpr bool IP = std::is_same<IPA, InPass>::value;
+    static_assert(!IP || TF == 0, "the in-pass finish belongs to the plain pass");
     constexpr int U = MAIN_UNROLL, S = MAIN_SUB, K = 4 * S;
 #ifdef KTH_DIAG_NOROWS
     constexpr bool ROWS = false;
@@ -1157,6 +1164,10 @@
         const uint32_t kk[2] = {okh ? p[threadIdx.x] : 0u, okt ? p[tail0 + threadIdx.x] : 0u};
         scan_keys<2, false>(kk, (okh ? 1u : 0u) | (okt ? 2u : 0u), slo, shi, clt, ceqlo, ceqhi, st);
     }
+    if constexpr (IP) {
+        KTH_STAMP(a, 2);
+        inpass_housekeeping(ip);
+    }
     u64 r0 = clt, r1 = ceqlo, r2 = ceqhi;
 #pragma unroll
     for (int o = WAVE / 2; o > 0; o >>= 1) {
@@ -1188,15 +1199,15 @@
         }
     }
     __syncthreads();
-    if (st.wfill) {
+    if (!IP && st.wfill) {
         u64 g = red[5][0];
         for (int w = 0; w < wid; ++w) g += red[4][w];
         st.put(g, st.wfill);
     }
     if constexpr (TF == 0) {
+        __shared__ uint32_t phist[PRE_BINS];
+        __shared__ uint32_t pflushed;
         if (a.pre_hist) {
-            __shared__ uint32_t phist[PRE_BINS];
-            __shared__ uint32_t pflushed;
             const uint32_t W = cand_width(ss.lo, ss.hi);
             const uint32_t d = min(W, fin_first_digit(W)), sh = W - d, base = ss.lo + 1u;
             if (threadIdx.x == 0) pflushed = 0u;
@@ -1228,9 +1239,15 @@
                 }
             }
         }
+        if constexpr (IP) {
+            u64 g = red[5][0];
+            for (int w = 0; w < wid; ++w) g += red[4][w];
+            inpass_finish(a, ip, ss, scratch, &region[0][0], red[4], phist, st, g);
+        }
     }
     KTH_STAMP(a, 5);
 }
+
 
 __global__ __launch_bounds__(BLK) void k_result(StepArgs a, int32_t *d_out, int32_t *d_status, u64 *izero,
                                                 u64 izero_words) {
diff --git a/mpi-k-selection_amd/kselect/__init__.py b/mpi-k-selection_amd/kselect/__init__.py
--- a/mpi-k-selection_amd/kselect/__init__.py
+++ b/mpi-k-selection_amd/kselect/__init__.py
@@ -11,6 +11,7 @@
     KTH_ENODEV,
     KTH_HOOK_FAULT_BARRIER,
     KTH_HOOK_FAULT_TOPK_RANK,
+    KTH_HOOK_INPASS,
     KTH_HOOK_TOPK_SEG_CAP,
     KTH_OK,
     KTH_PATH_LDS,
@@ -134,6 +135,18 @@
             check(r, "kth_ctx_coop")
         return bool(r)
 
+    def last_finish(self):
+        r = LIB.kth_ctx_last_finish(self._ctx)
+        if r < 0:
+            check(r, "kth_ctx_last_finish")
+        return r
+
+    def main_grid(self):
+        r = LIB.kth_ctx_main_grid(self._ctx)
+        if r < 0:
+            check(r, "kth_ctx_main_grid")
+        return r
+
     def test_hook(self, hook, value):
         check(LIB.kth_ctx_test_hook(self._ctx, int(hook), int(value)), "kth_ctx_test_hook")
 
diff --git a/mpi-k-selection_amd/kselect/_lib.py b/mpi-k-selection_amd/kselect/_lib.py
--- a/mpi-k-selection_amd/kselect/_lib.py
+++ b/mpi-k-selection_amd/kselect/_lib.py
@@ -19,7 +19,7 @@
 KTH_DIST_MAX_LEVELS = 3
 KTH_ROWS_MAX_COLS = 16384
 KTH_TOPK_MAX_COLS = 4096
-KTH_HOOK_FAULT_TOPK_RANK, KTH_HOOK_FAULT_BARRIER, KTH_HOOK_TOPK_SEG_CAP = 1, 2, 3
+KTH_HOOK_FAULT_TOPK_RANK, KTH_HOOK_FAULT_BARRIER, KTH_HOOK_TOPK_SEG_CAP, KTH_HOOK_INPASS = 1, 2, 3, 4
 
 c_i32p = ctypes.POINTER(ctypes.c_int32)
 c_u32p = ctypes.POINTER(ctypes.c_uint32)
@@ -80,6 +80,8 @@
     "kth_select_i32_async": (ctypes.c_int, [c_vp, c_vp, ctypes.c_int64, ctypes.c_int64, c_vp]),
     "kth_ctx_last_stats": (ctypes.c_int, [c_vp, ctypes.POINTER(KthStats)]),
     "kth_ctx_coop": (ctypes.c_int, [c_vp]),
+    "kth_ctx_last_finish": (ctypes.c_int, [c_vp]),
+    "kth_ctx_main_grid": (ctypes.c_int, [c_vp]),
     "kth_ctx_test_hook": (ctypes.c_int, [c_vp, ctypes.c_int, ctypes.c_int64]),
     "kth_ctx_enable_timing": (ctypes.c_int, [c_vp, ctypes.c_int]),
     "kth_ctx_take_timing": (ctypes.c_int, [c_vp, ctypes.POINTER(ctypes.c_int64), ctypes.POINTER(ctypes.c_double),
```

New measurement: 1578 Gkeys/s. 0.987x the previous value.
